# NERSC/swin_v2_weather

Measured on AMD Instinct MI355X. Metric: ERA5 samples/sec (73x721x1440) swin_73var depth12, higher is better.
Workload: dtype bf16

## Files before the change

include/swv2.h:

```cpp
#ifndef SWV2_H
#define SWV2_H
#include <stddef.h>
#include <stdint.h>

#ifdef __cplusplus
extern "C" {
#endif

#define SWV2_VERSION 112

enum {
    SWV2_OK = 0,
    SWV2_ERR_INVALID = -1,
    SWV2_ERR_UNSUPPORTED = -2,
    SWV2_ERR_LAUNCH = -3
};

int swv2_version(void);
const char* swv2_last_error(void);

int swv2_attn_geometry(int L, int head_dim, int* Lp, int* DP);

int swv2_attn_fwd_regime(int L, int head_dim, int has_bias, int dbg);

#define SWV2_ATTN_FIRST_GEN 16
#define SWV2_ATTN_PLAIN_STATS 8192
#define SWV2_ATTN_BWD_TWO_PHASE 32

typedef struct swv2_attn_args {
    const void* qkvh;
    const float* logit_scale;
    const float* bias;
    const void* bias_pack;
    void* oh;
    float* lse;
    const void* doh;
    const float* rnorm;
    void* dqkvh;
    float* dlogit_scale;
    float* dbias;
    int Bw, heads, L, head_dim;
    int nwh, nww;
    int mask_thr;
    int max_chunks;
    int dbg;
    void* dbias_ws;
    size_t dbias_ws_bytes;
    int dbias_partials;
} swv2_attn_args;

#define SWV2_ATTN_K_D256 0
#define SWV2_ATTN_K_FWD3 1
#define SWV2_ATTN_K_FWD3W 2
#define SWV2_ATTN_K_FWD3B 3
#define SWV2_ATTN_K_WIDE 4
#define SWV2_ATTN_K_STREAM 5
#define SWV2_ATTN_K_FIRST_GEN 6
typedef struct swv2_attn_kernel_t {
    int family;
    int Lp, DP;
    int LT, DK;
    int LFIX;
    int regime;
    int aug;
    int bias_lds;
    int qg;
} swv2_attn_kernel_t;
int swv2_attn_fwd_kernel(const swv2_attn_args* a, swv2_attn_kernel_t* out);
int swv2_attn_bwd_kernel(const swv2_attn_args* a, swv2_attn_kernel_t* out);

size_t swv2_attn_dbias_ws_bytes(int heads, int L, int max_chunks);

int swv2_attn_bias_chunks(int Bw);

size_t swv2_attn_pack_bias_bytes(int heads, int L);
int swv2_attn_pack_bias(const float* bias, int heads, int L, void* out, void* stream);
int swv2_attn_pack_bias_multi(const float* bias, int ntab, int heads, int L, void* out, void* stream);

int swv2_attn_fwd(const swv2_attn_args* a, void* stream);
int swv2_attn_bwd(const swv2_attn_args* a, void* stream);


enum swv2_operand_kind {
    SWV2_OP_F32 = 0,
    SWV2_OP_BF16 = 1,
    SWV2_OP_BF16_GELU = 2,
    SWV2_OP_HEADS = 3,
    SWV2_OP_PATCH = 4,
    SWV2_OP_MERGE_LN = 5,
    SWV2_OP_BF16_CSCALE = 6
};

typedef struct swv2_operand {
    int kind;
    const void* ptr;
    const int32_t* rowidx;
    const float* aux0;
    const float* aux1;
    const float* aux2;
    const float* aux3;
    long ld;
    int rows, cols;
    int p[4];
} swv2_operand;

enum swv2_epilogue_kind {
    SWV2_EPI_BF16 = 0,
    SWV2_EPI_F32 = 1,
    SWV2_EPI_QKV_HEADS = 2,
    SWV2_EPI_GELU_GRAD = 3,
    SWV2_EPI_UNPATCH = 4,
    SWV2_EPI_HEADS = 5,
    SWV2_EPI_F32_ACC = 6,
    SWV2_EPI_BF16_GELU = 7,
    SWV2_EPI_UNPATCH_LOSS = 8
};

typedef struct swv2_epilogue {
    int kind;
    void* out;
    const float* bias;
    const void* aux;
    float* aux_out;
    const int32_t* rowidx;
    long ld;
    int p[5];
    const float* loss_tar;
    const float* loss_qw;
    float* loss_part;
    void* loss_resid;
    int q[3];
} swv2_epilogue;

int swv2_linear(const swv2_operand* a, const void* w_bf16, const swv2_epilogue* e, int N, void* stream);

#define SWV2_LINEAR_RESIDENT_QKV128 0
#define SWV2_LINEAR_RESIDENT_QKV192X3 1
#define SWV2_LINEAR_RESIDENT_DX128 2
#define SWV2_LINEAR_WIDE_DMA 3
#define SWV2_LINEAR_WIDE 4
#define SWV2_LINEAR_TILE64 5
#define SWV2_LINEAR_TILE128 6
int swv2_linear_kernel(const swv2_operand* a, const swv2_epilogue* e, int N);

int swv2_linear_wgrad(const swv2_operand* dy, const swv2_operand* x, float* dW, float* db, const int32_t* nmap,
                      const int32_t* kmap, int ldw, int splits, void* stream);
size_t swv2_linear_wgrad_ws_bytes(int M, int N, int K, int splits);
int swv2_linear_wgrad_ws(const swv2_operand* dy, const swv2_operand* x, float* dW, float* db, const int32_t* nmap,
                         const int32_t* kmap, int ldw, int splits, void* ws, size_t ws_bytes, void* stream);
#define SWV2_WGRAD_WIDE 0
#define SWV2_WGRAD_TILE 1
int swv2_linear_wgrad_kernel(const swv2_operand* dy, const swv2_operand* x, int splits, size_t ws_bytes);

typedef struct swv2_wgrad_item {
    swv2_operand dy, x;
    float* dW;
    float* db;
    const int32_t* nmap;
    const int32_t* kmap;
    int ldw;
} swv2_wgrad_item;
size_t swv2_block_wgrad_ws_bytes(int C, int hidden, int heads_dp, int slices);
int swv2_block_wgrad(const swv2_wgrad_item* items4, int slices, void* ws, size_t ws_bytes, void* stream);
#define SWV2_BLOCK_WGRAD_SLAB 0
#define SWV2_BLOCK_WGRAD_GROUPED 1
int swv2_block_wgrad_kernel(const swv2_wgrad_item* items4, int slices, size_t ws_bytes);

int swv2_qk_normalize(void* qkvh_bf16, float* rnorm, int Bw, int heads, int Lp, int L, int DP, void* stream);

int swv2_prep_weight(const float* w, int rows, int cols, int transpose, const int32_t* row_map, int out_rows,
                     const int32_t* col_map, int out_cols, void* out_bf16, void* stream);

typedef struct swv2_prep_item {
    const float* w;
    int rows, cols, transpose;
    const int32_t* row_map;
    int out_rows;
    const int32_t* col_map;
    int out_cols;
    void* out;
    int out_f32;
} swv2_prep_item;
int swv2_prep_chunk(void);
int swv2_prep_item_chunks(int out_rows, int out_cols, int transpose);
int swv2_prep_multi(const swv2_prep_item* items_dev, const int* chunks_dev, int n_chunks, void* stream);

#define SWV2_LN_BWD_MAX_BLOCKS 512
typedef struct swv2_ln_args {
    const void* a;
    const float* res;
    const float* gamma;
    const float* beta;
    const float* scale;
    const int32_t* rowidx;
    float* y;
    float* mean;
    float* rstd;
    const float* dy;
    void* da;
    float* dgamma;
    float* dbeta;
    float* ws;
    int M, C, res_mod, rows_per_sample;
    float eps;
} swv2_ln_args;

int swv2_ln_residual_fwd(const swv2_ln_args* a, void* stream);
int swv2_ln_residual_bwd(const swv2_ln_args* a, void* stream);

int swv2_batch_sum(const float* in, float* out, int B, long n, int accumulate, void* stream);

int swv2_merge_stats(const float* x, float* mean, float* rstd, int B, int H, int W, int C, float eps, void* stream);
int swv2_merge_ln_bwd(const float* x, const void* dn_bf16, const float* gamma, const float* mean, const float* rstd,
                      float* dx, float* dgamma, float* dbeta, int B, int H, int W, int C, void* stream);

int swv2_loss_sums(const float* prd, const float* tar, const float* quad_w, float* sums, int BC, int H, int W, void* stream);
int swv2_loss_grad(const float* prd, const float* tar, const float* quad_w, const float* coef, float* dprd, int BC, int H,
                   int W, void* stream);
#define SWV2_LOSS_PART_SLICES 8
#define SWV2_LOSS_GROUP_ROWS 32
#define SWV2_LOSS_DUMP_BYTES 2048
#define SWV2_LOSS_RESID_PITCH(N) (((N) + 63) / 64 * 64)
int swv2_loss_part_reduce(const float* part, int M, int T, int B, int Cout, int Ct, int coff, float* sums, void* stream);
int swv2_loss_resid_to_image(const void* resid, const float* coef, const float* add, float* out, int B, int Cout, int H, int W, int Cs, int Cadd,
                             void* stream);
int swv2_loss_finalize(const float* sums, int layers, const float* chw, int BC, int C, int absolute, int squared, float* loss, float* coef,
                       void* stream);

int swv2_adam_step(float* p, const float* g, float* m, float* v, long n, float lr, float beta1, float beta2, float eps,
                   int step, float grad_inv_scale, void* stream);

typedef struct swv2_adam_item {
    float* p;
    const float* g;
    float* m;
    float* v;
    long n;
} swv2_adam_item;
int swv2_adam_chunk(void);
int swv2_adam_multi(const swv2_adam_item* items_dev, const int* chunks_dev, int n_chunks, float lr, float beta1, float beta2,
                    float eps, int step, float grad_inv_scale, void* stream);

typedef struct swv2_lamb_item {
    float* p;
    const float* g;
    float* m;
    float* v;
    long n;
    long chunk0;
} swv2_lamb_item;
#define SWV2_LAMB_SUM_DEPTH 64
#define SWV2_LAMB_ADAMW 1
#define SWV2_LAMB_BIAS_CORRECTION 2
#define SWV2_LAMB_GRAD_AVERAGING 4
#define SWV2_LAMB_NVLAMB 8
#define SWV2_LAMB_WS_GNORM2 0
#define SWV2_LAMB_WS_CLIP 1
#define SWV2_LAMB_WS_BC1 2
#define SWV2_LAMB_WS_BC2 3
#define SWV2_LAMB_WS_ITEM(i) (4 + 4 * (i))
int swv2_lamb_chunk(void);
size_t swv2_lamb_ws_bytes(int n_items, int n_chunks);
int swv2_lamb_grad_norm(const swv2_lamb_item* items_dev, const int* chunks_dev, int n_items, int n_chunks, float grad_inv_scale, void* ws,
                        size_t ws_bytes, void* stream);
int swv2_lamb_multi(const swv2_lamb_item* items_dev, const int* chunks_dev, int n_items, int n_chunks, int item_lo, int item_hi,
                    int chunk_lo, int chunk_hi, float lr, float beta1, float beta2, float eps, float weight_decay, float grad_inv_scale,
                    float max_grad_norm, int step, int flags, const float* extra_gnorm2, void* ws, size_t ws_bytes, void* stream);

int swv2_score_slices(int planes, int H, int W);
size_t swv2_score_ws_bytes(int planes, int H, int W);
int swv2_score_sums(const float* prd, long prd_bstride, const float* tar, long tar_bstride, const float* clim, const float* w, int B, int C,
                    int H, int W, void* ws, size_t ws_bytes, void* stream);
int swv2_score_finalize(const void* ws, size_t ws_bytes, int B, int C, int H, int W, const float* scale, float* sums, float* rmse, float* acc,
                        float* rmse_mean, float* acc_mean, void* stream);

int swv2_stats_slices(int C, int H, int W);
size_t swv2_stats_ws_bytes(int C, int H, int W);
int swv2_stats_accumulate(const float* slab, const float* prev, const double* pivot, double* tsum, void* part, size_t part_bytes, int C, int H,
                          int W, int first, void* stream);
int swv2_stats_finalize(const void* part, size_t part_bytes, const double* tsum, const double* pivot, int C, int H, int W, long T,
                        double* folded, float* time_means, void* stream);

size_t swv2_quantile_ws_bytes(int planes, int H, int W, int K);
int swv2_plane_order_stats(const float* x, long bstride, int B, int C, int H, int W, const int* ranks, int K, float* out, int* nan_count,
                           void* ws, size_t ws_bytes, void* stream);

size_t swv2_ens_ws_bytes(int planes, int H, int W, int M);
int swv2_ens_sums(const float* ens, long ens_mstride, long ens_bstride, const float* tar, long tar_bstride, const float* w, int M, int B, int C,
                  int H, int W, void* ws, size_t ws_bytes, void* stream);
int swv2_ens_finalize(const void* ws, size_t ws_bytes, int M, int B, int C, int H, int W, const float* scale, float* sums, int* hist,
                      float* ens_rmse, float* spread, float* crps, float* fair_crps, float* means, void* stream);

int swv2_era5_select_normalize(const float* raw, float* out, const int* chan, const float* mean, const float* stdv, int B, int S,
                               int Csel, int Craw, int Hraw, int Wraw, int H, int W, int Cout_total, int coff, void* stream);
int swv2_era5_zenith(float* out, const float* sun, int B, int nz, int H, int W, int Cout_total, int coff, void* stream);
int swv2_era5_static(const float* stat, float* out, int B, int Cs, int H, int W, int Cout_total, int coff, void* stream);

typedef struct {
    const void* oh;
    const void* wp;
    const float* bp;
    const float* gamma; const float* beta; const float* scale;
    const int32_t* rowidx;
    const float* x;
    void* a1; float* mean; float* rstd;
    float* y;
    int Bw, Lp, heads, C, rows_per_sample;
    float eps;
} swv2_proj_ln_args;
typedef struct {
    const float* dy;
    const void* a1; const float* mean; const float* rstd; const float* gamma; const float* scale;
    const int32_t* rowidx;
    const void* wpt;
    void* da1;
    void* doh;
    float* dgamma; float* dbeta; float* ws;
    int Bw, Lp, heads, C, rows_per_sample;
} swv2_proj_ln_bwd_args;
int swv2_proj_ln_supported(int C, int heads, int head_pad);
size_t swv2_proj_ln_bwd_ws_floats(int Mw, int C);
int swv2_proj_ln_fwd(const swv2_proj_ln_args* a, void* stream);
int swv2_proj_ln_bwd(const swv2_proj_ln_bwd_args* a, void* stream);

typedef struct {
    const float* x;
    const void* w1;
    const float* b1;
    const void* w2;
    const float* b2;
    const float* gamma;
    const float* beta;
    const float* scale;
    void* hpre;
    void* a2;
    float* mean;
    float* rstd;
    float* y;
    int M, C, hidden, rows_per_sample;
    float eps;
} swv2_mlp_args;
int swv2_mlp_supported(int C, int hidden);
int swv2_mlp_recompute_supported(int C, int hidden);
int swv2_mlp_fwd(const swv2_mlp_args* a, void* stream);

typedef struct {
    const float* dy;
    const void* a2;
    const float* mean;
    const float* rstd;
    const float* gamma;
    const float* scale;
    const void* hpre;
    const void* w2t;
    const void* w1t;
    void* da2;
    void* dh;
    float* dx;
    float* dgamma;
    float* dbeta;
    float* ws;
    int M, C, hidden, rows_per_sample;
    const float* x;
    const void* w1;
    const float* b1;
} swv2_mlp_bwd_args;
size_t swv2_mlp_bwd_ws_floats(int M, int C);
int swv2_mlp_bwd(const swv2_mlp_bwd_args* a, void* stream);

int swv2_cpb_fwd(const float* w1, const float* b1, const float* w2, const float* b2, const void* keep_bf16, float* bias,
                 int wh, int ww, int heads, int hidden, float drop_p, void* stream);
int swv2_cpb_bwd(const float* dbias, const float* w1, const float* b1, const float* w2, const void* keep_bf16, float* dw1,
                 float* db1, float* dw2, float* db2, int wh, int ww, int heads, int hidden, float drop_p, void* stream);
size_t swv2_cpb_bwd_ws_bytes(int wh, int ww, int heads, int hidden);
int swv2_cpb_bwd_ws(const float* dbias, const float* w1, const float* b1, const float* w2, const void* keep_bf16, float* dw1,
                    float* db1, float* dw2, float* db2, int wh, int ww, int heads, int hidden, float drop_p, void* ws,
                    size_t ws_bytes, void* stream);

int swv2_cpb_fwd_multi(const float* const* params_dev, int nblk, const uint32_t* keep_bits, float* bias, int wh, int ww, int heads,
                       int hidden, float drop_p, void* stream);
size_t swv2_cpb_bwd_multi_ws_bytes(int nblk, int wh, int ww, int heads, int hidden);
int swv2_cpb_bwd_multi(const float* dbias_tables, int nchunk, const float* const* params_dev, int nblk, const uint32_t* keep_bits,
                       float* grads, int wh, int ww, int heads, int hidden, float drop_p, void* ws, size_t ws_bytes, void* stream);

typedef struct swv2_block_desc {
    int B, T, C, heads, head_dim, hidden, L, Lp, DP, nwh, nww, mask_thr;
    const int32_t* rowidx;
    const int32_t* qkv_map;
    const int32_t* proj_map;
    const float *logit_scale, *qkv_b_pad, *proj_b, *n1_w, *n1_b, *fc1_b, *fc2_b, *n2_w, *n2_b;
    const void *w_qkv, *w_proj, *w_fc1, *w_fc2;
    const void *w_qkvt, *w_projt, *w_fc1t, *w_fc2t;
    const float* x;
    const float* bias;
    void* bias_pack;
    const float* dp1;
    const float* dp2;
    void* qkvh;  float* rnorm; void* oh; float* lse; void* a1; float* mean1; float* rstd1; float* x1;
    void* hpre;  void* hact;   void* a2; float* mean2; float* rstd2;
    float* x2;
    const float* dx2;
    void *da2, *dh, *da1, *doh, *dqkvh;
    float* dx1;
    float* ln_ws;
    float* dx;
    float *d_logit_scale, *d_bias, *d_qkv_w, *d_qkv_b, *d_proj_w, *d_proj_b, *d_n1_w, *d_n1_b, *d_fc1_w, *d_fc1_b,
          *d_fc2_w, *d_fc2_b, *d_n2_w, *d_n2_b;
    int wgrad_splits;
    int ev_kernel;
    void* ev_start;
    void* ev_stop;
    int fuse_proj_ln;
    int fuse_mlp;
    void* wgrad_ws;
    size_t wgrad_ws_bytes;
    int wgrad_group;
    void* grad_zero;
    size_t grad_zero_bytes;
    size_t ln_ws_floats;
    int bias_prepacked;
    float* dbias_part;
    size_t dbias_part_bytes;
} swv2_block_desc;

enum swv2_block_step {
    SWV2_STEP_RNORM_ZERO = 1,
    SWV2_STEP_QKV,
    SWV2_STEP_QK_NORMALIZE,
    SWV2_STEP_PACK_BIAS,
    SWV2_STEP_ATTN_FWD,
    SWV2_STEP_PROJ, SWV2_STEP_LN1_FWD,
    SWV2_STEP_PROJ_LN_FWD,
    SWV2_STEP_FC1, SWV2_STEP_FC2, SWV2_STEP_LN2_FWD,
    SWV2_STEP_MLP_FWD,
    SWV2_STEP_LN2_BWD, SWV2_STEP_WGRAD_FC2, SWV2_STEP_DH, SWV2_STEP_WGRAD_FC1, SWV2_STEP_DX1,
    SWV2_STEP_MLP_BWD,
    SWV2_STEP_LN1_BWD,
    SWV2_STEP_PROJ_LN_BWD,
    SWV2_STEP_WGRAD_PROJ, SWV2_STEP_DOH, SWV2_STEP_ATTN_BWD, SWV2_STEP_WGRAD_QKV, SWV2_STEP_DX,
    SWV2_STEP_LN_FOLD,
    SWV2_STEP_WGRAD_GROUP,
    SWV2_STEP_COUNT
};
#define SWV2_BLOCK_MAX_STEPS 12
enum { SWV2_DBIAS_NONE = 0,
       SWV2_DBIAS_ATOMICS = 1,
       SWV2_DBIAS_WGRAD_WS = 2,
       SWV2_DBIAS_PART = 3 };
typedef struct swv2_block_plan_t {
    int mlp_fused;
    int proj_ln_fused;
    int ln_deferred;
    int wgrad_grouped;
    int wgrad_kernel;
    int grad_zero_in_kernel;
    int attn_fwd_chunks, attn_bwd_chunks;
    int dbias_dest;
    size_t need_hact_bytes;
    size_t need_ln_ws_floats;
    size_t need_wgrad_ws_bytes;
    int n_fwd, n_bwd;
    int fwd[SWV2_BLOCK_MAX_STEPS], bwd[SWV2_BLOCK_MAX_STEPS];
} swv2_block_plan_t;
int swv2_block_plan(const swv2_block_desc* d, swv2_block_plan_t* out);
int swv2_block_step_id(int step);
const char* swv2_block_step_name(int step);

int swv2_block_fwd(const swv2_block_desc* d, void* stream);
int swv2_block_bwd(const swv2_block_desc* d, void* stream);

#ifdef __cplusplus
}
#endif
#endif
```

swin_v2_weather_amd/_lib.py:

```python
from __future__ import annotations

import ctypes as C
import os
import subprocess
import threading

HERE = os.path.dirname(os.path.abspath(__file__))
CSRC = os.path.join(HERE, "csrc")
LIB_PATH = os.environ.get("SWV2_LIB") or os.path.join(HERE, "libswv2.so")
SOURCES = ["capi.hip", "attn.hip", "attn2.hip", "attn_bwd_stream.hip", "attn_wide.hip", "attn_d256.hip", "gemm.hip", "gemm_tn.hip", "gemm_tn_slab.hip", "rowops.hip", "lamb.hip", "block.hip", "cpb.hip", "mlp.hip", "proj_ln.hip", "dataio.hip", "score.hip", "stats.hip", "quantile.hip", "ensemble.hip"]

ABI_VERSION = 112

_lib = None
_lock = threading.Lock()


class Swv2Error(RuntimeError):
    pass


def build_library(force: bool = False, verbose: bool = False) -> str:
    import glob
    srcs = [os.path.join(CSRC, s) for s in SOURCES]
    deps = srcs + glob.glob(os.path.join(CSRC, "*.h")) + [os.path.join(HERE, "..", "include", "swv2.h")]
    if not force and os.path.exists(LIB_PATH) and all(os.path.getmtime(LIB_PATH) >= os.path.getmtime(d) for d in deps):
        return LIB_PATH
    hipcc = os.environ.get("HIPCC", "/opt/rocm/bin/hipcc")
    objs, procs = [], []
    os.makedirs(os.path.join(HERE, "build"), exist_ok=True)
    for s in srcs:
        o = os.path.join(HERE, "build", os.path.basename(s) + ".o")
        objs.append(o)
        cmd = [hipcc, "--offload-arch=gfx950", "-O3", "-std=c++17", "-fPIC", "-c", s, "-o", o]
        procs.append((cmd, subprocess.Popen(cmd, stdout=subprocess.PIPE, stderr=subprocess.STDOUT)))
    for cmd, p in procs:
        out, _ = p.communicate()
        if p.returncode != 0:
            raise Swv2Error("hipcc failed: %s\n%s" % (" ".join(cmd), out.decode()))
        if verbose and out:
            print(out.decode())
    cmd = [hipcc, "--offload-arch=gfx950", "-shared", "-fPIC", "-o", LIB_PATH] + objs
    r = subprocess.run(cmd, stdout=subprocess.PIPE, stderr=subprocess.STDOUT)
    if r.returncode != 0:
        raise Swv2Error("link failed: %s\n%s" % (" ".join(cmd), r.stdout.decode()))
    return LIB_PATH


def source_hash() -> str:
    import glob
    import hashlib
    h = hashlib.sha256()
    files = sorted(glob.glob(os.path.join(CSRC, "*"))) + [os.path.join(HERE, "..", "include", "swv2.h")]
    for f in files:
        if os.path.isfile(f):
            h.update(os.path.basename(f).encode())
            h.update(open(f, "rb").read())
    return h.hexdigest()[:16]


class AttnArgs(C.Structure):
    _fields_ = [("qkvh", C.c_void_p), ("logit_scale", C.c_void_p), ("bias", C.c_void_p), ("bias_pack", C.c_void_p), ("oh", C.c_void_p),
                ("lse", C.c_void_p), ("doh", C.c_void_p), ("rnorm", C.c_void_p), ("dqkvh", C.c_void_p),
                ("dlogit_scale", C.c_void_p), ("dbias", C.c_void_p),
                ("Bw", C.c_int), ("heads", C.c_int), ("L", C.c_int), ("head_dim", C.c_int),
                ("nwh", C.c_int), ("nww", C.c_int), ("mask_thr", C.c_int), ("max_chunks", C.c_int), ("dbg", C.c_int),
                ("dbias_ws", C.c_void_p), ("dbias_ws_bytes", C.c_size_t), ("dbias_partials", C.c_int)]


class AttnKernelInfo(C.Structure):
    _fields_ = [(n, C.c_int) for n in ("family", "Lp", "DP", "LT", "DK", "LFIX", "regime", "aug", "bias_lds", "qg")]


ATTN_K_D256, ATTN_K_FWD3, ATTN_K_FWD3W, ATTN_K_FWD3B, ATTN_K_WIDE, ATTN_K_STREAM, ATTN_K_FIRST_GEN = range(7)
ATTN_K_NAMES = ("D256", "FWD3", "FWD3W", "FWD3B", "WIDE", "STREAM", "FIRST_GEN")


class Operand(C.Structure):
    _fields_ = [("kind", C.c_int), ("ptr", C.c_void_p), ("rowidx", C.c_void_p), ("aux0", C.c_void_p),
                ("aux1", C.c_void_p), ("aux2", C.c_void_p), ("aux3", C.c_void_p), ("ld", C.c_long),
                ("rows", C.c_int), ("cols", C.c_int), ("p", C.c_int * 4)]


class PrepItem(C.Structure):
    _fields_ = [("w", C.c_void_p), ("rows", C.c_int), ("cols", C.c_int), ("transpose", C.c_int), ("row_map", C.c_void_p),
                ("out_rows", C.c_int), ("col_map", C.c_void_p), ("out_cols", C.c_int), ("out", C.c_void_p), ("out_f32", C.c_int)]


class AdamItem(C.Structure):
    _fields_ = [("p", C.c_void_p), ("g", C.c_void_p), ("m", C.c_void_p), ("v", C.c_void_p), ("n", C.c_long)]


class LambItem(C.Structure):
    _fields_ = [("p", C.c_void_p), ("g", C.c_void_p), ("m", C.c_void_p), ("v", C.c_void_p), ("n", C.c_long), ("chunk0", C.c_long)]


class WgradItem(C.Structure):
    _fields_ = [("dy", Operand), ("x", Operand), ("dW", C.c_void_p), ("db", C.c_void_p), ("nmap", C.c_void_p),
                ("kmap", C.c_void_p), ("ldw", C.c_int)]


class Epilogue(C.Structure):
    _fields_ = [("kind", C.c_int), ("out", C.c_void_p), ("bias", C.c_void_p), ("aux", C.c_void_p),
                ("aux_out", C.c_void_p), ("rowidx", C.c_void_p), ("ld", C.c_long), ("p", C.c_int * 5),
                ("loss_tar", C.c_void_p), ("loss_qw", C.c_void_p), ("loss_part", C.c_void_p),
                ("loss_resid", C.c_void_p),
                ("q", C.c_int * 3)]


class ProjLnArgs(C.Structure):
    _fields_ = [(n, C.c_void_p) for n in ("oh", "wp", "bp", "gamma", "beta", "scale", "rowidx", "x", "a1", "mean", "rstd", "y")] + \
               [(n, C.c_int) for n in ("Bw", "Lp", "heads", "C", "rows_per_sample")] + [("eps", C.c_float)]


class ProjLnBwdArgs(C.Structure):
    _fields_ = [(n, C.c_void_p) for n in ("dy", "a1", "mean", "rstd", "gamma", "scale", "rowidx", "wpt", "da1", "doh", "dgamma", "dbeta",
                                           "ws")] + [(n, C.c_int) for n in ("Bw", "Lp", "heads", "C", "rows_per_sample")]


class MlpArgs(C.Structure):
    _fields_ = [(n, C.c_void_p) for n in ("x", "w1", "b1", "w2", "b2", "gamma", "beta", "scale", "hpre", "a2", "mean", "rstd", "y")] + \
               [(n, C.c_int) for n in ("M", "C", "hidden", "rows_per_sample")] + [("eps", C.c_float)]


class MlpBwdArgs(C.Structure):
    _fields_ = [(n, C.c_void_p) for n in ("dy", "a2", "mean", "rstd", "gamma", "scale", "hpre", "w2t", "w1t", "da2", "dh", "dx",
                                           "dgamma", "dbeta", "ws")] + [(n, C.c_int) for n in ("M", "C", "hidden", "rows_per_sample")] + \
               [(n, C.c_void_p) for n in ("x", "w1", "b1")]


class LnArgs(C.Structure):
    _fields_ = [("a", C.c_void_p), ("res", C.c_void_p), ("gamma", C.c_void_p), ("beta", C.c_void_p),
                ("scale", C.c_void_p), ("rowidx", C.c_void_p), ("y", C.c_void_p), ("mean", C.c_void_p),
                ("rstd", C.c_void_p), ("dy", C.c_void_p), ("da", C.c_void_p), ("dgamma", C.c_void_p),
                ("dbeta", C.c_void_p), ("ws", C.c_void_p), ("M", C.c_int), ("C", C.c_int), ("res_mod", C.c_int),
                ("rows_per_sample", C.c_int), ("eps", C.c_float)]


LN_BWD_MAX_BLOCKS = 512
ATTN_FIRST_GEN, ATTN_PLAIN_STATS, ATTN_BWD_TWO_PHASE = 16, 8192, 32
LOSS_PART_SLICES = 8
LOSS_GROUP_ROWS = 32
LOSS_DUMP_BYTES = 2048


def loss_resid_pitch(n: int) -> int:
    return (n + 63) // 64 * 64
class BlockDesc(C.Structure):
    _fields_ = ([(n, C.c_int) for n in ("B", "T", "C", "heads", "head_dim", "hidden", "L", "Lp", "DP", "nwh", "nww", "mask_thr")] +
                [(n, C.c_void_p) for n in (
                    "rowidx", "qkv_map", "proj_map",
                    "logit_scale", "qkv_b_pad", "proj_b", "n1_w", "n1_b", "fc1_b", "fc2_b", "n2_w", "n2_b",
                    "w_qkv", "w_proj", "w_fc1", "w_fc2", "w_qkvt", "w_projt", "w_fc1t", "w_fc2t",
                    "x", "bias", "bias_pack", "dp1", "dp2",
                    "qkvh", "rnorm", "oh", "lse", "a1", "mean1", "rstd1", "x1", "hpre", "hact", "a2", "mean2", "rstd2", "x2",
                    "dx2", "da2", "dh", "da1", "doh", "dqkvh", "dx1", "ln_ws", "dx",
                    "d_logit_scale", "d_bias", "d_qkv_w", "d_qkv_b", "d_proj_w", "d_proj_b", "d_n1_w", "d_n1_b", "d_fc1_w",
                    "d_fc1_b", "d_fc2_w", "d_fc2_b", "d_n2_w", "d_n2_b")] +
                [("wgrad_splits", C.c_int), ("ev_kernel", C.c_int), ("ev_start", C.c_void_p), ("ev_stop", C.c_void_p),
                 ("fuse_proj_ln", C.c_int), ("fuse_mlp", C.c_int), ("wgrad_ws", C.c_void_p), ("wgrad_ws_bytes", C.c_size_t), ("wgrad_group", C.c_int), ("grad_zero", C.c_void_p),
                 ("grad_zero_bytes", C.c_size_t), ("ln_ws_floats", C.c_size_t),
                 ("bias_prepacked", C.c_int), ("dbias_part", C.c_void_p), ("dbias_part_bytes", C.c_size_t)])


LAMB_ADAMW, LAMB_BIAS_CORRECTION, LAMB_GRAD_AVERAGING, LAMB_NVLAMB = 1, 2, 4, 8
LAMB_SUM_DEPTH = 64
LAMB_WS_GNORM2, LAMB_WS_CLIP, LAMB_WS_BC1, LAMB_WS_BC2 = range(4)


def lamb_ws_item(i: int) -> int:
    return 4 + 4 * i


BLOCK_MAX_STEPS = 12
DBIAS_NONE, DBIAS_ATOMICS, DBIAS_WGRAD_WS, DBIAS_PART = range(4)


class BlockPlan(C.Structure):
    _fields_ = ([(n, C.c_int) for n in ("mlp_fused", "proj_ln_fused", "ln_deferred", "wgrad_grouped", "wgrad_kernel", "grad_zero_in_kernel",
                                        "attn_fwd_chunks", "attn_bwd_chunks", "dbias_dest")] +
                [(n, C.c_size_t) for n in ("need_hact_bytes", "need_ln_ws_floats", "need_wgrad_ws_bytes")] +
                [("n_fwd", C.c_int), ("n_bwd", C.c_int), ("fwd", C.c_int * BLOCK_MAX_STEPS), ("bwd", C.c_int * BLOCK_MAX_STEPS)])

    def steps(self, phase):
        lib = load()
        return [lib.swv2_block_step_name(s).decode() for s in getattr(self, phase)[:getattr(self, "n_" + phase)]]


def block_plan(desc: BlockDesc) -> BlockPlan:
    plan = BlockPlan()
    check(load().swv2_block_plan(C.byref(desc), C.byref(plan)), "swv2_block_plan")
    return plan


OP_F32, OP_BF16, OP_BF16_GELU, OP_HEADS, OP_PATCH, OP_MERGE_LN, OP_BF16_CSCALE = range(7)
EPI_BF16, EPI_F32, EPI_QKV_HEADS, EPI_GELU_GRAD, EPI_UNPATCH, EPI_HEADS, EPI_F32_ACC, EPI_BF16_GELU, EPI_UNPATCH_LOSS = range(9)
LINEAR_RESIDENT_QKV128, LINEAR_RESIDENT_QKV192X3, LINEAR_RESIDENT_DX128, LINEAR_WIDE_DMA, LINEAR_WIDE, LINEAR_TILE64, LINEAR_TILE128 = range(7)
LINEAR_WIDE_KERNELS, LINEAR_TILE_KERNELS = (LINEAR_WIDE_DMA, LINEAR_WIDE), (LINEAR_TILE64, LINEAR_TILE128)
WGRAD_WIDE, WGRAD_TILE = range(2)
BLOCK_WGRAD_SLAB, BLOCK_WGRAD_GROUPED = range(2)

_P, _I, _L, _F = C.c_void_p, C.c_int, C.c_long, C.c_float
SYMBOLS = {
    "swv2_version": (_I, []),
    "swv2_last_error": (C.c_char_p, []),
    "swv2_attn_geometry": (_I, [_I, _I, C.POINTER(_I), C.POINTER(_I)]),
    "swv2_attn_fwd_regime": (_I, [_I, _I, _I, _I]),
    "swv2_attn_fwd_kernel": (_I, [C.POINTER(AttnArgs), C.POINTER(AttnKernelInfo)]),
    "swv2_attn_bwd_kernel": (_I, [C.POINTER(AttnArgs), C.POINTER(AttnKernelInfo)]),
    "swv2_attn_pack_bias_bytes": (C.c_size_t, [_I, _I]),
    "swv2_attn_dbias_ws_bytes": (C.c_size_t, [_I, _I, _I]),
    "swv2_attn_pack_bias": (_I, [_P, _I, _I, _P, _P]),
    "swv2_attn_pack_bias_multi": (_I, [_P, _I, _I, _I, _P, _P]),
    "swv2_attn_bias_chunks": (_I, [_I]),
    "swv2_attn_fwd": (_I, [C.POINTER(AttnArgs), _P]),
    "swv2_attn_bwd": (_I, [C.POINTER(AttnArgs), _P]),
    "swv2_linear": (_I, [C.POINTER(Operand), _P, C.POINTER(Epilogue), _I, _P]),
    "swv2_linear_kernel": (_I, [C.POINTER(Operand), C.POINTER(Epilogue), _I]),
    "swv2_linear_wgrad_kernel": (_I, [C.POINTER(Operand), C.POINTER(Operand), _I, C.c_size_t]),
    "swv2_block_wgrad_kernel": (_I, [C.POINTER(WgradItem), _I, C.c_size_t]),
    "swv2_linear_wgrad": (_I, [C.POINTER(Operand), C.POINTER(Operand), _P, _P, _P, _P, _I, _I, _P]),
    "swv2_linear_wgrad_ws_bytes": (C.c_size_t, [_I, _I, _I, _I]),
    "swv2_qk_normalize": (_I, [_P, _P, _I, _I, _I, _I, _I, _P]),
    "swv2_block_wgrad_ws_bytes": (C.c_size_t, [_I, _I, _I, _I]),
    "swv2_block_wgrad": (_I, [C.POINTER(WgradItem), _I, _P, C.c_size_t, _P]),
    "swv2_linear_wgrad_ws": (_I, [C.POINTER(Operand), C.POINTER(Operand), _P, _P, _P, _P, _I, _I, _P, C.c_size_t, _P]),
    "swv2_prep_weight": (_I, [_P, _I, _I, _I, _P, _I, _P, _I, _P, _P]),
    "swv2_ln_residual_fwd": (_I, [C.POINTER(LnArgs), _P]),
    "swv2_ln_residual_bwd": (_I, [C.POINTER(LnArgs), _P]),
    "swv2_batch_sum": (_I, [_P, _P, _I, _L, _I, _P]),
    "swv2_merge_stats": (_I, [_P, _P, _P, _I, _I, _I, _I, _F, _P]),
    "swv2_merge_ln_bwd": (_I, [_P, _P, _P, _P, _P, _P, _P, _P, _I, _I, _I, _I, _P]),
    "swv2_loss_sums": (_I, [_P, _P, _P, _P, _I, _I, _I, _P]),
    "swv2_loss_grad": (_I, [_P, _P, _P, _P, _P, _I, _I, _I, _P]),
    "swv2_loss_part_reduce": (_I, [_P, _I, _I, _I, _I, _I, _I, _P, _P]),
    "swv2_loss_resid_to_image": (_I, [_P, _P, _P, _P, _I, _I, _I, _I, _I, _I, _P]),
    "swv2_loss_finalize": (_I, [_P, _I, _P, _I, _I, _I, _I, _P, _P, _P]),
    "swv2_prep_chunk": (_I, []),
    "swv2_prep_item_chunks": (_I, [_I, _I, _I]),
    "swv2_prep_multi": (_I, [_P, _P, _I, _P]),
    "swv2_adam_chunk": (_I, []),
    "swv2_adam_multi": (_I, [_P, _P, _I, _F, _F, _F, _F, _I, _F, _P]),
    "swv2_adam_step": (_I, [_P, _P, _P, _P, _L, _F, _F, _F, _F, _I, _F, _P]),
    "swv2_lamb_chunk": (_I, []),
    "swv2_lamb_ws_bytes": (C.c_size_t, [_I, _I]),
    "swv2_lamb_grad_norm": (_I, [_P, _P, _I, _I, _F, _P, C.c_size_t, _P]),
    "swv2_lamb_multi": (_I, [_P, _P, _I, _I, _I, _I, _I, _I, _F, _F, _F, _F, _F, _F, _F, _I, _I, _P, _P, C.c_size_t, _P]),
    "swv2_score_slices": (_I, [_I, _I, _I]),
    "swv2_score_ws_bytes": (C.c_size_t, [_I, _I, _I]),
    "swv2_score_sums": (_I, [_P, _L, _P, _L, _P, _P, _I, _I, _I, _I, _P, C.c_size_t, _P]),
    "swv2_score_finalize": (_I, [_P, C.c_size_t, _I, _I, _I, _I, _P, _P, _P, _P, _P, _P, _P]),
    "swv2_stats_slices": (_I, [_I, _I, _I]),
    "swv2_stats_ws_bytes": (C.c_size_t, [_I, _I, _I]),
    "swv2_stats_accumulate": (_I, [_P, _P, _P, _P, _P, C.c_size_t, _I, _I, _I, _I, _P]),
    "swv2_stats_finalize": (_I, [_P, C.c_size_t, _P, _P, _I, _I, _I, _L, _P, _P, _P]),
    "swv2_quantile_ws_bytes": (C.c_size_t, [_I, _I, _I, _I]),
    "swv2_plane_order_stats": (_I, [_P, _L, _I, _I, _I, _I, _P, _I, _P, _P, _P, C.c_size_t, _P]),
    "swv2_ens_ws_bytes": (C.c_size_t, [_I, _I, _I, _I]),
    "swv2_ens_sums": (_I, [_P, _L, _L, _P, _L, _P, _I, _I, _I, _I, _I, _P, C.c_size_t, _P]),
    "swv2_ens_finalize": (_I, [_P, C.c_size_t, _I, _I, _I, _I, _I, _P, _P, _P, _P, _P, _P, _P, _P, _P]),
    "swv2_era5_select_normalize": (_I, [_P, _P, _P, _P, _P] + [_I] * 10 + [_P]),
    "swv2_era5_zenith": (_I, [_P, _P, _I, _I, _I, _I, _I, _I, _P]),
    "swv2_era5_static": (_I, [_P, _P, _I, _I, _I, _I, _I, _I, _P]),
    "swv2_proj_ln_supported": (_I, [_I, _I, _I]),
    "swv2_proj_ln_bwd_ws_floats": (C.c_size_t, [_I, _I]),
    "swv2_proj_ln_fwd": (_I, [C.POINTER(ProjLnArgs), _P]),
    "swv2_proj_ln_bwd": (_I, [C.POINTER(ProjLnBwdArgs), _P]),
    "swv2_mlp_supported": (_I, [_I, _I]),
    "swv2_mlp_recompute_supported": (_I, [_I, _I]),
    "swv2_mlp_fwd": (_I, [C.POINTER(MlpArgs), _P]),
    "swv2_mlp_bwd_ws_floats": (C.c_size_t, [_I, _I]),
    "swv2_mlp_bwd": (_I, [C.POINTER(MlpBwdArgs), _P]),
    "swv2_cpb_fwd": (_I, [_P, _P, _P, _P, _P, _P, _I, _I, _I, _I, _F, _P]),
    "swv2_cpb_bwd": (_I, [_P, _P, _P, _P, _P, _P, _P, _P, _P, _I, _I, _I, _I, _F, _P]),
    "swv2_cpb_bwd_ws": (_I, [_P, _P, _P, _P, _P, _P, _P, _P, _P, _I, _I, _I, _I, _F, _P, C.c_size_t, _P]),
    "swv2_cpb_bwd_ws_bytes": (C.c_size_t, [_I, _I, _I, _I]),
    "swv2_cpb_fwd_multi": (_I, [_P, _I, _P, _P, _I, _I, _I, _I, _F, _P]),
    "swv2_cpb_bwd_multi_ws_bytes": (C.c_size_t, [_I, _I, _I, _I, _I]),
    "swv2_cpb_bwd_multi": (_I, [_P, _I, _P, _I, _P, _P, _I, _I, _I, _I, _F, _P, C.c_size_t, _P]),
    "swv2_block_plan": (_I, [C.POINTER(BlockDesc), C.POINTER(BlockPlan)]),
    "swv2_block_step_id": (_I, [_I]),
    "swv2_block_step_name": (C.c_char_p, [_I]),
    "swv2_block_fwd": (_I, [C.POINTER(BlockDesc), _P]),
    "swv2_block_bwd": (_I, [C.POINTER(BlockDesc), _P]),
}


def load() -> C.CDLL:
    global _lib
    if _lib is not None:
        return _lib
    with _lock:
        if _lib is None:
            if not os.path.exists(LIB_PATH):
                raise Swv2Error(f"{LIB_PATH} not found: run `python -c 'import __graft_entry__ as g; g.build()'` "
                                "(the HIP library is required; there is no fallback path)")
            import torch
            lib = C.CDLL(LIB_PATH)
            for name, (res, args) in SYMBOLS.items():
                fn = getattr(lib, name)
                fn.restype, fn.argtypes = res, args
            got = lib.swv2_version()
            if got != ABI_VERSION:
                raise Swv2Error(f"{LIB_PATH} reports ABI revision {got}, this binding mirrors revision {ABI_VERSION} of include/swv2.h: "
                                "rebuild the library (python -c 'import __graft_entry__ as g; g.build()')")
            _lib = lib
    return _lib


def check(rc: int, what: str = "") -> None:
    if rc != 0:
        msg = load().swv2_last_error()
        raise Swv2Error(f"{what} failed with code {rc}: {msg.decode() if msg else ''}")
```

swin_v2_weather_amd/csrc/block.hip:

```cpp
#include "common.h"

namespace {

swv2_operand op(int kind, const void* p, int rows, int cols, long ld, const int32_t* rowidx = nullptr) {
    swv2_operand o = {};
    o.kind = kind; o.ptr = p; o.rowidx = rowidx; o.ld = ld; o.rows = rows; o.cols = cols;
    return o;
}
swv2_operand op_heads(const void* p, int Bw, int heads, int parts, int Lp, int DP) {
    swv2_operand o = op(SWV2_OP_HEADS, p, Bw * Lp, parts * heads * DP, parts);
    o.p[0] = heads; o.p[2] = Lp; o.p[3] = DP;
    return o;
}
swv2_epilogue epi(int kind, void* out, long ld, const float* bias = nullptr, const void* aux = nullptr,
                  float* aux_out = nullptr, const int32_t* rowidx = nullptr) {
    swv2_epilogue e = {};
    e.kind = kind; e.out = out; e.ld = ld; e.bias = bias; e.aux = aux; e.aux_out = aux_out; e.rowidx = rowidx;
    return e;
}
swv2_attn_args attn(const swv2_block_desc* d, int max_chunks) {
    swv2_attn_args a = {};
    a.qkvh = d->qkvh; a.logit_scale = d->logit_scale; a.bias = d->bias; a.bias_pack = d->bias ? d->bias_pack : nullptr;
    a.oh = d->oh; a.lse = d->lse;
    a.Bw = d->B * d->nwh * d->nww; a.heads = d->heads; a.L = d->L; a.head_dim = d->head_dim; a.nwh = d->nwh; a.nww = d->nww;
    a.mask_thr = d->mask_thr; a.max_chunks = max_chunks;
    return a;
}
void wgrad_items(const swv2_block_desc* d, bool fused, swv2_wgrad_item it[4]) {
    const int BT = d->B * d->T, Bw = d->B * d->nwh * d->nww, Mw = Bw * d->Lp, C = d->C, h = d->heads, hid = d->hidden;
    it[0].dy = op(SWV2_OP_BF16, d->da2, BT, C, C);
    it[0].x = fused ? op(SWV2_OP_BF16_GELU, d->hpre, BT, hid, hid) : op(SWV2_OP_BF16, d->hact, BT, hid, hid);
    it[0].dW = d->d_fc2_w; it[0].db = d->d_fc2_b; it[0].ldw = hid;
    it[1].dy = op(SWV2_OP_BF16, d->dh, BT, hid, hid); it[1].x = op(SWV2_OP_F32, d->x1, BT, C, C);
    it[1].dW = d->d_fc1_w; it[1].db = d->d_fc1_b; it[1].ldw = C;
    it[2].dy = op(SWV2_OP_BF16, d->da1, Mw, C, C); it[2].x = op_heads(d->oh, Bw, h, 1, d->Lp, d->DP);
    it[2].dW = d->d_proj_w; it[2].db = d->d_proj_b; it[2].kmap = d->proj_map; it[2].ldw = C;
    it[3].dy = op_heads(d->dqkvh, Bw, h, 3, d->Lp, d->DP); it[3].x = op(SWV2_OP_F32, d->x, Mw, C, C, d->rowidx);
    it[3].dW = d->d_qkv_w; it[3].db = d->d_qkv_b; it[3].nmap = d->qkv_map; it[3].ldw = C;
}
#define TRY(x) do { int rc_ = (x); if (rc_) return rc_; } while (0)

const struct { int id; const char* name; } STEPS[SWV2_STEP_COUNT] = {
    {0, "end"},
    {0, "rnorm_zero"}, {1, "qkv"}, {0, "qk_normalize"}, {0, "pack_bias"}, {2, "attn_fwd"}, {3, "proj"}, {4, "ln1_fwd"}, {3, "proj_ln_fwd"},
    {5, "fc1"}, {6, "fc2"}, {7, "ln2_fwd"}, {5, "mlp_fwd"},
    {11, "ln2_bwd"}, {12, "wgrad_fc2"}, {13, "dh"}, {14, "wgrad_fc1"}, {15, "dx1"}, {13, "mlp_bwd"}, {16, "ln1_bwd"}, {16, "proj_ln_bwd"},
    {17, "wgrad_proj"}, {18, "doh"}, {19, "attn_bwd"}, {20, "wgrad_qkv"}, {21, "dx"}, {0, "ln_fold"}, {22, "wgrad_group"},
};
static_assert(SWV2_STEP_WGRAD_GROUP + 1 == SWV2_STEP_COUNT && SWV2_STEP_MLP_FWD == 12 && SWV2_STEP_LN2_BWD == 13, "STEPS follows enum swv2_block_step");

#define LAUNCH(step, x)                                                                                     \
    do {                                                                                                    \
        const bool t_ = d->ev_kernel == STEPS[step].id && d->ev_start && d->ev_stop;                         \
        if (t_) (void)hipEventRecord((hipEvent_t)d->ev_start, (hipStream_t)st);                             \
        TRY(x);                                                                                             \
        if (t_) (void)hipEventRecord((hipEvent_t)d->ev_stop, (hipStream_t)st);                              \
    } while (0)

int plan_block(const swv2_block_desc* d, swv2_block_plan_t* p) {
    SWV2_CHECK_ARG(d && p, "swv2_block_plan: null descriptor or plan");
    SWV2_CHECK_ARG(d->B > 0 && d->T > 0 && d->C > 0 && d->heads > 0 && d->hidden > 0 && d->Lp > 0 && d->DP > 0 && d->nwh > 0 && d->nww > 0,
                   "swv2_block_plan: non-positive geometry");
    *p = {};
    const int BT = d->B * d->T, Bw = d->B * d->nwh * d->nww, Mw = Bw * d->Lp, C = d->C, h = d->heads, hid = d->hidden;
    const int sp = d->wgrad_splits > 0 ? d->wgrad_splits : 64;
    const size_t ws_bytes = d->wgrad_ws ? d->wgrad_ws_bytes : 0;
    const size_t ln_pair = swv2_mlp_bwd_ws_floats(BT, C) + swv2_proj_ln_bwd_ws_floats(Mw, C);
    p->need_ln_ws_floats = std::max((size_t)SWV2_LN_BWD_MAX_BLOCKS * 2 * C, ln_pair);
    p->need_wgrad_ws_bytes = d->wgrad_group ? swv2_block_wgrad_ws_bytes(C, hid, h * d->DP, 0) : 0;
    const int prod[4][3] = {{BT, C, hid}, {BT, hid, C}, {Mw, C, h * d->DP}, {Mw, 3 * h * d->DP, C}};
    for (const auto& q : prod)
        p->need_wgrad_ws_bytes = std::max(p->need_wgrad_ws_bytes, swv2_linear_wgrad_ws_bytes(q[0], q[1], q[2], sp));

    p->mlp_fused = d->fuse_mlp && swv2_mlp_supported(C, hid);
    p->proj_ln_fused = d->fuse_proj_ln && swv2_proj_ln_supported(C, h, d->DP);
    p->need_hact_bytes = p->mlp_fused ? 0 : (size_t)BT * hid * 2;
    p->ln_deferred = p->mlp_fused && p->proj_ln_fused && d->ln_ws_floats >= ln_pair;
    p->wgrad_grouped = d->wgrad_group && p->mlp_fused && d->wgrad_ws && ws_bytes >= swv2_block_wgrad_ws_bytes(C, hid, h * d->DP, 0);
    p->wgrad_kernel = -1;
    p->grad_zero_in_kernel = p->mlp_fused && d->grad_zero != nullptr;
    p->attn_fwd_chunks = d->bias ? 32 : 64;
    p->attn_bwd_chunks = 64;
    if (d->bias) {
        p->attn_bwd_chunks = swv2_attn_bias_chunks(Bw);
        p->dbias_dest = d->dbias_part ? SWV2_DBIAS_PART : ws_bytes ? SWV2_DBIAS_WGRAD_WS : SWV2_DBIAS_ATOMICS;
    } else if (d->Lp == 176 && h <= 256) {
        p->attn_bwd_chunks = 256 / h;
    }

    auto fwd = [&](int s) { p->fwd[p->n_fwd++] = s; };
    auto bwd = [&](int s) { p->bwd[p->n_bwd++] = s; };
    const bool wide = d->DP > 64;
    if (wide) fwd(SWV2_STEP_RNORM_ZERO);
    fwd(SWV2_STEP_QKV);
    if (wide) fwd(SWV2_STEP_QK_NORMALIZE);
    if (d->bias && d->bias_pack && !d->bias_prepacked) fwd(SWV2_STEP_PACK_BIAS);
    fwd(SWV2_STEP_ATTN_FWD);
    if (p->proj_ln_fused) fwd(SWV2_STEP_PROJ_LN_FWD);
    else { fwd(SWV2_STEP_PROJ); fwd(SWV2_STEP_LN1_FWD); }
    if (p->mlp_fused) fwd(SWV2_STEP_MLP_FWD);
    else { fwd(SWV2_STEP_FC1); fwd(SWV2_STEP_FC2); fwd(SWV2_STEP_LN2_FWD); }

    const bool single = !p->wgrad_grouped;
    if (p->mlp_fused) {
        bwd(SWV2_STEP_MLP_BWD);
        if (single) { bwd(SWV2_STEP_WGRAD_FC2); bwd(SWV2_STEP_WGRAD_FC1); }
    } else {
        bwd(SWV2_STEP_LN2_BWD); bwd(SWV2_STEP_WGRAD_FC2); bwd(SWV2_STEP_DH); bwd(SWV2_STEP_WGRAD_FC1); bwd(SWV2_STEP_DX1);
    }
    bwd(p->proj_ln_fused ? SWV2_STEP_PROJ_LN_BWD : SWV2_STEP_LN1_BWD);
    if (single) bwd(SWV2_STEP_WGRAD_PROJ);
    if (!p->proj_ln_fused) bwd(SWV2_STEP_DOH);
    bwd(SWV2_STEP_ATTN_BWD);
    if (single) bwd(SWV2_STEP_WGRAD_QKV);
    bwd(SWV2_STEP_DX);
    if (p->ln_deferred && single) bwd(SWV2_STEP_LN_FOLD);
    if (p->wgrad_grouped) bwd(SWV2_STEP_WGRAD_GROUP);
    return SWV2_OK;
}

}

extern "C" int swv2_block_step_id(int step) { return step > 0 && step < SWV2_STEP_COUNT ? STEPS[step].id : -1; }
extern "C" const char* swv2_block_step_name(int step) { return step > 0 && step < SWV2_STEP_COUNT ? STEPS[step].name : nullptr; }

extern "C" int swv2_block_plan(const swv2_block_desc* d, swv2_block_plan_t* p) {
    TRY(plan_block(d, p));
    if (p->wgrad_grouped) {
        swv2_wgrad_item it[4] = {};
        wgrad_items(d, true, it);
        p->wgrad_kernel = swv2_block_wgrad_kernel(it, 0, d->wgrad_ws_bytes);
    }
    return SWV2_OK;
}

extern "C" int swv2_block_fwd(const swv2_block_desc* d, void* st) {
    SWV2_CHECK_ARG(d && d->x && d->x2 && d->qkvh && d->rowidx, "swv2_block_fwd: null descriptor field");
    swv2_block_plan_t p;
    TRY(plan_block(d, &p));
    SWV2_CHECK_ARG(d->hact || !p.need_hact_bytes, "swv2_block_fwd: the separate MLP kernels need hact (swv2_block_plan: need_hact_bytes)");
    const int BT = d->B * d->T, Bw = d->B * d->nwh * d->nww, Mw = Bw * d->Lp, C = d->C, h = d->heads, hid = d->hidden;
    for (int i = 0; i < p.n_fwd; ++i) switch (p.fwd[i]) {
    case SWV2_STEP_RNORM_ZERO:
        if (hipMemsetAsync(d->rnorm, 0, (size_t)Bw * h * 2 * d->Lp * sizeof(float), (hipStream_t)st) != hipSuccess) {
            swv2_set_error("swv2_block_fwd: hipMemsetAsync(rnorm) failed");
            return SWV2_ERR_LAUNCH;
        }
        break;
    case SWV2_STEP_QKV: {
        swv2_operand a = op(SWV2_OP_F32, d->x, Mw, C, C, d->rowidx);
        swv2_epilogue e = epi(SWV2_EPI_QKV_HEADS, d->qkvh, 0, d->qkv_b_pad, nullptr, d->rnorm);
        e.p[0] = h; e.p[2] = d->Lp; e.p[3] = d->DP; e.p[4] = d->L;
        LAUNCH(SWV2_STEP_QKV, swv2_linear(&a, d->w_qkv, &e, 3 * h * d->DP, st));
    } break;
    case SWV2_STEP_QK_NORMALIZE: TRY(swv2_qk_normalize(d->qkvh, (float*)d->rnorm, Bw, h, d->Lp, d->L, d->DP, st)); break;
    case SWV2_STEP_PACK_BIAS: TRY(swv2_attn_pack_bias(d->bias, h, d->L, d->bias_pack, st)); break;
    case SWV2_STEP_ATTN_FWD: {
        swv2_attn_args a = attn(d, p.attn_fwd_chunks);
        LAUNCH(SWV2_STEP_ATTN_FWD, swv2_attn_fwd(&a, st));
    } break;
    case SWV2_STEP_PROJ_LN_FWD: {
        swv2_proj_ln_args m = {};
        m.oh = d->oh; m.wp = d->w_proj; m.bp = d->proj_b; m.gamma = d->n1_w; m.beta = d->n1_b; m.scale = d->dp1; m.rowidx = d->rowidx;
        m.x = d->x; m.a1 = d->a1; m.mean = d->mean1; m.rstd = d->rstd1; m.y = d->x1; m.Bw = Bw; m.Lp = d->Lp; m.heads = h; m.C = C;
        m.rows_per_sample = d->T; m.eps = 1e-5f;
        LAUNCH(SWV2_STEP_PROJ_LN_FWD, swv2_proj_ln_fwd(&m, st));
    } break;
    case SWV2_STEP_PROJ: {
        swv2_operand a = op_heads(d->oh, Bw, h, 1, d->Lp, d->DP);
        swv2_epilogue e = epi(SWV2_EPI_BF16, d->a1, C, d->proj_b);
        LAUNCH(SWV2_STEP_PROJ, swv2_linear(&a, d->w_proj, &e, C, st));
    } break;
    case SWV2_STEP_LN1_FWD: {
        swv2_ln_args l = {};
        l.a = d->a1; l.res = d->x; l.gamma = d->n1_w; l.beta = d->n1_b; l.scale = d->dp1; l.rowidx = d->rowidx; l.y = d->x1;
        l.mean = d->mean1; l.rstd = d->rstd1; l.M = Mw; l.C = C; l.res_mod = 0; l.rows_per_sample = d->T; l.eps = 1e-5f;
        LAUNCH(SWV2_STEP_LN1_FWD, swv2_ln_residual_fwd(&l, st));
    } break;
    case SWV2_STEP_MLP_FWD: {
        swv2_mlp_args m = {};
        m.x = d->x1; m.w1 = d->w_fc1; m.b1 = d->fc1_b; m.w2 = d->w_fc2; m.b2 = d->fc2_b; m.gamma = d->n2_w; m.beta = d->n2_b;
        m.scale = d->dp2; m.hpre = d->hpre; m.a2 = d->a2; m.mean = d->mean2; m.rstd = d->rstd2; m.y = d->x2;
        m.M = BT; m.C = C; m.hidden = hid; m.rows_per_sample = d->T; m.eps = 1e-5f;
        LAUNCH(SWV2_STEP_MLP_FWD, swv2_mlp_fwd(&m, st));
    } break;
    case SWV2_STEP_FC1: {
        swv2_operand a = op(SWV2_OP_F32, d->x1, BT, C, C);
        swv2_epilogue e = epi(SWV2_EPI_BF16_GELU, d->hpre, hid, d->fc1_b, nullptr, (float*)d->hact);
        LAUNCH(SWV2_STEP_FC1, swv2_linear(&a, d->w_fc1, &e, hid, st));
    } break;
    case SWV2_STEP_FC2: {
        swv2_operand a = op(SWV2_OP_BF16, d->hact, BT, hid, hid);
        swv2_epilogue e = epi(SWV2_EPI_BF16, d->a2, C, d->fc2_b);
        LAUNCH(SWV2_STEP_FC2, swv2_linear(&a, d->w_fc2, &e, C, st));
    } break;
    case SWV2_STEP_LN2_FWD: {
        swv2_ln_args l = {};
        l.a = d->a2; l.res = d->x1; l.gamma = d->n2_w; l.beta = d->n2_b; l.scale = d->dp2; l.y = d->x2; l.mean = d->mean2;
        l.rstd = d->rstd2; l.M = BT; l.C = C; l.res_mod = 0; l.rows_per_sample = d->T; l.eps = 1e-5f;
        LAUNCH(SWV2_STEP_LN2_FWD, swv2_ln_residual_fwd(&l, st));
    } break;
    }
    return SWV2_OK;
}

extern "C" int swv2_block_bwd(const swv2_block_desc* d, void* st) {
    SWV2_CHECK_ARG(d && d->dx2 && d->dx && d->da2 && d->dh && d->dx1 && d->da1 && d->doh && d->dqkvh && d->ln_ws,
                   "swv2_block_bwd: null descriptor field");
    swv2_block_plan_t p;
    TRY(plan_block(d, &p));
    SWV2_CHECK_ARG(d->hact || !p.need_hact_bytes, "swv2_block_bwd: the separate MLP kernels need hact (swv2_block_plan: need_hact_bytes)");
    const int BT = d->B * d->T, Bw = d->B * d->nwh * d->nww, Mw = Bw * d->Lp, C = d->C, h = d->heads, hid = d->hidden;
    const int sp = d->wgrad_splits > 0 ? d->wgrad_splits : 64;
    swv2_wgrad_item it[4] = {};
    wgrad_items(d, p.mlp_fused, it);
    float* const ln1_ws = p.ln_deferred ? d->ln_ws + swv2_mlp_bwd_ws_floats(BT, C) : d->ln_ws;
    int n_ln1 = 0, n_ln2 = 0;
    for (int i = 0; i < p.n_bwd; ++i) switch (const int s = p.bwd[i]; s) {
    case SWV2_STEP_MLP_BWD: {
        swv2_mlp_bwd_args m = {};
        m.dy = d->dx2; m.a2 = d->a2; m.mean = d->mean2; m.rstd = d->rstd2; m.gamma = d->n2_w; m.scale = d->dp2; m.hpre = d->hpre;
        m.w2t = d->w_fc2t; m.w1t = d->w_fc1t; m.da2 = d->da2; m.dh = d->dh; m.dx = d->dx1; m.dgamma = d->d_n2_w;
        m.dbeta = d->d_n2_b; m.ws = d->ln_ws; m.M = BT; m.C = C; m.hidden = hid; m.rows_per_sample = d->T;
        LAUNCH(SWV2_STEP_MLP_BWD, swv2_mlp_bwd_impl(&m, st, p.ln_deferred ? &n_ln2 : nullptr, p.grad_zero_in_kernel ? (float*)d->grad_zero : nullptr,
                                                    (long)(d->grad_zero_bytes / 4)));
    } break;
    case SWV2_STEP_LN2_BWD: {
        swv2_ln_args l = {};
        l.a = d->a2; l.dy = d->dx2; l.gamma = d->n2_w; l.scale = d->dp2; l.mean = d->mean2; l.rstd = d->rstd2; l.da = d->da2;
        l.dgamma = d->d_n2_w; l.dbeta = d->d_n2_b; l.ws = d->ln_ws; l.M = BT; l.C = C; l.rows_per_sample = d->T;
        LAUNCH(SWV2_STEP_LN2_BWD, swv2_ln_residual_bwd(&l, st));
    } break;
    case SWV2_STEP_WGRAD_FC2: case SWV2_STEP_WGRAD_FC1: case SWV2_STEP_WGRAD_PROJ: case SWV2_STEP_WGRAD_QKV: {
        const swv2_wgrad_item& w = it[s == SWV2_STEP_WGRAD_FC2 ? 0 : s == SWV2_STEP_WGRAD_FC1 ? 1 : s == SWV2_STEP_WGRAD_PROJ ? 2 : 3];
        LAUNCH(s, swv2_linear_wgrad_ws(&w.dy, &w.x, w.dW, w.db, w.nmap, w.kmap, w.ldw, sp, d->wgrad_ws, d->wgrad_ws_bytes, st));
    } break;
    case SWV2_STEP_DH: {
        swv2_epilogue e = epi(SWV2_EPI_GELU_GRAD, d->dh, hid, nullptr, d->hpre);
        LAUNCH(SWV2_STEP_DH, swv2_linear(&it[0].dy, d->w_fc2t, &e, hid, st));
    } break;
    case SWV2_STEP_DX1: {
        swv2_epilogue e = epi(SWV2_EPI_F32, d->dx1, C, nullptr, d->dx2);
        LAUNCH(SWV2_STEP_DX1, swv2_linear(&it[1].dy, d->w_fc1t, &e, C, st));
    } break;
    case SWV2_STEP_PROJ_LN_BWD: {
        swv2_proj_ln_bwd_args m = {};
        m.dy = d->dx1; m.a1 = d->a1; m.mean = d->mean1; m.rstd = d->rstd1; m.gamma = d->n1_w; m.scale = d->dp1; m.rowidx = d->rowidx;
        m.wpt = d->w_projt; m.da1 = d->da1; m.doh = d->doh; m.dgamma = d->d_n1_w; m.dbeta = d->d_n1_b; m.ws = ln1_ws;
        m.Bw = Bw; m.Lp = d->Lp; m.heads = h; m.C = C; m.rows_per_sample = d->T;
        LAUNCH(SWV2_STEP_PROJ_LN_BWD, swv2_proj_ln_bwd_impl(&m, st, p.ln_deferred ? &n_ln1 : nullptr));
    } break;
    case SWV2_STEP_LN1_BWD: {
        swv2_ln_args l = {};
        l.a = d->a1; l.dy = d->dx1; l.gamma = d->n1_w; l.scale = d->dp1; l.rowidx = d->rowidx; l.mean = d->mean1; l.rstd = d->rstd1;
        l.da = d->da1; l.dgamma = d->d_n1_w; l.dbeta = d->d_n1_b; l.ws = d->ln_ws; l.M = Mw; l.C = C; l.rows_per_sample = d->T;
        LAUNCH(SWV2_STEP_LN1_BWD, swv2_ln_residual_bwd(&l, st));
    } break;
    case SWV2_STEP_DOH: {
        swv2_epilogue e = epi(SWV2_EPI_HEADS, d->doh, 0);
        e.p[0] = h; e.p[2] = d->Lp; e.p[3] = d->DP; e.p[4] = d->L;
        LAUNCH(SWV2_STEP_DOH, swv2_linear(&it[2].dy, d->w_projt, &e, h * d->DP, st));
    } break;
    case SWV2_STEP_ATTN_BWD: {
        swv2_attn_args a = attn(d, p.attn_bwd_chunks);
        a.doh = d->doh; a.rnorm = d->rnorm; a.dqkvh = d->dqkvh; a.dlogit_scale = d->d_logit_scale; a.dbias = d->d_bias;
        if (p.dbias_dest == SWV2_DBIAS_PART) { a.dbias_ws = d->dbias_part; a.dbias_ws_bytes = d->dbias_part_bytes; a.dbias_partials = 1; }
        if (p.dbias_dest == SWV2_DBIAS_WGRAD_WS) { a.dbias_ws = d->wgrad_ws; a.dbias_ws_bytes = d->wgrad_ws_bytes; }
        LAUNCH(SWV2_STEP_ATTN_BWD, swv2_attn_bwd(&a, st));
    } break;
    case SWV2_STEP_DX: {
        swv2_epilogue e = epi(SWV2_EPI_F32, d->dx, C, nullptr, d->dx1, nullptr, d->rowidx);
        LAUNCH(SWV2_STEP_DX, swv2_linear(&it[3].dy, d->w_qkvt, &e, C, st));
    } break;
    case SWV2_STEP_LN_FOLD:
        swv2_launch_ln_partials_reduce2(d->ln_ws, d->d_n2_w, d->d_n2_b, n_ln2, ln1_ws, d->d_n1_w, d->d_n1_b, n_ln1, C, (hipStream_t)st);
        break;
    case SWV2_STEP_WGRAD_GROUP: {
        swv2_ln_partials lnp = {{d->ln_ws, ln1_ws}, {d->d_n2_w, d->d_n1_w}, {d->d_n2_b, d->d_n1_b}, {n_ln2, n_ln1}, C};
        LAUNCH(SWV2_STEP_WGRAD_GROUP, swv2_block_wgrad_ln(it, 0, d->wgrad_ws, d->wgrad_ws_bytes, p.ln_deferred ? &lnp : nullptr, st));
    } break;
    }
    return SWV2_OK;
}
```

swin_v2_weather_amd/csrc/gemm.hip:

```cpp
#include "common.h"

#include <cmath>
#include <cstdlib>
#include "gemm_common.h"

namespace {

constexpr int EP = 68;

struct EpiDesc {
    void* out;
    const float* bias;
    const void* aux;
    float* aux_out;
    const int32_t* rowidx;
    long ld;
    int M, N;
    int p0, p1, p2, p3, p4;
    uint32_t mg0, mg1, mg2;
    const float* loss_tar; const float* loss_qw; float* loss_part; uint16_t* loss_resid; int q0, q1, q2, q3;
};

enum { E_BF16 = 0, E_F32 = 1, E_QKV_HEADS = 2, E_GELU_GRAD = 3, E_UNPATCH = 4, E_HEADS = 5, E_F32_ACC = 6, E_BF16_GELU = 7,
       E_UNPATCH_LOSS = 8, E_UNPATCH_LOSS_SKIP = 9 };
// ... 638 lines not shown
    const int wr = wave >> 2, wc = wave & 3;
    const int xcd = blockIdx.x & 7, nper = gridDim.x >> 3, stages = K / 32;
    const uint32_t lds0 = (uint32_t)(uintptr_t)smem;
    const int drow = wave * 32 + (lane >> 2);
    int dkc[2];
#pragma unroll
    for (int i = 0; i < 2; ++i) dkc[i] = (lane & 3) ^ ((0 - ((drow + 16 * i) >> 2)) & 3);
    struct Tile { int m_base, n_base; uint32_t boff[2], aoff[2]; };
    auto make_tile = [&](int mt, int nt) {
        Tile t;
        t.m_base = mt * WBM; t.n_base = nt * WBN;
#pragma unroll
        for (int i = 0; i < 2; ++i) {
            const int row = drow + 16 * i;
            t.boff[i] = 2u * (uint32_t)(min(t.n_base + row, N - 1) * K + dkc[i] * 8);
            t.aoff[i] = AK == A_BF16 ? 2u * (uint32_t)(min(t.m_base + row, M - 1) * (int)al.d.ld + dkc[i] * 8) : 0u;
        }
        return t;
    };
    auto issue = [&](const Tile& tl, int t, int slot) {
        const uint32_t la = lds0 + (uint32_t)(slot * WSTG * 2) + (uint32_t)(wave * 2048), lb = la + WBM * 32 * 2;
#pragma unroll
        for (int i = 0; i < 2; ++i) dma_x4(Wb + t * 32, tl.boff[i], lb + 1024 * i);
        if constexpr (AK == A_BF16) {
#pragma unroll
            for (int i = 0; i < 2; ++i) dma_x4((const uint16_t*)al.d.ptr + t * 32, tl.aoff[i], la + 1024 * i);
        } else {
#pragma unroll
            for (int i = 0; i < 2; ++i)
                dma_x4(al.d.ptr, 2u * al.elem_off(min(tl.m_base + drow + 16 * i, M - 1), t * 32 + dkc[i] * 8), la + 1024 * i);
        }
    };
    int v = blockIdx.x >> 3, mt = 0, nt = 0;
    while (v < vmax && !wide_tile(xcd, v, mtiles, ntn, mt, nt)) v += nper;
    if (v >= vmax) return;
    Tile cur = make_tile(mt, nt);
    issue(cur, 0, 0); issue(cur, 1, 1); issue(cur, 2, 2);
    asm volatile("s_waitcnt vmcnt(8)" ::: "memory");
    __builtin_amdgcn_s_barrier();
    if (wr == 1) __builtin_amdgcn_s_barrier();
    for (;;) {
        int v2 = v + nper, mt2 = 0, nt2 = 0;
        while (v2 < vmax && !wide_tile(xcd, v2, mtiles, ntn, mt2, nt2)) v2 += nper;
        const bool has_next = v2 < vmax;
        const Tile nxt = has_next ? make_tile(mt2, nt2) : cur;
        f32x4 acc[8][4];
#pragma unroll
        for (int i = 0; i < 8; ++i)
#pragma unroll
            for (int j = 0; j < 4; ++j) acc[i][j] = (f32x4){0.f, 0.f, 0.f, 0.f};
        for (int t = 0; t < stages; ++t) {
            if (t + 3 < stages) issue(cur, t + 3, (t + 3) & 3);
            else issue(nxt, has_next ? t + 3 - stages : stages - 1, (t + 3) & 3);
            const uint16_t* As = smem + (t & 3) * WSTG;
            const uint16_t* Bs = As + WBM * 32;
            bf16x8 af[8], bf[4];
#pragma unroll
            for (int j = 0; j < 4; ++j) bf[j] = *(const bf16x8*)(Bs + swz32(wc * 64 + j * 16 + fr, g));
#pragma unroll
            for (int i = 0; i < 8; ++i) af[i] = *(const bf16x8*)(As + swz32(wr * 128 + i * 16 + fr, g));
            asm volatile("s_waitcnt vmcnt(8)" ::: "memory");
            asm volatile("s_waitcnt lgkmcnt(0)" ::: "memory");
            __builtin_amdgcn_sched_barrier(0);
            __builtin_amdgcn_s_barrier();
            __builtin_amdgcn_sched_barrier(0);
            __builtin_amdgcn_s_setprio(1);
#pragma unroll
            for (int i = 0; i < 8; ++i)
#pragma unroll
                for (int j = 0; j < 4; ++j) acc[i][j] = mfma32(af[i], bf[j], acc[i][j]);
            __builtin_amdgcn_s_setprio(0);
            __builtin_amdgcn_sched_barrier(0);
            __builtin_amdgcn_s_barrier();
            __builtin_amdgcn_sched_barrier(0);
        }
        if (wr == 0) __builtin_amdgcn_s_barrier();
        __builtin_amdgcn_sched_barrier(0);
        {
            float* st = (float*)(smem + 3 * WSTG) + wave * 16 * EP;
            if (cur.n_base + wc * 64 < N) wide_epilogue<EK>(ep, acc, st, cur.m_base + wr * 128, cur.n_base + wc * 64, lane);
        }
        asm volatile("s_waitcnt lgkmcnt(0)" ::: "memory");
        __builtin_amdgcn_sched_barrier(0);
        __builtin_amdgcn_s_barrier();
        if (wr == 1) __builtin_amdgcn_s_barrier();
        __builtin_amdgcn_sched_barrier(0);
        if (!has_next) break;
        cur = nxt; v = v2;
    }
    if (wr == 0) __builtin_amdgcn_s_barrier();
}

__device__ __forceinline__ int tn_pchunk(int row, int c) { return ((((c >> 1) ^ (row & 7)) << 1) | (c & 1)); }
template <int YK, int XK>
__global__ __launch_bounds__(WTH) void gemm_tn_wide_kernel(ALoad<YK> yl, ALoad<XK> xl, float* __restrict__ part, float* __restrict__ dbpart,
                                                           int M, int N, int K, int S, int wgs, int per_xcd) {
    static_assert((YK == A_BF16 || YK == A_HEADS) && (XK == A_BF16 || XK == A_HEADS), "raw bf16 operands");
    constexpr int SLABE = 32 * 256;
    __shared__ __attribute__((aligned(1024))) unsigned char smem_b[WSM_BYTES];
    uint16_t* const smem = (uint16_t*)smem_b;
    const int tid = threadIdx.x, lane = tid & 63, wave = __builtin_amdgcn_readfirstlane(tid >> 6);
    const int fr = lane & 15, g = lane >> 4;
    const int wr = wave >> 2, wc = wave & 3;
    const int w = (blockIdx.x & 7) * per_xcd + (blockIdx.x >> 3);
    if ((int)(blockIdx.x >> 3) >= per_xcd || w >= wgs) return;
    const int ntk = K / WBN, tiles = (N / WBM) * ntk;
    const int slice = w / tiles, tile = w - slice * tiles, tn = tile / ntk, tk = tile - tn * ntk;
    const int n_base = tn * WBM, k_base = tk * WBN;
    const int T = M / 32, t0 = (int)((long)slice * T / S), t1 = (int)((long)(slice + 1) * T / S), stages = t1 - t0;
    const uint32_t lds0 = (uint32_t)(uintptr_t)smem;
    int drw[2], dcl[2];
    uint32_t yoff[2], xoff[2];
#pragma unroll
    for (int i = 0; i < 2; ++i) {
        drw[i] = wave * 4 + 2 * i + (lane >> 5);
        dcl[i] = tn_pchunk(drw[i], lane & 31) * 8;
        yoff[i] = YK == A_BF16 ? 2u * (uint32_t)((t0 * 32 + drw[i]) * (int)yl.d.ld + n_base + dcl[i]) : 0u;
        xoff[i] = XK == A_BF16 ? 2u * (uint32_t)((t0 * 32 + drw[i]) * (int)xl.d.ld + k_base + dcl[i]) : 0u;
    }
    const long ystep = 32 * (long)yl.d.ld, xstep = 32 * (long)xl.d.ld;
    auto issue = [&](int t, int slot) {
        const uint32_t ly = lds0 + (uint32_t)(slot * WSTG * 2) + (uint32_t)(wave * 2048), lx = ly + SLABE * 2;
#pragma unroll
        for (int i = 0; i < 2; ++i) {
            if constexpr (YK == A_BF16) dma_x4((const uint16_t*)yl.d.ptr + t * ystep, yoff[i], ly + 1024 * i);
            else dma_x4(yl.d.ptr, 2u * yl.elem_off((t0 + t) * 32 + drw[i], n_base + dcl[i]), ly + 1024 * i);
        }
#pragma unroll
        for (int i = 0; i < 2; ++i) {
            if constexpr (XK == A_BF16) dma_x4((const uint16_t*)xl.d.ptr + t * xstep, xoff[i], lx + 1024 * i);
            else dma_x4(xl.d.ptr, 2u * xl.elem_off((t0 + t) * 32 + drw[i], k_base + dcl[i]), lx + 1024 * i);
        }
    };
    f32x4 acc[8][4];
#pragma unroll
    for (int i = 0; i < 8; ++i)
#pragma unroll
        for (int j = 0; j < 4; ++j) acc[i][j] = (f32x4){0.f, 0.f, 0.f, 0.f};
    auto trf = [&](const uint16_t* slab, int r0, int c0) -> bf16x4 {
        const int row = r0 + 4 * g + (fr >> 2), col = c0 + (fr & 3) * 4;
        return lds_tr_read(slab + row * 256 + tn_pchunk(row, col >> 3) * 8 + (col & 7));
    };
    float cs[8] = {0.f, 0.f, 0.f, 0.f, 0.f, 0.f, 0.f, 0.f};
    const int cs_off = (tid >> 5) * 256 + tn_pchunk(tid >> 5, tid & 31) * 8;
    const bool want_db = dbpart != nullptr;

    if (stages > 0) {
        issue(0, 0); issue(min(1, stages - 1), 1); issue(min(2, stages - 1), 2);
        asm volatile("s_waitcnt vmcnt(8)" ::: "memory");
        __builtin_amdgcn_s_barrier();
        if (wr == 1) __builtin_amdgcn_s_barrier();
        for (int t = 0; t < stages; ++t) {
            issue(min(t + 3, stages - 1), (t + 3) & 3);
            const uint16_t* Ys = smem + (t & 3) * WSTG;
            const uint16_t* Xs = Ys + SLABE;
            bf16x8 af[8], bf[4];
#pragma unroll
            for (int j = 0; j < 4; ++j)
                bf[j] = __builtin_shufflevector(trf(Xs, 0, wc * 64 + 16 * j), trf(Xs, 16, wc * 64 + 16 * j), 0, 1, 2, 3, 4, 5, 6, 7);
#pragma unroll
            for (int i = 0; i < 8; ++i)
                af[i] = __builtin_shufflevector(trf(Ys, 0, wr * 128 + 16 * i), trf(Ys, 16, wr * 128 + 16 * i), 0, 1, 2, 3, 4, 5, 6, 7);
            if (want_db && ((t0 + t) % ntk) == tk) {
                const uint4 a = *(const uint4*)(Ys + cs_off), b = *(const uint4*)(Ys + cs_off + 16 * 256);
                float va[8], vb[8];
                unpack8(a, va); unpack8(b, vb);
#pragma unroll
                for (int e = 0; e < 8; ++e) cs[e] += va[e] + vb[e];
            }
            asm volatile("s_waitcnt vmcnt(8)" ::: "memory");
            asm volatile("s_waitcnt lgkmcnt(0)" ::: "memory");
            __builtin_amdgcn_sched_barrier(0);
            __builtin_amdgcn_s_barrier();
            __builtin_amdgcn_sched_barrier(0);
            __builtin_amdgcn_s_setprio(1);
#pragma unroll
            for (int i = 0; i < 8; ++i)
#pragma unroll
                for (int j = 0; j < 4; ++j) acc[i][j] = mfma32(af[i], bf[j], acc[i][j]);
            __builtin_amdgcn_s_setprio(0);
            __builtin_amdgcn_sched_barrier(0);
            __builtin_amdgcn_s_barrier();
            __builtin_amdgcn_sched_barrier(0);
        }
        if (wr == 0) __builtin_amdgcn_s_barrier();
        asm volatile("s_waitcnt vmcnt(0)" ::: "memory");
    }
    __syncthreads();
    Epi<E_F32> ep;
    ep.d.out = part + (size_t)slice * N * K; ep.d.bias = nullptr; ep.d.aux = nullptr; ep.d.aux_out = nullptr; ep.d.rowidx = nullptr;
    ep.d.ld = K; ep.d.M = N; ep.d.N = K;
    wide_epilogue<E_F32>(ep, acc, (float*)smem + wave * 16 * EP, n_base + wr * 128, k_base + wc * 64, lane);
    if (want_db) {
        __syncthreads();
        float* red = (float*)smem;
#pragma unroll
        for (int e = 0; e < 8; ++e) red[(tid >> 5) * 256 + (tid & 31) * 8 + e] = cs[e];
        __syncthreads();
        if (tid < 256) {
            float sum = 0.f;
#pragma unroll
            for (int r = 0; r < 16; ++r) sum += red[r * 256 + tid];
            dbpart[((size_t)slice * ntk + tk) * N + n_base + tid] = sum;
        }
    }
}

template <int AK, int EK>
__global__ __launch_bounds__(WTH) void gemm_nt_wide_kernel(ALoad<AK> al, const uint16_t* __restrict__ Wb, Epi<EK> ep,
                                                           int M, int N, int K, int mtiles, int ntn) {
    static_assert(!ALoad<AK>::ROW_FASTEST, "row-major staging map only");
    constexpr int TILE = (WBM + WBN) * BK;
    __shared__ __attribute__((aligned(1024))) uint16_t smem[2 * TILE];
    static_assert(2 * TILE * 2 >= 8 * 16 * EP * 4, "the epilogue staging re-uses the tile buffers");
    const int tid = threadIdx.x, lane = tid & 63, wave = __builtin_amdgcn_readfirstlane(tid >> 6);
    const int fr = lane & 15, g = lane >> 4;
    const int wr = wave >> 2, wc = wave & 3;
    int mt, nt;
    if (!wide_tile(blockIdx.x & 7, blockIdx.x >> 3, mtiles, ntn, mt, nt)) return;
    const int m_base = mt * WBM, n_base = nt * WBN;
    const uint32_t lds0 = (uint32_t)(uintptr_t)smem;
    f32x4 acc[8][4];
#pragma unroll
    for (int i = 0; i < 8; ++i)
#pragma unroll
        for (int j = 0; j < 4; ++j) acc[i][j] = (f32x4){0.f, 0.f, 0.f, 0.f};
    {
        const int ksteps = K / BK;
        const int drow = wave * 32 + (lane >> 3);
        uint32_t boff[4];
#pragma unroll
        for (int i = 0; i < 4; ++i) {
            const int row = drow + 8 * i, kcl = (lane & 7) ^ ((row >> 1) & 7);
            boff[i] = 2u * (uint32_t)((n_base + row) * K + kcl * 8);
        }
        typename ALoad<AK>::Raw ra[4];
        int arow[4];
        uint32_t aok = 0;
        const int kc = tid & 7;
#pragma unroll
        for (int i = 0; i < 4; ++i) {
            const int src = al.row_of(m_base + (tid >> 3) + 64 * i);
            arow[i] = max(src, 0);
            aok |= (src >= 0 ? 1u : 0u) << i;
        }
        auto issue = [&](int s, int buf) {
            const uint32_t lb = lds0 + (uint32_t)(buf * TILE * 2) + (uint32_t)(wave * 4096) + WBM * BK * 2;
#pragma unroll
            for (int i = 0; i < 4; ++i) dma_x4(Wb + s * BK, boff[i], lb + 1024 * i);
#pragma unroll
            for (int i = 0; i < 4; ++i) ra[i] = al.raw_unc(arow[i], s * BK + kc * 8);
        };
        auto commit = [&](int buf) {
            uint16_t* As = smem + buf * TILE;
#pragma unroll
            for (int i = 0; i < 4; ++i) {
                uint4 v = al.cvt(ra[i]);
                if (!((aok >> i) & 1)) v = make_uint4(0, 0, 0, 0);
                *(uint4*)(As + swz((tid >> 3) + 64 * i, kc)) = v;
            }
        };
        auto compute = [&](int buf) {
            const uint16_t* As = smem + buf * TILE;
            const uint16_t* Bs = As + WBM * BK;
#pragma unroll
            for (int kk = 0; kk < 2; ++kk) {
                bf16x8 bf[4];
#pragma unroll
                for (int j = 0; j < 4; ++j) bf[j] = *(const bf16x8*)(Bs + swz(wc * 64 + j * 16 + fr, kk * 4 + g));
#pragma unroll
                for (int i = 0; i < 8; ++i) {
                    const bf16x8 af = *(const bf16x8*)(As + swz(wr * 128 + i * 16 + fr, kk * 4 + g));
#pragma unroll
                    for (int j = 0; j < 4; ++j) acc[i][j] = mfma32(af, bf[j], acc[i][j]);
                }
            }
        };
        issue(0, 0);
        asm volatile("s_waitcnt vmcnt(0)" ::: "memory");
        commit(0);
        __syncthreads();
        for (int s = 0; s + 1 < ksteps; ++s) {
            issue(s + 1, (s + 1) & 1);
            __builtin_amdgcn_sched_barrier(0);
            compute(s & 1);
            __builtin_amdgcn_sched_barrier(0);
            asm volatile("s_waitcnt vmcnt(0)" ::: "memory");
            commit((s + 1) & 1);
            __syncthreads();
        }
        compute((ksteps - 1) & 1);
        __syncthreads();
    }
    wide_epilogue<EK>(ep, acc, (float*)smem + wave * 16 * EP, m_base + wr * 128, n_base + wc * 64, lane);
}

#ifdef SWV2_RW_STAMPS
__device__ unsigned long long rw_stamps[256 * 8];
#define SWV2_STAMPS
#endif
#include "stamps.h"
__device__ __forceinline__ int swzk(int r, int kc, int K) { return r * K + ((kc ^ ((r >> 1) & 7)) << 3); }

template <int AK, int EK, int N, int K, int BMT, int HS = 16>
__global__ __launch_bounds__(512) void gemm_rw_kernel(ALoad<AK> al, const uint16_t* __restrict__ Wb, Epi<EK> ep, int M) {
    constexpr int NTH = 512, KC = K / 8;
    constexpr int ACH = BMT * KC / NTH;
    constexpr int RT = BMT / 64;
    constexpr int CT = N / 32;
    constexpr int WCH = N * KC / NTH;
    constexpr int A_BYTES = BMT * K * 2, ST_BYTES = 8 * 16 * EP * 4;
    constexpr int AS_BYTES = A_BYTES > ST_BYTES ? A_BYTES : ST_BYTES;
    static_assert(BMT * KC % NTH == 0 && N * KC % NTH == 0 && K % 64 == 0 && N % 64 == 0, "tile shapes");
    static_assert(N * K * 2 + AS_BYTES <= 160 * 1024, "LDS budget");
    __shared__ __attribute__((aligned(16))) uint16_t Ws[N * K];
    __shared__ __attribute__((aligned(16))) unsigned char as_raw[AS_BYTES];
    __shared__ __attribute__((aligned(16))) float bs[N];
    uint16_t* As = (uint16_t*)as_raw;
    float* stage_all = (float*)as_raw;

    const int tid = threadIdx.x, lane = tid & 63, wave = tid >> 6;
    const int fr = lane & 15, g = lane >> 4;
    const int wr = wave >> 1, wc = wave & 1;
    const int ntiles = (M + BMT - 1) / BMT;
    static_assert(EK != E_F32 || (RT == 1 && CT == 4), "the E_F32 prefetch below covers one 16 x 64 wave tile");
    for (int i = tid; i < N; i += NTH) bs[i] = ep.d.bias ? ep.d.bias[i] : 0.f;
    int erow_nxt = -1, erow_cur = -1;
    f32x4 aux_nxt[4], aux_cur[4];
    const int ecol = wc * (N / 2) + (lane & 3) * 16;

    typename ALoad<AK>::Raw ra[ACH];
    int arow[ACH];
    int erow_res = -1;
    auto crow = [&](int c) { return AK == A_HEADS ? ((c >> 1) & (BMT - 1)) : c / KC; };
    auto ccol = [&](int c) { return AK == A_HEADS ? (((c / (2 * BMT)) << 1) | (c & 1)) : c % KC; };
    static_assert(AK != A_HEADS || (BMT & (BMT - 1)) == 0, "head-major chunk map needs a power-of-two tile height");
    uint32_t ain = 0;
    uint32_t aok = 0;
    bool ein = false;
    auto resolve = [&](int t) {
        ain = 0;
#pragma unroll
        for (int i = 0; i < ACH; ++i) {
            const int c = tid + i * NTH, m = t * BMT + crow(c);
            const bool in = (t < ntiles) && (m < M);
            ain |= (uint32_t)in << i;
            if constexpr (AK == A_F32) arow[i] = al.d.rowidx[min(m, M - 1)];
            else arow[i] = min(m, M - 1);
        }
        if constexpr (EK == E_F32) {
            const int m = t * BMT + wr * 16 + (lane >> 2);
            ein = (t < ntiles) && (m < M);
            erow_res = ein ? ep.d.rowidx[m] : -1;
        }
    };
    auto issue = [&]() {
        aok = 0;
#pragma unroll
        for (int i = 0; i < ACH; ++i) {
            const int c = tid + i * NTH;
            const int r = ((ain >> i) & 1) ? arow[i] : -1;
            if constexpr (AK == A_HEADS) ra[i] = al.raw_at(r, ccol(c) * 8);
            else ra[i] = al.raw_unc(max(r, 0), ccol(c) * 8);
            aok |= (uint32_t)(r >= 0) << i;
        }
        if constexpr (EK == E_F32) {
            erow_nxt = ein ? erow_res : -1;
            const float* ax = (const float*)ep.d.aux + (long)max(erow_nxt, 0) * ep.d.ld + ecol;
#pragma unroll
            for (int i = 0; i < 4; ++i) aux_nxt[i] = *(const f32x4*)(ax + 4 * i);
        }
    };
    auto commit = [&]() {
#pragma unroll
        for (int i = 0; i < ACH; ++i) {
            const int c = tid + i * NTH;
            *(uint4*)(As + swzk(crow(c), ccol(c), K)) = ((aok >> i) & 1) ? al.cvt(ra[i]) : make_uint4(0, 0, 0, 0);
        }
    };
    const int G = gridDim.x;
    STAMP_DECL(8)
    auto tile_step = [&](int t) {
        STAMP_WAITV();
        STAMP(0);
        commit();
        if constexpr (EK == E_F32) {
            erow_cur = erow_nxt;
#pragma unroll
            for (int i = 0; i < 4; ++i) aux_cur[i] = aux_nxt[i];
        }
        STAMP(1);
        __syncthreads();
        STAMP(2);
        issue();
        resolve(t + 2 * G);
        STAMP(3);
        f32x4 acc[RT][CT];
#pragma unroll
        for (int i = 0; i < RT; ++i)
#pragma unroll
            for (int j = 0; j < CT; ++j) acc[i][j] = (f32x4){0.f, 0.f, 0.f, 0.f};
#pragma unroll
        for (int ks = 0; ks < K / 32; ++ks) {
            bf16x8 af[RT];
#pragma unroll
            for (int i = 0; i < RT; ++i) af[i] = *(const bf16x8*)(As + swzk(wr * 16 * RT + i * 16 + fr, ks * 4 + g, K));
#pragma unroll
            for (int j = 0; j < CT; ++j) {
                const bf16x8 bf = *(const bf16x8*)(Ws + swzk(wc * (N / 2) + j * 16 + fr, ks * 4 + g, K));
#pragma unroll
                for (int i = 0; i < RT; ++i) acc[i][j] = mfma32(af[i], bf, acc[i][j]);
            }
        }
        asm volatile("" :: "v"(acc[0][0][0]), "v"(acc[RT - 1][CT - 1][3]));
        STAMP(4);
        __syncthreads();
        STAMP(5);
        float* st = stage_all + wave * 16 * EP;
#pragma unroll
        for (int i = 0; i < RT; ++i)
#pragma unroll
            for (int j0 = 0; j0 < CT; j0 += 4) {
#pragma unroll
                for (int j = 0; j < 4; ++j)
#pragma unroll
                    for (int r = 0; r < 4; ++r) st[(4 * g + r) * EP + 16 * j + fr] = acc[i][j0 + j][r];
                const int m0 = t * BMT + wr * 16 * RT + i * 16, n0 = wc * (N / 2) + j0 * 16;
                if constexpr (EK == E_QKV_HEADS) {
                    const EpiDesc& d = ep.d;
                    const int h = d.p0, Lp = d.p2, L = d.p4;
                    const int r = lane & 15, slot = lane >> 4, nb = n0 + slot * 16, m = m0 + r;
                    if (m < d.M) {
                        const int ph = HS == 16 ? nb >> 4 : nb >> 5, lp = (h == 1) ? ph : fdiv(ph, h, d.mg1), hd = ph - lp * h;
                        const int part = lp + d.p1;
                        const int bw = fdiv(m, Lp, d.mg0), tt = m - bw * Lp;
                        const bool valid = tt < L;
                        float v[16];
                        float ss = 0.f;
#pragma unroll
                        for (int j = 0; j < 16; j += 4) {
                            const f32x4 x = *(const f32x4*)(st + r * EP + slot * 16 + j) + *(const f32x4*)(bs + nb + j);
#pragma unroll
                            for (int e = 0; e < 4; ++e) {
                                v[j + e] = valid ? x[e] : 0.f;
                                ss = fmaf(v[j + e], v[j + e], ss);
                            }
                        }
                        if constexpr (HS == 32) ss += __shfl_xor(ss, 16);
                        float rn = 1.f;
                        if (part < 2) {
                            rn = 1.f / fmaxf(sqrtf(ss), 1e-12f);
                            if (HS == 16 || !(slot & 1)) d.aux_out[(((long)bw * h + hd) * 2 + part) * Lp + tt] = valid ? rn : 0.f;
                        }
                        uint16_t* o = (uint16_t*)d.out + ((((long)bw * h + hd) * 3 + part) * Lp + tt) * HS + (HS == 32 ? (slot & 1) * 16 : 0);
                        float w8[8];
#pragma unroll
                        for (int e = 0; e < 8; ++e) w8[e] = v[e] * rn;
                        *(uint4*)o = pack8(w8);
#pragma unroll
                        for (int e = 0; e < 8; ++e) w8[e] = v[8 + e] * rn;
                        *(uint4*)(o + 8) = pack8(w8);
                    }
                } else if constexpr (EK == E_F32) {
                    if (erow_cur >= 0) {
                        float* o = (float*)ep.d.out + (long)erow_cur * ep.d.ld + ecol;
                        const int r = lane >> 2, c0 = (lane & 3) * 16;
#pragma unroll
                        for (int q = 0; q < 4; ++q)
                            *(f32x4*)(o + 4 * q) = *(const f32x4*)(st + r * EP + c0 + 4 * q) + *(const f32x4*)(bs + ecol + 4 * q) + aux_cur[q];
                    }
                } else {
                    ep.tile(st, m0, n0, lane);
                }
            }
        STAMP(6);
        __syncthreads();
        STAMP(7);
    };
    int t = blockIdx.x;
    resolve(t);
    issue();
    resolve(t + G);
#pragma unroll
    for (int i = 0; i < WCH; ++i) {
        const int c = tid + i * NTH, n = c / KC, kc = c - n * KC;
        *(uint4*)(Ws + swzk(n, kc, K)) = *(const uint4*)(Wb + (long)n * K + kc * 8);
    }

    STAMP_START();
    for (; t < ntiles; t += G) tile_step(t);
#ifdef SWV2_RW_STAMPS
    if (tid == 0)
        for (int k = 0; k < 8; ++k) rw_stamps[blockIdx.x * 8 + k] = st_acc[k];
#endif
}

enum class LinearKernel {
    RESIDENT_QKV128 = SWV2_LINEAR_RESIDENT_QKV128, RESIDENT_QKV192X3 = SWV2_LINEAR_RESIDENT_QKV192X3, RESIDENT_DX128 = SWV2_LINEAR_RESIDENT_DX128,
    WIDE_DMA = SWV2_LINEAR_WIDE_DMA, WIDE = SWV2_LINEAR_WIDE, TILE64 = SWV2_LINEAR_TILE64, TILE128 = SWV2_LINEAR_TILE128
};

constexpr bool qkv_pair(int ak, int ek) { return ak == A_F32 && ek == E_QKV_HEADS; }
constexpr bool dx_pair(int ak, int ek) { return ak == A_HEADS && ek == E_F32; }
constexpr bool loss_epi(int ek) { return ek == E_UNPATCH_LOSS || ek == E_UNPATCH_LOSS_SKIP; }
constexpr bool wide_pair(int ak, int ek) {
    return (ak == A_F32 || ak == A_BF16 || ak == A_HEADS) &&
           (ek == E_BF16 || ek == E_F32 || ek == E_F32_ACC || ek == E_QKV_HEADS || ek == E_HEADS || ek == E_GELU_GRAD || ek == E_BF16_GELU);
}
constexpr bool dma_loader(int ak) { return ak == A_BF16 || ak == A_HEADS; }

LinearKernel linear_kernel_for(int ak, int ek, const swv2_operand* a, const swv2_epilogue* e, int N, int wide) {
    const int M = a->rows, K = a->cols;
    if (qkv_pair(ak, ek) && M >= 256 * 128 && a->rowidx) {
        if (N == 384 && K == 128 && e->p[3] == 16) return LinearKernel::RESIDENT_QKV128;
        if (N == 768 && K == 192 && e->p[3] == 32 && e->p[0] == 8) return LinearKernel::RESIDENT_QKV192X3;
    }
    if (dx_pair(ak, ek) && N == 128 && K == 384 && M >= 256 * 64 && e->rowidx && e->aux && !a->rowidx) return LinearKernel::RESIDENT_DX128;
    if (wide_pair(ak, ek)) {
        const bool part192 = dx_pair(ak, ek) && N == 192 && K == 768 && !a->rowidx && M >= 64 * WBM &&
                             (double)a->rows * a->cols * 2 < 4.29e9;
        if (wide && (N % WBN == 0 || part192) && K % BK == 0 && (N >= 512 || part192) && K >= 512 && M >= 16 * WBM) {
            const bool small = (double)a->rows * (ak == A_HEADS ? a->cols : a->ld) * 2 < 4.29e9;
            return dma_loader(ak) && small && K % 128 == 0 && (ak == A_HEADS || !a->rowidx) ? LinearKernel::WIDE_DMA : LinearKernel::WIDE;
        }
    }
    if (loss_epi(ek)) return LinearKernel::TILE64;
    if (qkv_pair(ak, ek) || dx_pair(ak, ek)) {
        const double w1 = cdiv(M, BM), w2 = cdiv(M, BM / 2), slots = 768.0;
        const double e1 = w1 / (std::ceil(w1 / slots) * slots), e2 = w2 / (std::ceil(w2 / slots) * slots);
        if (e2 > e1 + 0.08) return LinearKernel::TILE64;
    }
    return LinearKernel::TILE128;
}

int linear_epi_kind(int ak, const swv2_epilogue* e) {
    static_assert(E_BF16 == SWV2_EPI_BF16 && E_BF16_GELU == SWV2_EPI_BF16_GELU && A_F32 == SWV2_OP_F32 && A_BF16_CS == SWV2_OP_BF16_CSCALE,
                  "A_* / E_* mirror the public kinds");
    if (ak == A_BF16_CS) {
        if (e->kind == SWV2_EPI_F32) return E_F32;
        swv2_set_error("swv2_linear: SWV2_OP_BF16_CSCALE supports SWV2_EPI_F32 only (got %d)", e->kind);
        return SWV2_ERR_INVALID;
    }
    if (ak == A_F32 && e->kind == SWV2_EPI_UNPATCH_LOSS) return e->p[3] ? E_UNPATCH_LOSS_SKIP : E_UNPATCH_LOSS;
    if (e->kind >= SWV2_EPI_BF16 && e->kind <= SWV2_EPI_BF16_GELU) return e->kind;
    swv2_set_error("swv2_linear: unknown epilogue kind %d (or not available for operand kind %d)", e->kind, ak);
    return SWV2_ERR_INVALID;
}

template <int EK>
Epi<EK> make_epi(const swv2_epilogue* e, int M, int N) {
    Epi<EK> ep;
    ep.d.out = e->out; ep.d.bias = e->bias; ep.d.aux = e->aux; ep.d.aux_out = e->aux_out; ep.d.rowidx = e->rowidx;
    ep.d.ld = e->ld; ep.d.M = M; ep.d.N = N;
    ep.d.p0 = e->p[0]; ep.d.p1 = e->p[1]; ep.d.p2 = e->p[2]; ep.d.p3 = e->p[3]; ep.d.p4 = e->p[4];
    ep.d.mg0 = ep.d.mg1 = ep.d.mg2 = 0;
    ep.d.loss_tar = nullptr; ep.d.loss_qw = nullptr; ep.d.loss_part = nullptr; ep.d.loss_resid = nullptr; ep.d.q0 = ep.d.q1 = ep.d.q2 = ep.d.q3 = 0;
    if (EK == E_QKV_HEADS || EK == E_HEADS) { ep.d.mg0 = fdiv_magic(e->p[2]); ep.d.mg1 = fdiv_magic(e->p[0]); ep.d.mg2 = fdiv_magic(e->p[3]); }
    if (EK == E_UNPATCH || loss_epi(EK)) { ep.d.mg0 = fdiv_magic((e->p[1] / 4) * (e->p[2] / 4)); ep.d.mg1 = fdiv_magic(e->p[2] / 4); }
    if (loss_epi(EK)) {
        ep.d.loss_tar = e->loss_tar; ep.d.loss_qw = e->loss_qw; ep.d.loss_part = e->loss_part; ep.d.loss_resid = (uint16_t*)e->loss_resid;
        ep.d.q0 = e->q[0]; ep.d.q1 = e->q[1];
        const long nb = M / ((e->p[1] / 4) * (e->p[2] / 4)), plane = (long)e->p[1] * e->p[2];
        ep.d.q2 = e->q[2] ? e->q[2] : (int)(nb * e->p[0] * plane);
        ep.d.q3 = (int)(nb * e->ld * plane);
    }
    return ep;
}

template <int AK, int EK>
int launch_nt2(const swv2_operand* a, const void* w, const swv2_epilogue* e, int M, int N, int K, hipStream_t st) {
    const Epi<EK> ep = make_epi<EK>(e, M, N);
    const uint16_t* wb = (const uint16_t*)w;
    const LinearKernel kern = linear_kernel_for(AK, EK, a, e, N, swv2_gemm_wide());
    switch (kern) {
        case LinearKernel::RESIDENT_QKV128:
            if constexpr (qkv_pair(AK, EK)) {
                Epi<EK> ep1 = ep;
                ep1.d.p1 = 0;
                hipLaunchKernelGGL((gemm_rw_kernel<AK, EK, 384, 128, 128>), dim3(256), dim3(512), 0, st, make_loader<AK>(a), wb, ep1, M);
            }
            break;
        case LinearKernel::RESIDENT_QKV192X3:
            if constexpr (qkv_pair(AK, EK)) {
                for (int part = 0; part < 3; ++part) {
                    Epi<EK> ep2 = ep;
                    ep2.d.N = 256;
                    ep2.d.p1 = part;
                    ep2.d.bias = e->bias ? e->bias + 256 * part : nullptr;
                    hipLaunchKernelGGL((gemm_rw_kernel<AK, EK, 256, 192, 128, 32>), dim3(256), dim3(512), 0, st, make_loader<AK>(a),
                                       wb + (size_t)part * 256 * 192, ep2, M);
                }
            }
            break;
        case LinearKernel::RESIDENT_DX128:
            if constexpr (dx_pair(AK, EK))
                hipLaunchKernelGGL((gemm_rw_kernel<AK, EK, 128, 384, 64>), dim3(256), dim3(512), 0, st, make_loader<AK>(a), wb, ep, M);
            break;
        case LinearKernel::WIDE_DMA:
        case LinearKernel::WIDE:
            if constexpr (wide_pair(AK, EK)) {
                SWV2_CHECK_ARG((double)N * K * 2 < 4.29e9, "swv2_linear: weight too large for the wide kernel's 32-bit offsets");
                const int mtiles = cdiv(M, WBM), ntn = cdiv(N, WBN), groups = cdiv(mtiles, 8);
                const int vmax = cdiv(groups, 8) * 8 * ntn;
                if (kern == LinearKernel::WIDE_DMA) {
                    if constexpr (dma_loader(AK))
                        hipLaunchKernelGGL((gemm_nt_wide_dma_kernel<AK, EK>), dim3(8 * (vmax < 32 || !swv2_wide_persist() ? vmax : 32)), dim3(WTH), 0, st,
                                           make_loader<AK>(a), wb, ep, M, N, K, mtiles, ntn, vmax);
                } else {
                    hipLaunchKernelGGL((gemm_nt_wide_kernel<AK, EK>), dim3(8 * vmax), dim3(WTH), 0, st, make_loader<AK>(a), wb, ep, M, N, K, mtiles, ntn);
                }
            }
            break;
        case LinearKernel::TILE64:
            if constexpr (qkv_pair(AK, EK) || dx_pair(AK, EK) || loss_epi(EK))
                hipLaunchKernelGGL((gemm_nt_kernel<AK, EK, BM / 2>), dim3(cdiv(M, BM / 2)), dim3(NTHREADS), 0, st, make_loader<AK>(a), wb, ep, M, N, K);
            break;
        case LinearKernel::TILE128:
            if constexpr (!loss_epi(EK))
                hipLaunchKernelGGL((gemm_nt_kernel<AK, EK>), dim3(cdiv(M, BM)), dim3(NTHREADS), 0, st, make_loader<AK>(a), wb, ep, M, N, K);
            break;
    }
    SWV2_CHECK_LAUNCH("swv2_linear");
    return SWV2_OK;
}

template <int AK>
int launch_nt1(const swv2_operand* a, const void* w, const swv2_epilogue* e, int M, int N, int K, hipStream_t st) {
    const int ek = linear_epi_kind(AK, e);
    if (ek < 0) return ek;
    if constexpr (AK == A_BF16_CS) {
        return launch_nt2<AK, E_F32>(a, w, e, M, N, K, st);
    } else {
    if constexpr (AK == A_F32) {
        if (ek == E_UNPATCH_LOSS_SKIP) return launch_nt2<AK, E_UNPATCH_LOSS_SKIP>(a, w, e, M, N, K, st);
        if (ek == E_UNPATCH_LOSS) return launch_nt2<AK, E_UNPATCH_LOSS>(a, w, e, M, N, K, st);
    }
    switch (ek) {
        case E_BF16: return launch_nt2<AK, E_BF16>(a, w, e, M, N, K, st);
        case E_F32: return launch_nt2<AK, E_F32>(a, w, e, M, N, K, st);
        case E_F32_ACC: return launch_nt2<AK, E_F32_ACC>(a, w, e, M, N, K, st);
        case E_QKV_HEADS: return launch_nt2<AK, E_QKV_HEADS>(a, w, e, M, N, K, st);
        case E_HEADS: return launch_nt2<AK, E_HEADS>(a, w, e, M, N, K, st);
        case E_GELU_GRAD: return launch_nt2<AK, E_GELU_GRAD>(a, w, e, M, N, K, st);
        case E_UNPATCH: return launch_nt2<AK, E_UNPATCH>(a, w, e, M, N, K, st);
        case E_BF16_GELU: return launch_nt2<AK, E_BF16_GELU>(a, w, e, M, N, K, st);
    }
    return SWV2_ERR_INVALID;
    }
}

}

int swv2_tn_wide_launch(const swv2_operand* y, const swv2_operand* x, float* part, float* dbpart, int M, int N, int K, int S, hipStream_t st) {
    const int tiles = (N / WBM) * (K / WBN), wgs = S * tiles, per_xcd = cdiv(wgs, 8);
#define SWV2_TNW(YK_, XK_)                                                                                                           \
    hipLaunchKernelGGL((gemm_tn_wide_kernel<YK_, XK_>), dim3(8 * per_xcd), dim3(WTH), 0, st, make_loader<YK_>(y), make_loader<XK_>(x), part, \
                       dbpart, M, N, K, S, wgs, per_xcd)
    if (y->kind == SWV2_OP_BF16 && x->kind == SWV2_OP_BF16) SWV2_TNW(A_BF16, A_BF16);
    else if (y->kind == SWV2_OP_BF16 && x->kind == SWV2_OP_HEADS) SWV2_TNW(A_BF16, A_HEADS);
    else if (y->kind == SWV2_OP_HEADS && x->kind == SWV2_OP_BF16) SWV2_TNW(A_HEADS, A_BF16);
    else { swv2_set_error("swv2_linear_wgrad: wide kernel: operand pair (%d, %d) not instantiated", y->kind, x->kind); return SWV2_ERR_UNSUPPORTED; }
#undef SWV2_TNW
    SWV2_CHECK_LAUNCH("swv2_linear_wgrad");
    return SWV2_OK;
}

#ifdef SWV2_RW_STAMPS
extern "C" int swv2_debug_rw_stamps(void* out) {
    return hipMemcpyFromSymbol(out, HIP_SYMBOL(rw_stamps), sizeof(unsigned long long) * 256 * 8) == hipSuccess ? 0 : -3;
}
#endif

extern "C" int swv2_linear_kernel(const swv2_operand* a, const swv2_epilogue* e, int N) {
    SWV2_CHECK_ARG(a && e && N > 0 && a->rows > 0 && a->cols > 0, "swv2_linear_kernel: null operand / epilogue or empty product");
    SWV2_CHECK_ARG(a->kind >= SWV2_OP_F32 && a->kind <= SWV2_OP_BF16_CSCALE, "swv2_linear_kernel: unknown operand kind %d", a->kind);
    const int ek = linear_epi_kind(a->kind, e);
    return ek < 0 ? ek : (int)linear_kernel_for(a->kind, ek, a, e, N, swv2_gemm_wide());
}

extern "C" int swv2_linear(const swv2_operand* a, const void* w_bf16, const swv2_epilogue* e, int N, void* stream) {
    int rc = check_operand(a, "swv2_linear");
    if (rc) return rc;
    SWV2_CHECK_ARG(w_bf16 && e && e->out && N > 0, "swv2_linear: null weight / epilogue / N");
    SWV2_CHECK_ARG(((uintptr_t)w_bf16 & 15) == 0 && ((uintptr_t)e->out & 15) == 0, "swv2_linear: unaligned pointer");
    if (e->kind == SWV2_EPI_BF16_GELU) SWV2_CHECK_ARG(e->aux_out != nullptr, "swv2_linear: GELU epilogue needs aux_out");
    if (e->kind == SWV2_EPI_BF16 || e->kind == SWV2_EPI_GELU_GRAD || e->kind == SWV2_EPI_BF16_GELU)
        SWV2_CHECK_ARG(e->ld % 8 == 0 && e->ld >= N, "swv2_linear: output pitch %ld must be a multiple of 8 and >= N", e->ld);
    if (e->kind == SWV2_EPI_F32 || e->kind == SWV2_EPI_F32_ACC)
        SWV2_CHECK_ARG(e->ld % 4 == 0 && e->ld >= N, "swv2_linear: output pitch %ld must be a multiple of 4 and >= N", e->ld);
    if (e->kind == SWV2_EPI_QKV_HEADS || e->kind == SWV2_EPI_HEADS)
        SWV2_CHECK_ARG((e->p[3] == 16 || e->p[3] == 32 || e->p[3] == 64 || e->p[3] == 96 || e->p[3] == 128 || e->p[3] == 256) && N % e->p[3] == 0 && e->p[0] > 0 && e->p[2] > 0,
                       "swv2_linear: head-split epilogue needs DP in {16,32,64,96,128,256} and N a multiple of DP (DP=%d N=%d)", e->p[3], N);
    if (e->kind == SWV2_EPI_UNPATCH || e->kind == SWV2_EPI_UNPATCH_LOSS)
        SWV2_CHECK_ARG(N == e->p[0] * 16, "swv2_linear: un-patchify needs N == Cout*16");
    if (e->kind == SWV2_EPI_UNPATCH_LOSS) {
        SWV2_CHECK_ARG(a->kind == SWV2_OP_F32, "swv2_linear: the loss epilogue takes an fp32 operand");
        SWV2_CHECK_ARG((e->p[4] == 0 || (e->p[4] >= e->p[0] && e->q[2] > 0)) && (!e->aux_out || e->ld >= e->p[0]) && e->q[2] >= 0,
                       "swv2_linear: loss epilogue: p[4] (channels of the destination tensor) needs q[2] (its dump offset), aux_out needs ld >= Cout");
        SWV2_CHECK_ARG(e->loss_tar && e->loss_qw && e->loss_part && e->loss_resid && e->q[0] >= e->q[1] + e->p[0] && e->q[1] >= 0,
                       "swv2_linear: the loss epilogue needs target, quadrature weights, sums, residual and q[1] + Cout <= q[0]");
        SWV2_CHECK_ARG((((uintptr_t)e->loss_tar | (uintptr_t)e->loss_resid) & 15) == 0, "swv2_linear: unaligned loss pointer");
        const double plane_ = (double)e->p[1] * e->p[2], nb_ = (double)a->rows / ((e->p[1] / 4) * (e->p[2] / 4));
        SWV2_CHECK_ARG((e->p[1] / 4) * (e->p[2] / 4) >= SWV2_LOSS_GROUP_ROWS, "swv2_linear: the loss epilogue needs at least %d patches per sample", SWV2_LOSS_GROUP_ROWS);
        const double cmax_ = fmax(fmax((double)e->p[3], (double)e->p[0]), fmax((double)e->p[4], e->aux_out ? (double)e->ld : 0.0));
        SWV2_CHECK_ARG(nb_ * e->q[0] * plane_ < 4.29e9 && nb_ * cmax_ * plane_ + 1024 < 4.29e9 && (double)a->rows * SWV2_LOSS_RESID_PITCH(N) + 2048 < 4.29e9 && (double)e->q[2] < 4.29e9,
                       "swv2_linear: the loss epilogue indexes its tensors with 32-bit element offsets (tensor too large)");
    }
    const int M = a->rows, K = a->cols;
    hipStream_t st = (hipStream_t)stream;
    switch (a->kind) {
        case SWV2_OP_F32: return launch_nt1<A_F32>(a, w_bf16, e, M, N, K, st);
        case SWV2_OP_BF16: return launch_nt1<A_BF16>(a, w_bf16, e, M, N, K, st);
        case SWV2_OP_BF16_GELU: return launch_nt1<A_BF16_GELU>(a, w_bf16, e, M, N, K, st);
        case SWV2_OP_HEADS: return launch_nt1<A_HEADS>(a, w_bf16, e, M, N, K, st);
        case SWV2_OP_PATCH: return launch_nt1<A_PATCH>(a, w_bf16, e, M, N, K, st);
        case SWV2_OP_MERGE_LN: return launch_nt1<A_MERGE_LN>(a, w_bf16, e, M, N, K, st);
        case SWV2_OP_BF16_CSCALE: return launch_nt1<A_BF16_CS>(a, w_bf16, e, M, N, K, st);
    }
    swv2_set_error("swv2_linear: unknown operand kind %d", a->kind);
    return SWV2_ERR_INVALID;
}
```

swin_v2_weather_amd/csrc/gemm_common.h:

```cpp
#pragma once
#include <cstdlib>
#include "common.h"

int swv2_tn_wide_launch(const swv2_operand* y, const swv2_operand* x, float* part, float* dbpart, int M, int N, int K, int S, hipStream_t st);

size_t swv2_tn_slab_ws_bytes(int C, int hidden, int heads_dp);
bool swv2_tn_slab_covers(const swv2_wgrad_item* it, size_t ws_bytes);
int swv2_tn_slab_launch(const swv2_wgrad_item* it, void* ws, size_t ws_bytes, const swv2_ln_partials* ln, hipStream_t st);

inline int swv2_env_switch(const char* name) { const char* v = getenv(name); return v ? atoi(v) : 1; }
inline int swv2_gemm_wide() { return swv2_env_switch("SWV2_GEMM_WIDE"); }
inline int swv2_wide_persist() { return swv2_env_switch("SWV2_WIDE_PERSIST"); }

namespace {

constexpr int BM = 128, BN = 128, BK = 64;
constexpr int KCH = BK / 8;
constexpr int NTHREADS = 256;

__device__ __forceinline__ int swz(int r, int kc) { return r * BK + ((kc ^ ((r >> 1) & 7)) << 3); }

__device__ __forceinline__ void erf_parts(float x, float& erf_v, float& gauss) {
    const float z = fabsf(x) * 0.70710678118654752f;
    const float t = __builtin_amdgcn_rcpf(fmaf(0.3275911f, z, 1.f));
    gauss = __expf(-z * z);
    const float poly = t * fmaf(t, fmaf(t, fmaf(t, fmaf(t, 1.061405429f, -1.453152027f), 1.421413741f), -0.284496736f), 0.254829592f);
    const float e = fmaf(-poly, gauss, 1.f);
    erf_v = copysignf(e, x);
}
__device__ __forceinline__ int fdiv(int n, int d, uint32_t magic) {
    int q = (int)__umulhi((uint32_t)n, magic);
    return q - (q * d > n);
}
static inline uint32_t fdiv_magic(int d) { return d > 1 ? (uint32_t)((0x100000000ull + (uint64_t)d - 1) / (uint64_t)d) : 0u; }

__device__ __forceinline__ float gelu_f(float x) {
    float e, gs;
    erf_parts(x, e, gs);
    return 0.5f * x * (1.f + e);
}
__device__ __forceinline__ float gelu_grad_f(float x) {
    float e, gs;
    erf_parts(x, e, gs);
    return fmaf(x * 0.3989422804014327f, gs, 0.5f * (1.f + e));
}

constexpr int GT_LO = (127 - 14) << 7;
constexpr int GT_HALF = 18 * 128;
constexpr int GT_N = 2 * GT_HALF;
typedef unsigned short u16x2_t __attribute__((ext_vector_type(2)));

__device__ __forceinline__ uint16_t gelu_tab_arg(int i) { return (uint16_t)(((i / GT_HALF) << 15) | (GT_LO + i % GT_HALF)); }

template <int ESZ, bool SIGNED = true>
__device__ __forceinline__ uint32_t gelu_tab_off2(uint32_t w, bool& bad) {
    const u16x2_t a = __builtin_bit_cast(u16x2_t, w & 0x7fff7fffu);
    const u16x2_t lo = {(unsigned short)GT_LO, (unsigned short)GT_LO};
    const u16x2_t mx = {(unsigned short)(GT_HALF - 1), (unsigned short)(GT_HALF - 1)};
    const u16x2_t idx = a - lo;
    const u16x2_t idc = __builtin_elementwise_min(idx, mx);
    bad = bad || (__builtin_bit_cast(uint32_t, idx) != __builtin_bit_cast(uint32_t, idc));
    if constexpr (!SIGNED) return __builtin_bit_cast(uint32_t, (u16x2_t)(idc * (unsigned short)ESZ));
    const u16x2_t sg = __builtin_bit_cast(u16x2_t, w) >> 15;
    const u16x2_t half = {(unsigned short)GT_HALF, (unsigned short)GT_HALF};
    const u16x2_t off = (idc + sg * half) * (unsigned short)ESZ;
    return __builtin_bit_cast(uint32_t, off);
}

struct LoadDesc {
    const void* ptr;
    const int32_t* rowidx;
    const float* aux0;
    const float* aux1;
    const float* aux2;
    const float* aux3;
    long ld;
    int M, K;
    int p0, p1, p2, p3;
    uint32_t mg0, mg1, mg2;
};

template <int KIND> struct ALoad;

enum { A_F32 = 0, A_BF16 = 1, A_BF16_GELU = 2, A_HEADS = 3, A_PATCH = 4, A_MERGE_LN = 5, A_BF16_CS = 6 };

struct RawF32 { f32x4 a, b; };
__device__ __forceinline__ uint4 cvt_f32x8(const RawF32& r) {
    uint4 o;
    o.x = f2bf2(r.a[0], r.a[1]); o.y = f2bf2(r.a[2], r.a[3]); o.z = f2bf2(r.b[0], r.b[1]); o.w = f2bf2(r.b[2], r.b[3]);
    return o;
}

template <> struct ALoad<A_F32> {
    static constexpr bool ROW_FASTEST = false;
    static constexpr bool LINEAR = true;
    typedef RawF32 Raw;
    LoadDesc d;
    __device__ __forceinline__ Raw raw_lin(uint32_t off) const {
        const float* p = (const float*)d.ptr + off;
        Raw o = {*(const f32x4*)p, *(const f32x4*)(p + 4)};
        return o;
    }
    __device__ __forceinline__ int row_of(int m) const { return m >= d.M ? -1 : (d.rowidx ? d.rowidx[m] : m); }
    __device__ __forceinline__ Raw raw_at(int r, int k0) const {
        Raw z = {(f32x4){0.f, 0.f, 0.f, 0.f}, (f32x4){0.f, 0.f, 0.f, 0.f}};
        if (r < 0 || k0 >= d.K) return z;
        const float* p = (const float*)d.ptr + (long)r * d.ld + k0;
        Raw o = {*(const f32x4*)p, *(const f32x4*)(p + 4)};
        return o;
    }
    __device__ __forceinline__ Raw raw(int m, int k0) const { return raw_at(row_of(m), k0); }
    __device__ __forceinline__ Raw raw_unc(int r, int k0) const {
        const float* p = (const float*)d.ptr + (long)r * d.ld + k0;
        Raw o = {*(const f32x4*)p, *(const f32x4*)(p + 4)};
        return o;
    }
    __device__ __forceinline__ uint4 cvt(const Raw& r) const { return cvt_f32x8(r); }
    __device__ __forceinline__ uint4 chunk(int m, int k0) const { return cvt(raw(m, k0)); }
};
template <> struct ALoad<A_BF16> {
    static constexpr bool ROW_FASTEST = false;
    static constexpr bool LINEAR = true;
    typedef uint4 Raw;
    LoadDesc d;
    __device__ __forceinline__ Raw raw_lin(uint32_t off) const { return *(const uint4*)((const uint16_t*)d.ptr + off); }
    __device__ __forceinline__ uint4 cvt(const Raw& r) const { return r; }
    __device__ __forceinline__ int row_of(int m) const { return m >= d.M ? -1 : (d.rowidx ? d.rowidx[m] : m); }
    __device__ __forceinline__ Raw raw_at(int r, int k0) const {
        if (r < 0 || k0 >= d.K) return make_uint4(0, 0, 0, 0);
        return *(const uint4*)((const uint16_t*)d.ptr + (long)r * d.ld + k0);
    }
    __device__ __forceinline__ Raw raw_unc(int r, int k0) const { return *(const uint4*)((const uint16_t*)d.ptr + (long)r * d.ld + k0); }
    __device__ __forceinline__ Raw raw(int m, int k0) const { return raw_at(row_of(m), k0); }
    __device__ __forceinline__ uint4 chunk(int m, int k0) const { return raw(m, k0); }
};
struct RawCS { uint4 v; float s; };
template <> struct ALoad<A_BF16_CS> {
    static constexpr bool ROW_FASTEST = false;
    static constexpr bool LINEAR = false;
    typedef RawCS Raw;
    LoadDesc d;
    __device__ __forceinline__ int row_of(int m) const { return m >= d.M ? -1 : m; }
    __device__ __forceinline__ Raw raw_unc(int r, int k0) const {
        const int b = fdiv(r, d.p0, d.mg0);
        Raw o = {*(const uint4*)((const uint16_t*)d.ptr + (long)r * d.ld + k0), d.aux0[b * d.p2 + (k0 >> 4)]};
        return o;
    }
    __device__ __forceinline__ Raw raw_at(int r, int k0) const {
        Raw z = {make_uint4(0, 0, 0, 0), 0.f};
        if (r < 0 || k0 >= d.K) return z;
        return raw_unc(r, k0);
    }
    __device__ __forceinline__ Raw raw(int m, int k0) const { return raw_at(row_of(m), k0); }
    __device__ __forceinline__ uint4 cvt(const Raw& r) const {
        float v[8];
        unpack8(r.v, v);
#pragma unroll
        for (int i = 0; i < 8; ++i) v[i] *= r.s;
        return pack8(v);
    }
    __device__ __forceinline__ uint4 chunk(int m, int k0) const { return cvt(raw(m, k0)); }
};
template <> struct ALoad<A_BF16_GELU> {
    static constexpr bool ROW_FASTEST = false;
    static constexpr bool LINEAR = true;
    __device__ __forceinline__ uint4 raw_lin(uint32_t off) const { return *(const uint4*)((const uint16_t*)d.ptr + off); }
    __device__ __forceinline__ int row_of(int m) const { return m >= d.M ? -1 : m; }
    __device__ __forceinline__ auto raw_at(int r, int k0) const { return raw(r < 0 ? d.M : r, k0); }
    typedef uint4 Raw;
    LoadDesc d;
    __device__ __forceinline__ Raw raw(int m, int k0) const {
        if (m >= d.M || k0 >= d.K) return make_uint4(0, 0, 0, 0);
        return *(const uint4*)((const uint16_t*)d.ptr + (long)m * d.ld + k0);
    }
    __device__ __forceinline__ Raw raw_unc(int r, int k0) const { return *(const uint4*)((const uint16_t*)d.ptr + (long)r * d.ld + k0); }
    const uint16_t* tab = nullptr;
    __device__ __forceinline__ uint4 cvt(const Raw& r) const {
        if (tab) {
            bool bad = false;
            const uint32_t o[4] = {gelu_tab_off2<2>(r.x, bad), gelu_tab_off2<2>(r.y, bad), gelu_tab_off2<2>(r.z, bad),
                                   gelu_tab_off2<2>(r.w, bad)};
            if (!__builtin_expect(__any((int)bad), 0)) {
                const unsigned char* tb = (const unsigned char*)tab;
                uint32_t q[4];
#pragma unroll
                for (int i = 0; i < 4; ++i)
                    q[i] = (uint32_t)*(const uint16_t*)(tb + (o[i] & 0xffffu)) | ((uint32_t)*(const uint16_t*)(tb + (o[i] >> 16)) << 16);
                return make_uint4(q[0], q[1], q[2], q[3]);
            }
        }
        float v[8];
        unpack8(r, v);
#pragma unroll
        for (int i = 0; i < 8; ++i) v[i] = gelu_f(v[i]);
        return pack8(v);
    }
    __device__ __forceinline__ uint4 chunk(int m, int k0) const { return cvt(raw(m, k0)); }
};
template <> struct ALoad<A_HEADS> {
    static constexpr bool ROW_FASTEST = false;
    static constexpr bool LINEAR = false;
    __device__ __forceinline__ int row_of(int m) const { return m >= d.M ? -1 : m; }
    __device__ __forceinline__ auto raw_at(int r, int k0) const { return raw(r < 0 ? d.M : r, k0); }
    typedef uint4 Raw;
    LoadDesc d;
    __device__ __forceinline__ uint4 cvt(const Raw& r) const { return r; }
    __device__ __forceinline__ Raw raw(int m, int k0) const { return chunk(m, k0); }
    __device__ __forceinline__ uint4 chunk(int m, int k0) const {
        if (m >= d.M || k0 >= d.K) return make_uint4(0, 0, 0, 0);
        return raw_unc(m, k0);
    }
    struct Split { int bw, t, part, hd, j; };
    __device__ __forceinline__ Split split(int m, int k0) const {
        const int h = d.p0, Lp = d.p2, DP = d.p3;
        const int bw = fdiv(m, Lp, d.mg0), t = m - bw * Lp;
        const int ph = d.p1 >= 0 ? (k0 >> d.p1) : fdiv(k0, DP, d.mg2), j = k0 - ph * DP;
        const int part = (h == 1) ? ph : fdiv(ph, h, d.mg1), hd = ph - part * h;
        return {bw, t, part, hd, j};
    }
    __device__ __forceinline__ uint4 raw_unc(int m, int k0) const {
        const int h = d.p0, Lp = d.p2, DP = d.p3, S = (int)d.ld;
        const Split s = split(m, k0);
        return *(const uint4*)((const uint16_t*)d.ptr + ((((long)s.bw * h + s.hd) * S + s.part) * Lp + s.t) * DP + s.j);
    }
    __device__ __forceinline__ uint32_t elem_off(const Split& s) const {
        return (uint32_t)((((s.bw * d.p0 + s.hd) * (int)d.ld + s.part) * d.p2 + s.t) * d.p3 + s.j);
    }
    __device__ __forceinline__ uint32_t elem_off(int m, int k0) const { return elem_off(split(m, k0)); }
    struct Step { uint32_t off0; int t0; };
    __device__ __forceinline__ Step step_base(int m, int k0) const {
        const Split s = split(m, k0);
        Step o = {elem_off(s), s.t};
        return o;
    }
    __device__ __forceinline__ uint32_t step_off(const Step& b, int i) const {
        const int Lp = d.p2, DP = d.p3;
        const uint32_t hop = (uint32_t)((d.p0 * (int)d.ld - 1) * Lp * DP);
        return b.off0 + (uint32_t)(16 * i * DP) + ((b.t0 + 16 * i >= Lp) ? hop : 0u);
    }
    __device__ __forceinline__ uint4 raw_lin(uint32_t off) const { return *(const uint4*)((const uint16_t*)d.ptr + off); }
};
template <> struct ALoad<A_PATCH> {
    static constexpr bool ROW_FASTEST = true;
    static constexpr bool LINEAR = false;
    __device__ __forceinline__ int row_of(int m) const { return m >= d.M ? -1 : m; }
    __device__ __forceinline__ auto raw_at(int r, int k0) const { return raw(r < 0 ? d.M : r, k0); }
    typedef RawF32 Raw;
    LoadDesc d;
    __device__ __forceinline__ Raw raw(int m, int k0) const {
        Raw z = {(f32x4){0.f, 0.f, 0.f, 0.f}, (f32x4){0.f, 0.f, 0.f, 0.f}};
        if (m >= d.M || k0 >= d.K) return z;
        return raw_unc(m, k0);
    }
    __device__ __forceinline__ Raw raw_unc(int m, int k0) const {
        const int Cin = d.p0, H = d.p1, W = d.p2, gw = W >> 2, gh = H >> 2;
        const int b = fdiv(m, gh * gw, d.mg0), ij = m - b * gh * gw, i = fdiv(ij, gw, d.mg1), j = ij - i * gw;
        const int cin = k0 >> 4, p = (k0 >> 2) & 3;
        const int Ct = d.p3 ? d.p3 : Cin;
        const float* src = (const float*)d.ptr + (((long)b * Ct + cin) * H + 4 * i + p) * W + 4 * j;
        Raw o = {*(const f32x4*)src, *(const f32x4*)(src + W)};
        if (d.aux0) {
            const float* s2 = d.aux0 + (((long)b * d.ld + cin) * H + 4 * i + p) * W + 4 * j;
            o.a += *(const f32x4*)s2;
            o.b += *(const f32x4*)(s2 + W);
        }
        return o;
    }
    __device__ __forceinline__ uint4 cvt(const Raw& r) const { return cvt_f32x8(r); }
    __device__ __forceinline__ uint4 chunk(int m, int k0) const { return cvt(raw(m, k0)); }
};
template <> struct ALoad<A_MERGE_LN> {
    static constexpr bool ROW_FASTEST = false;
    static constexpr bool LINEAR = false;
    __device__ __forceinline__ int row_of(int m) const { return m >= d.M ? -1 : m; }
    __device__ __forceinline__ auto raw_at(int r, int k0) const { return raw(r < 0 ? d.M : r, k0); }
    typedef uint4 Raw;
    LoadDesc d;
    __device__ __forceinline__ uint4 cvt(const Raw& r) const { return r; }
    __device__ __forceinline__ Raw raw(int m, int k0) const { return chunk(m, k0); }
    __device__ __forceinline__ uint4 chunk(int m, int k0) const {
        if (m >= d.M || k0 >= d.K) return make_uint4(0, 0, 0, 0);
        return raw_unc(m, k0);
    }
    __device__ __forceinline__ uint4 raw_unc(int m, int k0) const {
        const int H = d.p0, W = d.p1, C = d.p2, h2 = H >> 1, w2 = W >> 1;
        const int b = m / (h2 * w2), ij = m - b * h2 * w2, i = ij / w2, j = ij - i * w2;
        const float mu = d.aux0[m], rs = d.aux1[m];
        float v[8];
#pragma unroll
        for (int e = 0; e < 8; ++e) {
            const int k = k0 + e, blk = k / C, c = k - blk * C, wp = blk >> 1, hp = blk & 1;
            const float x = ((const float*)d.ptr)[(((long)b * H + 2 * i + hp) * W + 2 * j + wp) * C + c];
            v[e] = (x - mu) * rs * d.aux2[k] + d.aux3[k];
        }
        return pack8(v);
    }
};

template <int AK>
ALoad<AK> make_loader(const swv2_operand* o) {
    ALoad<AK> l;
    l.d.ptr = o->ptr; l.d.rowidx = o->rowidx; l.d.aux0 = o->aux0; l.d.aux1 = o->aux1; l.d.aux2 = o->aux2;
    l.d.aux3 = o->aux3; l.d.ld = o->ld; l.d.M = o->rows; l.d.K = o->cols;
    l.d.p0 = o->p[0]; l.d.p1 = o->p[1]; l.d.p2 = o->p[2]; l.d.p3 = o->p[3];
    l.d.mg0 = l.d.mg1 = l.d.mg2 = 0;
    if (AK == A_HEADS) {
        l.d.mg0 = fdiv_magic(o->p[2]); l.d.mg1 = fdiv_magic(o->p[0]);
        l.d.p1 = o->p[3] == 16 ? 4 : o->p[3] == 32 ? 5 : o->p[3] == 64 ? 6 : o->p[3] == 128 ? 7 : o->p[3] == 256 ? 8 : -1;
        l.d.mg2 = fdiv_magic(o->p[3]);
    }
    if (AK == A_PATCH) { l.d.mg0 = fdiv_magic((o->p[1] / 4) * (o->p[2] / 4)); l.d.mg1 = fdiv_magic(o->p[2] / 4); }
    if (AK == A_BF16_CS) l.d.mg0 = fdiv_magic(o->p[0]);
    return l;
}

int check_operand(const swv2_operand* o, const char* who) {
    SWV2_CHECK_ARG(o && o->ptr, "%s: null operand", who);
    SWV2_CHECK_ARG(o->rows > 0 && o->cols > 0, "%s: empty operand", who);
    SWV2_CHECK_ARG(o->cols % 8 == 0, "%s: operand width %d must be a multiple of 8", who, o->cols);
    SWV2_CHECK_ARG(((uintptr_t)o->ptr & 15) == 0, "%s: operand pointer must be 16-byte aligned", who);
    if (o->kind == SWV2_OP_F32 || o->kind == SWV2_OP_BF16 || o->kind == SWV2_OP_BF16_GELU || o->kind == SWV2_OP_BF16_CSCALE)
        SWV2_CHECK_ARG(o->ld % 8 == 0 && o->ld >= o->cols, "%s: row pitch %ld must be a multiple of 8 and >= cols", who, o->ld);
    if (o->kind == SWV2_OP_F32 || o->kind == SWV2_OP_BF16 || o->kind == SWV2_OP_BF16_GELU)
        SWV2_CHECK_ARG((double)o->rows * (double)o->ld < 4.29e9, "%s: row-major operands are indexed with 32-bit element offsets (%d x %ld too large)", who, o->rows, o->ld);
    if (o->kind == SWV2_OP_BF16_CSCALE)
        SWV2_CHECK_ARG(o->aux0 && o->p[0] > 0 && o->p[2] * 16 >= o->cols && o->cols % 16 == 0 && !o->rowidx,
                       "%s: scaled operand needs aux0, rows per sample p[0] > 0, p[2] >= cols / 16 groups, no gather", who);
    if (o->kind == SWV2_OP_HEADS)
        SWV2_CHECK_ARG(o->p[3] == 16 || o->p[3] == 32 || o->p[3] == 64 || o->p[3] == 96 || o->p[3] == 128 || o->p[3] == 256, "%s: head pad %d not in {16,32,64,96,128,256}", who, o->p[3]);
    if (o->kind == SWV2_OP_PATCH)
        SWV2_CHECK_ARG(o->p[1] % 4 == 0 && o->p[2] % 4 == 0 && o->cols == o->p[0] * 16, "%s: bad patch geometry", who);
    if (o->kind == SWV2_OP_MERGE_LN)
        SWV2_CHECK_ARG(o->aux0 && o->aux1 && o->aux2 && o->aux3 && o->cols == 4 * o->p[2], "%s: bad merge operand", who);
    return SWV2_OK;
}


}
```

swin_v2_weather_amd/csrc/proj_ln.hip:

```cpp
#include <cstdlib>
#include "gemm_common.h"
#include "ln_common.h"

namespace {

constexpr int PL_MAX_HDP = 128;

template <int ROWS, int COLS, int PITCH, int NT>
__device__ __forceinline__ void stage_weight(uint16_t* dst, const uint16_t* __restrict__ src, int rows, int cols, int tid) {
    typedef uint32_t u32x4 __attribute__((ext_vector_type(4)));
    constexpr int CPRW = COLS / 8, CHUNKS = ROWS * CPRW, PER = (CHUNKS + NT - 1) / NT, B = PER < 6 ? PER : 6;
#pragma unroll
    for (int j0 = 0; j0 < PER; j0 += B) {
        u32x4 v[B];
#pragma unroll
        for (int u = 0; u < B; ++u) {
            const int i = tid + (j0 + u) * NT, r = i / CPRW, c8 = i % CPRW;
            v[u] = *(const u32x4*)(src + (size_t)min(r, rows - 1) * cols + min(8 * c8, cols - 8));
        }
#pragma unroll
        for (int u = 0; u < B; ++u) {
            const int i = tid + (j0 + u) * NT, r = i / CPRW, c8 = i % CPRW;
            if (j0 + u < PER && r < rows && 8 * c8 < cols) *(u32x4*)(dst + r * PITCH + 8 * c8) = v[u];
        }
    }
}

struct ProjLnFwd {
    const uint16_t* oh; const uint16_t* wp; const float* bp; const float* gamma; const float* beta; const float* scale;
    const int32_t* rowidx; const float* x; uint16_t* a1; float* mean; float* rstd; float* y;
    int Mw, Lp, h, rows_per_sample; float eps;
};

template <int C, int MT, int HS = 16, int NW = 4>
__global__ __launch_bounds__(64 * NW, NW == 4 ? 2 : 1) void proj_ln_fwd_kernel(const ProjLnFwd a) {
    constexpr int NTC = C / 16, NT = 64 * NW;
    constexpr int HDPM = 8 * HS;
    constexpr int PWP = HDPM + 8, PA = C + 8;
    constexpr int EWAVE = 16 * PA * 2 + 16 * 2 * 4;
    constexpr int KSM = HDPM / 32;
    static_assert(C * PWP * 2 + NW * EWAVE + 3 * C * 4 <= 160 * 1024, "LDS budget");
    __shared__ __attribute__((aligned(16))) uint16_t Wps[C * PWP];
    __shared__ __attribute__((aligned(16))) unsigned char epi[NW * EWAVE];
    __shared__ __attribute__((aligned(16))) float cs[3 * C];
    typedef uint32_t u32x4 __attribute__((ext_vector_type(4)));

    const int tid = threadIdx.x, lane = tid & 63, wave = tid >> 6, fr = lane & 15, g = lane >> 4;
    const int hdp = a.h * HS, ksn = hdp / 32;
    const int row0 = blockIdx.x * (16 * NW * MT) + wave * (16 * MT);

    constexpr int UNITS = 16 * (C / 8), NP = (UNITS + 63) / 64;
    int dstv[MT][NP];
    f32x4 xr[MT][NP][2];
    float scv[MT][NP];
#pragma unroll
    for (int mt = 0; mt < MT; ++mt)
#pragma unroll
        for (int p = 0; p < NP; ++p) {
            const int u = min(lane + 64 * p, UNITS - 1), row = u / (C / 8);
            const int m = min(row0 + 16 * mt + row, a.Mw - 1);
            dstv[mt][p] = a.rowidx ? a.rowidx[m] : m;
        }
    bf16x8 xf[MT][KSM];
#pragma unroll
    for (int mt = 0; mt < MT; ++mt) {
        const int m = min(row0 + 16 * mt + fr, a.Mw - 1), w = m / a.Lp, t = m - w * a.Lp;
#pragma unroll
        for (int ks = 0; ks < KSM; ++ks) {
            const int k0 = 32 * ks + 8 * g, kc = min(k0, hdp - 8);
            xf[mt][ks] = *(const bf16x8*)(a.oh + (((size_t)w * a.h + kc / HS) * a.Lp + t) * HS + (kc & (HS - 1)));
        }
    }
    stage_weight<C, HDPM, PWP, NT>(Wps, a.wp, C, hdp, tid);
    for (int i = tid; i < C; i += NT) { cs[i] = a.bp[i]; cs[C + i] = a.gamma[i]; cs[2 * C + i] = a.beta[i]; }
#pragma unroll
    for (int mt = 0; mt < MT; ++mt)
#pragma unroll
        for (int p = 0; p < NP; ++p) {
            const int u = min(lane + 64 * p, UNITS - 1), c8 = u % (C / 8);
            const size_t off = (size_t)max(dstv[mt][p], 0) * C + 8 * c8;
            xr[mt][p][0] = *(const f32x4*)(a.x + off);
            xr[mt][p][1] = *(const f32x4*)(a.x + off + 4);
            scv[mt][p] = (a.scale ? a.scale : a.gamma)[a.scale ? max(dstv[mt][p], 0) / a.rows_per_sample : 0];
        }
    __syncthreads();

    f32x4 yacc[MT][NTC];
#pragma unroll
    for (int mt = 0; mt < MT; ++mt)
#pragma unroll
        for (int tn = 0; tn < NTC; ++tn) yacc[mt][tn] = (f32x4){0.f, 0.f, 0.f, 0.f};
#pragma unroll
    for (int ks = 0; ks < KSM; ++ks) {
        if (ks < ksn) {
#pragma unroll
            for (int tn = 0; tn < NTC; ++tn) {
                const bf16x8 wf = *(const bf16x8*)(Wps + (16 * tn + fr) * PWP + 32 * ks + 8 * g);
#pragma unroll
                for (int mt = 0; mt < MT; ++mt) yacc[mt][tn] = mfma32(wf, xf[mt][ks], yacc[mt][tn]);
            }
        }
    }

    uint16_t* As = (uint16_t*)(epi + wave * EWAVE);
    float* St = (float*)(As + 16 * PA);
#pragma unroll
    for (int mt = 0; mt < MT; ++mt) {
        float s = 0.f;
#pragma unroll
        for (int tn = 0; tn < NTC; ++tn) {
            const f32x4 bv = *(const f32x4*)(cs + 16 * tn + 4 * g);
            const bf16x4 ar = f2bf4(yacc[mt][tn] + bv);
            *(bf16x4*)(As + fr * PA + 16 * tn + 4 * g) = ar;
#pragma unroll
            for (int e = 0; e < 4; ++e) { yacc[mt][tn][e] = bf2f(ar[e]); s += yacc[mt][tn][e]; }
        }
        s = xor32_allsum(xor16_allsum(s));
        const float mu = s * (1.f / C);
        float q = 0.f;
#pragma unroll
        for (int tn = 0; tn < NTC; ++tn)
#pragma unroll
            for (int e = 0; e < 4; ++e) { const float d = yacc[mt][tn][e] - mu; q = fmaf(d, d, q); }
        q = xor32_allsum(xor16_allsum(q));
        const float rs = rsqrtf(q * (1.f / C) + a.eps);
        if (g == 0) {
            const int m = min(row0 + 16 * mt + fr, a.Mw - 1);
            a.mean[m] = mu;
            a.rstd[m] = rs;
            St[2 * fr] = mu;
            St[2 * fr + 1] = rs;
        }
        __syncthreads();
#pragma unroll
        for (int p = 0; p < NP; ++p) {
            const int u = lane + 64 * p, row = u / (C / 8), c8 = u % (C / 8);
            if (UNITS % 64 == 0 || u < UNITS) {
                const int m = min(row0 + 16 * mt + row, a.Mw - 1);
                const u32x4 av = *(const u32x4*)(As + row * PA + 8 * c8);
                *(u32x4*)(a.a1 + (size_t)m * C + 8 * c8) = av;
                const int dst = dstv[mt][p];
                if (dst >= 0) {
                    const float mu_r = St[2 * row], rs_r = St[2 * row + 1];
                    const float sc = a.scale ? scv[mt][p] : 1.f;
                    const size_t off = (size_t)dst * C + 8 * c8;
                    float v[8];
                    unpack8(__builtin_bit_cast(uint4, av), v);
#pragma unroll
                    for (int hlf = 0; hlf < 2; ++hlf) {
                        const f32x4 gm = *(const f32x4*)(cs + C + 8 * c8 + 4 * hlf), bt = *(const f32x4*)(cs + 2 * C + 8 * c8 + 4 * hlf);
                        f32x4 o = xr[mt][p][hlf];
#pragma unroll
                        for (int e = 0; e < 4; ++e) o[e] += sc * ((v[4 * hlf + e] - mu_r) * rs_r * gm[e] + bt[e]);
                        *(f32x4*)(a.y + off + 4 * hlf) = o;
                    }
                }
            }
        }
        if (mt + 1 < MT) __syncthreads();
    }
}

struct ProjLnBwd {
    const float* dy; const uint16_t* a1; const float* mean; const float* rstd; const float* gamma; const float* scale;
    const int32_t* rowidx; const uint16_t* wpt; uint16_t* da1; uint16_t* doh; float* ws;
    int Mw, Lp, h, rows_per_sample;
};

template <int C, int MT, int HS = 16, int NW = 4>
__global__ __launch_bounds__(64 * NW, NW == 4 ? 2 : 1) void proj_ln_bwd_kernel(const ProjLnBwd a) {
    constexpr int KS = C / 32, NT = 64 * NW, HDPM = 8 * HS;
    constexpr int ROWS = 16 * NW * MT, PX = C + 8, PW = C + 8;
    typedef LnBwdShape<C, NT, ROWS> Sh;
    constexpr int LPR = Sh::LPR, RPP = Sh::RPP, NPASS = Sh::NPASS, BATCH = Sh::BATCH;
    constexpr bool TWO_ROUNDS = NW == 8;
    constexpr int GROWS = TWO_ROUNDS ? RPP / 2 : RPP;
    static_assert(HDPM * PW * 2 + ROWS * PX * 2 + GROWS * 2 * C * 4 <= 160 * 1024, "LDS budget");
    __shared__ __attribute__((aligned(16))) uint16_t Wts[HDPM * PW];
    __shared__ __attribute__((aligned(16))) uint16_t Xs[ROWS * PX];
    __shared__ __attribute__((aligned(16))) float gs[GROWS * 2 * C];
    typedef uint32_t u32x4 __attribute__((ext_vector_type(4)));
    typedef uint32_t u32x2 __attribute__((ext_vector_type(2)));

    const int tid = threadIdx.x, lane = tid & 63, wave = tid >> 6, fr = lane & 15, g = lane >> 4;
    const int hdp = a.h * HS;
    const int wg_row0 = blockIdx.x * ROWS;

    stage_weight<HDPM, C, PW, NT>(Wts, a.wpt, hdp, C, tid);
    {
        const int lr = tid % LPR, rg = tid / LPR;
        const bool act = 4 * lr < C;
        const int c0 = act ? 4 * lr : 0;
        const f32x4 gm = *(const f32x4*)(a.gamma + c0);
        f32x4 dgm = {0.f, 0.f, 0.f, 0.f}, dbt = {0.f, 0.f, 0.f, 0.f};
        int srcv[NPASS];
#pragma unroll
        for (int i = 0; i < NPASS; ++i) {
            const int m = min(wg_row0 + i * RPP + rg, a.Mw - 1);
            srcv[i] = a.rowidx ? a.rowidx[m] : m;
        }
        f32x4 d4s[2][BATCH];
        u32x2 a4s[2][BATCH];
        float mus[2][BATCH], rss[2][BATCH], scs[2][BATCH];
        int oks[2][BATCH];
        const float* scp = a.scale ? a.scale : a.gamma;
        auto load_batch = [&](int pb, auto set_c) {
            constexpr int S = decltype(set_c)::value;
#pragma unroll
            for (int i = 0; i < BATCH; ++i) {
                const int m = min(wg_row0 + (pb + i) * RPP + rg, a.Mw - 1);
                const int src = srcv[(pb + i) % NPASS];
                oks[S][i] = src >= 0;
                const int sr = max(src, 0);
                d4s[S][i] = *(const f32x4*)(a.dy + (size_t)sr * C + c0);
                a4s[S][i] = *(const u32x2*)(a.a1 + (size_t)m * C + c0);
                mus[S][i] = a.mean[m];
                rss[S][i] = a.rstd[m];
                scs[S][i] = scp[a.scale ? sr / a.rows_per_sample : 0];
            }
        };
        load_batch(0, std::integral_constant<int, 0>{});
#pragma unroll
        for (int pb = 0; pb < NPASS; pb += BATCH) {
            constexpr int dummy = 0; (void)dummy;
            const int cur = (pb / BATCH) & 1;
            if (pb + BATCH < NPASS) {
                if (cur == 0) load_batch(pb + BATCH, std::integral_constant<int, 1>{});
                else load_batch(pb + BATCH, std::integral_constant<int, 0>{});
            }
            f32x4 d4[BATCH];
            u32x2 a4[BATCH];
            float mu[BATCH], rs[BATCH], sc[BATCH];
            int ok[BATCH];
#pragma unroll
            for (int i = 0; i < BATCH; ++i) {
                d4[i] = d4s[cur][i]; a4[i] = a4s[cur][i]; mu[i] = mus[cur][i]; rs[i] = rss[cur][i];
                sc[i] = a.scale ? scs[cur][i] : 1.f; ok[i] = oks[cur][i];
            }
#pragma unroll
            for (int i = 0; i < BATCH; ++i) {
                const int row = (pb + i) * RPP + rg;
                const bool live = act && ok[i];
                const float once = (live && wg_row0 + row < a.Mw) ? 1.f : 0.f;
                const float av[4] = {__uint_as_float(a4[i][0] << 16), __uint_as_float(a4[i][0] & 0xffff0000u),
                                     __uint_as_float(a4[i][1] << 16), __uint_as_float(a4[i][1] & 0xffff0000u)};
                float gg[4], xh[4], t1 = 0.f, t2 = 0.f;
#pragma unroll
                for (int e = 0; e < 4; ++e) {
                    const float d = live ? sc[i] * d4[i][e] : 0.f;
                    xh[e] = (av[e] - mu[i]) * rs[i];
                    gg[e] = d * gm[e];
                    dgm[e] = fmaf(once * d, xh[e], dgm[e]);
                    dbt[e] = fmaf(once, d, dbt[e]);
                    t1 += gg[e];
                    t2 = fmaf(gg[e], xh[e], t2);
                }
                t1 = group_allsum<LPR>(t1); t2 = group_allsum<LPR>(t2);
                t1 *= (1.f / C); t2 *= (1.f / C);
                f32x4 o4;
#pragma unroll
                for (int e = 0; e < 4; ++e) o4[e] = ok[i] ? rs[i] * (gg[e] - t1 - xh[e] * t2) : 0.f;
                const bf16x4 ob = f2bf4(o4);
                if (act) {
                    *(bf16x4*)(a.da1 + (size_t)min(wg_row0 + row, a.Mw - 1) * C + c0) = ob;
                    *(bf16x4*)(Xs + row * PX + c0) = ob;
                }
            }
        }
        if constexpr (TWO_ROUNDS) {
            if (act && rg >= GROWS) {
                *(f32x4*)(gs + ((rg - GROWS) * 2 + 0) * C + c0) = dgm;
                *(f32x4*)(gs + ((rg - GROWS) * 2 + 1) * C + c0) = dbt;
            }
            __syncthreads();
            if (act && rg < GROWS) {
                dgm += *(const f32x4*)(gs + (rg * 2 + 0) * C + c0);
                dbt += *(const f32x4*)(gs + (rg * 2 + 1) * C + c0);
            }
            __syncthreads();
        }
        if (act && rg < GROWS) {
            *(f32x4*)(gs + (rg * 2 + 0) * C + c0) = dgm;
            *(f32x4*)(gs + (rg * 2 + 1) * C + c0) = dbt;
        }
        __syncthreads();
        for (int i = tid; i < 2 * C; i += NT) {
            float t = 0.f;
#pragma unroll
            for (int r = 0; r < GROWS; ++r) t += gs[r * 2 * C + i];
            a.ws[(size_t)blockIdx.x * 2 * C + i] = t;
        }
    }
#pragma unroll
    for (int mt = 0; mt < MT; ++mt) {
        bf16x8 xf[KS];
#pragma unroll
        for (int ks = 0; ks < KS; ++ks) xf[ks] = *(const bf16x8*)(Xs + (wave * 16 * MT + 16 * mt + fr) * PX + 32 * ks + 8 * g);
        const int m = min(wg_row0 + wave * 16 * MT + 16 * mt + fr, a.Mw - 1), w = m / a.Lp, t = m - w * a.Lp;
        for (int kt = 0; kt < a.h * (HS / 16); ++kt) {
            f32x4 acc = {0.f, 0.f, 0.f, 0.f};
#pragma unroll
            for (int ks = 0; ks < KS; ++ks) {
                const bf16x8 wf = *(const bf16x8*)(Wts + (16 * kt + fr) * PW + 32 * ks + 8 * g);
                acc = mfma32(wf, xf[ks], acc);
            }
            *(bf16x4*)(a.doh + (((size_t)w * a.h + kt / (HS / 16)) * a.Lp + t) * HS + 16 * (kt % (HS / 16)) + 4 * g) = f2bf4(acc);
        }
    }
}

}

extern "C" int swv2_proj_ln_supported(int C, int heads, int head_pad) {
    if (C == 192) return head_pad == 32 && heads >= 1 && heads <= 8;
    return (C == 32 || C == 64 || C == 96 || C == 128) && head_pad == 16 && heads >= 2 && heads % 2 == 0 && heads * 16 <= PL_MAX_HDP;
}

extern "C" size_t swv2_proj_ln_bwd_ws_floats(int Mw, int C) { return (Mw > 0 && C > 0) ? (size_t)cdiv(Mw, 64) * 2 * C : 0; }

extern "C" int swv2_proj_ln_fwd(const swv2_proj_ln_args* a, void* stream) {
    SWV2_CHECK_ARG(a && a->oh && a->wp && a->bp && a->gamma && a->beta && a->x && a->a1 && a->mean && a->rstd && a->y,
                   "swv2_proj_ln_fwd: null pointer");
    SWV2_CHECK_ARG(a->Bw > 0 && a->Lp > 0 && a->Lp % 16 == 0 && a->rows_per_sample > 0, "swv2_proj_ln_fwd: bad geometry");
    if (!swv2_proj_ln_supported(a->C, a->heads, a->C == 192 ? 32 : 16)) {
        swv2_set_error("swv2_proj_ln_fwd: C=%d heads=%d not instantiated; use swv2_linear + swv2_ln_residual_fwd", a->C, a->heads);
        return SWV2_ERR_UNSUPPORTED;
    }
    const int Mw = a->Bw * a->Lp;
    ProjLnFwd k = {(const uint16_t*)a->oh, (const uint16_t*)a->wp, a->bp, a->gamma, a->beta, a->scale, a->rowidx, a->x,
                   (uint16_t*)a->a1, a->mean, a->rstd, a->y, Mw, a->Lp, a->heads, a->rows_per_sample, a->eps};
    hipStream_t st = (hipStream_t)stream;
    const bool mt2 = Mw >= 128 * 256;
#define PL_CASE(CC)                                                                                                  \
    case CC:                                                                                                         \
        if (mt2) hipLaunchKernelGGL((proj_ln_fwd_kernel<CC, 2>), dim3(cdiv(Mw, 128)), dim3(256), 0, st, k);          \
        else hipLaunchKernelGGL((proj_ln_fwd_kernel<CC, 1>), dim3(cdiv(Mw, 64)), dim3(256), 0, st, k);               \
        break;
    switch (a->C) {
        PL_CASE(32) PL_CASE(64) PL_CASE(96) PL_CASE(128)
        case 192: hipLaunchKernelGGL((proj_ln_fwd_kernel<192, 1, 32, 8>), dim3(cdiv(Mw, 128)), dim3(512), 0, st, k); break;
    }
#undef PL_CASE
    SWV2_CHECK_LAUNCH("swv2_proj_ln_fwd");
    return SWV2_OK;
}

extern "C" int swv2_proj_ln_bwd(const swv2_proj_ln_bwd_args* a, void* stream) { return swv2_proj_ln_bwd_impl(a, stream, nullptr); }

int swv2_proj_ln_bwd_impl(const swv2_proj_ln_bwd_args* a, void* stream, int* deferred) {
    SWV2_CHECK_ARG(a && a->dy && a->a1 && a->mean && a->rstd && a->gamma && a->wpt && a->da1 && a->doh && a->dgamma && a->dbeta &&
                       a->ws, "swv2_proj_ln_bwd: null pointer");
    SWV2_CHECK_ARG(a->Bw > 0 && a->Lp > 0 && a->Lp % 16 == 0 && a->rows_per_sample > 0, "swv2_proj_ln_bwd: bad geometry");
    if (!swv2_proj_ln_supported(a->C, a->heads, a->C == 192 ? 32 : 16)) {
        swv2_set_error("swv2_proj_ln_bwd: C=%d heads=%d not instantiated; use swv2_ln_residual_bwd + swv2_linear", a->C, a->heads);
        return SWV2_ERR_UNSUPPORTED;
    }
    const int Mw = a->Bw * a->Lp;
    ProjLnBwd k = {a->dy, (const uint16_t*)a->a1, a->mean, a->rstd, a->gamma, a->scale, a->rowidx, (const uint16_t*)a->wpt,
                   (uint16_t*)a->da1, (uint16_t*)a->doh, a->ws, Mw, a->Lp, a->heads, a->rows_per_sample};
    hipStream_t st = (hipStream_t)stream;
    const bool mt2 = Mw >= 128 * 256;
#define PL_CASE(CC)                                                                                                  \
    case CC:                                                                                                         \
        if (mt2) hipLaunchKernelGGL((proj_ln_bwd_kernel<CC, 2>), dim3(cdiv(Mw, 128)), dim3(256), 0, st, k);          \
        else hipLaunchKernelGGL((proj_ln_bwd_kernel<CC, 1>), dim3(cdiv(Mw, 64)), dim3(256), 0, st, k);               \
        break;
    int nblk = cdiv(Mw, mt2 ? 128 : 64);
    switch (a->C) {
        PL_CASE(32) PL_CASE(64) PL_CASE(96) PL_CASE(128)
        case 192: nblk = cdiv(Mw, 128); hipLaunchKernelGGL((proj_ln_bwd_kernel<192, 1, 32, 8>), dim3(nblk), dim3(512), 0, st, k); break;
    }
#undef PL_CASE
    if (deferred) *deferred = nblk;
    else swv2_launch_ln_partials_reduce(a->ws, a->dgamma, a->dbeta, nblk, a->C, st);
    SWV2_CHECK_LAUNCH("swv2_proj_ln_bwd");
    return SWV2_OK;
}
```

swin_v2_weather_amd/ops.py:

```python
from __future__ import annotations

import ctypes as C
import functools
from typing import Optional

import torch

from . import _lib as L

BF16 = torch.bfloat16


def _p(t: Optional[torch.Tensor]):
    return None if t is None else t.data_ptr()


def _stream():
    return torch.cuda.current_stream().cuda_stream


_TIMED = None


_EVERY = 1
# ... 273 lines not shown
    a.doh, a.rnorm, a.dqkvh, a.dlogit_scale, a.dbias = _p(doh), _p(rnorm), _p(dqkvh), _p(dlogit), _p(dbias)
    a.Bw, a.heads, a.L, a.head_dim, a.nwh, a.nww, a.mask_thr, a.max_chunks = Bw, heads, Lwin, head_dim, nwh, nww, mask_thr, max_chunks
    if dbias_ws is not None:
        a.dbias_ws, a.dbias_ws_bytes = _p(dbias_ws), dbias_ws.numel() * dbias_ws.element_size()
    return a


def attn_pack_bias(bias: torch.Tensor) -> torch.Tensor:
    heads, Lw = bias.shape[0], bias.shape[1]
    out = torch.empty(L.load().swv2_attn_pack_bias_bytes(heads, Lw), dtype=torch.uint8, device=bias.device)
    L.check(L.load().swv2_attn_pack_bias(_p(bias), heads, Lw, _p(out), _stream()), "swv2_attn_pack_bias")
    return out


def attn_fwd(a: L.AttnArgs):
    L.check(_timed("attn_fwd", L.load().swv2_attn_fwd, C.byref(a), _stream()), "swv2_attn_fwd")


def attn_bwd(a: L.AttnArgs):
    L.check(_timed("attn_bwd", L.load().swv2_attn_bwd, C.byref(a), _stream()), "swv2_attn_bwd")


def batch_sum(inp: torch.Tensor, out: torch.Tensor, accumulate=False):
    B = inp.shape[0]
    n = inp[0].numel()
    L.check(L.load().swv2_batch_sum(_p(inp), _p(out), B, n, int(accumulate), _stream()), "swv2_batch_sum")


def merge_stats(x, mean, rstd, eps=1e-5):
    B, H, W, Cc = x.shape
    L.check(L.load().swv2_merge_stats(_p(x), _p(mean), _p(rstd), B, H, W, Cc, eps, _stream()), "swv2_merge_stats")


def merge_ln_bwd(x, dn, gamma, mean, rstd, dx, dgamma, dbeta):
    B, H, W, Cc = x.shape
    L.check(L.load().swv2_merge_ln_bwd(_p(x), _p(dn), _p(gamma), _p(mean), _p(rstd), _p(dx), _p(dgamma), _p(dbeta),
                                       B, H, W, Cc, _stream()), "swv2_merge_ln_bwd")


def loss_sums(prd, tar, qw, sums):
    B, Cc, H, W = prd.shape
    L.check(L.load().swv2_loss_sums(_p(prd), _p(tar), _p(qw), _p(sums), B * Cc, H, W, _stream()), "swv2_loss_sums")


def loss_finalize(sums, chw, absolute: bool, squared: bool, loss, coef):
    layers = sums.shape[0] if sums.dim() == 4 else 1
    BC, Cc = sums.shape[-3] * sums.shape[-2], chw.numel()
    L.check(L.load().swv2_loss_finalize(_p(sums), layers, _p(chw), BC, Cc, int(absolute), int(squared), _p(loss), _p(coef), _stream()),
            "swv2_loss_finalize")


def loss_part_reduce(part, M, T, B, Cout, coff, sums):
    L.check(L.load().swv2_loss_part_reduce(_p(part), M, T, B, Cout, sums.shape[2], coff, _p(sums), _stream()), "swv2_loss_part_reduce")


def loss_resid_to_image(resid, coef, out, Cout: int, add=None):
    _chk(resid, BF16, "loss residual"); _chk(coef, torch.float32, "coef"); _chk(out, torch.float32, "out")
    B, Cs, H, W = out.shape
    if resid.shape[1] != L.loss_resid_pitch(Cout * 16):
        raise L.Swv2Error(f"loss_resid_to_image: residual rows of {resid.shape[1]} elements, expected the padded pitch {L.loss_resid_pitch(Cout * 16)}")
    if add is not None:
        _chk(add, torch.float32, "add")
    L.check(L.load().swv2_loss_resid_to_image(_p(resid), _p(coef), _p(add), _p(out), B, Cout, H, W, Cs, add.shape[1] if add is not None else 0,
                                              _stream()), "swv2_loss_resid_to_image")


def loss_finalize_sums(sums, chw, absolute: bool, squared: bool):
    B, Cc = sums.shape[-3:-1]
    buf = torch.empty(B * Cc + 1, dtype=torch.float32, device=sums.device)
    coef, loss = buf[:B * Cc].view(B, Cc), buf[B * Cc:]
    loss_finalize(sums, chw, absolute, squared, loss, coef)
    return loss, coef


def loss_grad(prd, tar, qw, coef, dprd):
    B, Cc, H, W = prd.shape
    L.check(L.load().swv2_loss_grad(_p(prd), _p(tar), _p(qw), _p(coef), _p(dprd), B * Cc, H, W, _stream()), "swv2_loss_grad")


def score_slices(planes: int, H: int, W: int) -> int:
    return int(L.load().swv2_score_slices(planes, H, W))


def score_workspace(planes: int, H: int, W: int, device) -> torch.Tensor:
    return torch.empty(int(L.load().swv2_score_ws_bytes(planes, H, W)) // 4, dtype=torch.float32, device=device)


def _planes_in_place(t: torch.Tensor, lead: int) -> bool:
    if not (t.is_cuda and t.dtype == torch.float32 and t.dim() == lead + 3 and t.numel() > 0):
        return False
    B, (Cc, H, W), bs = t.shape[lead - 1], t.shape[lead:], t.stride(lead - 1)
    return tuple(t.stride()[lead:]) == (H * W, W, 1) and t.data_ptr() % 16 == 0 and (B == 1 or (bs % 4 == 0 and bs >= Cc * H * W))


def score_planes_ok(t: torch.Tensor) -> bool:
    return _planes_in_place(t, 1) and t.shape[3] % 4 == 0


def score_sums(prd, tar, w, ws, clim=None):
    if not (score_planes_ok(prd) and score_planes_ok(tar)) or prd.shape != tar.shape:
        raise L.Swv2Error(f"score_sums: expected two CUDA fp32 [B, C, H, W] tensors of one shape with contiguous planes and W % 4 == 0, got "
                          f"{tuple(prd.shape)} {prd.dtype} strides {prd.stride()} / {tuple(tar.shape)} {tar.dtype} strides {tar.stride()}")
    B, Cc, H, W = prd.shape
    _chk(w, torch.float32, "row weights"); _chk(ws, torch.float32, "score workspace")
    if w.numel() != H:
        raise L.Swv2Error(f"score_sums: {w.numel()} row weights for {H} rows")
    if clim is not None and (_chk(clim, torch.float32, "climatology").shape != (Cc, H, W)):
        raise L.Swv2Error(f"score_sums: climatology {tuple(clim.shape)}, expected {(Cc, H, W)}")
    L.check(L.load().swv2_score_sums(_p(prd), prd.stride(0) if B > 1 else Cc * H * W, _p(tar), tar.stride(0) if B > 1 else Cc * H * W,
                                     _p(clim), _p(w), B, Cc, H, W, _p(ws), ws.numel() * 4, _stream()), "swv2_score_sums")


def score_finalize(ws, B: int, Cc: int, H: int, W: int, scale=None):
    _chk(ws, torch.float32, "score workspace")
    if scale is not None and _chk(scale, torch.float32, "scale").numel() != Cc:
        raise L.Swv2Error(f"score_finalize: scale of {scale.numel()} values for {Cc} channels")
    n = B * Cc
    buf = torch.empty(6 * n + 2 * Cc, dtype=torch.float32, device=ws.device)
    sums, rmse, acc = buf[:4 * n].view(B, Cc, 4), buf[4 * n:5 * n].view(B, Cc), buf[5 * n:6 * n].view(B, Cc)
    rmse_mean, acc_mean = buf[6 * n:6 * n + Cc], buf[6 * n + Cc:]
    L.check(L.load().swv2_score_finalize(_p(ws), ws.numel() * 4, B, Cc, H, W, _p(scale), _p(sums), _p(rmse), _p(acc), _p(rmse_mean),
                                         _p(acc_mean), _stream()), "swv2_score_finalize")
    return sums, rmse, acc, rmse_mean, acc_mean


def forecast_scores(prd, tar, w, clim=None, scale=None, ws=None):
    B, Cc, H, W = prd.shape
    if ws is None:
        ws = score_workspace(B * Cc, H, W, prd.device)
    score_sums(prd, tar, w, ws, clim)
    return score_finalize(ws, B, Cc, H, W, scale)


ENS_MAX_MEMBERS = 64


def ens_workspace(planes: int, H: int, W: int, M: int, device) -> torch.Tensor:
    n = int(L.load().swv2_ens_ws_bytes(planes, H, W, M))
    if n == 0:
        raise L.Swv2Error(f"ens_workspace: planes {planes}, H {H}, W {W} must be positive and M = {M} within 2 .. {ENS_MAX_MEMBERS}")
    return torch.empty(n // 4, dtype=torch.float32, device=device)


def ens_members_ok(t: torch.Tensor) -> bool:
    return _planes_in_place(t, 2) and 2 <= t.shape[0] <= ENS_MAX_MEMBERS and t.shape[4] % 4 == 0 and t.stride(0) % 4 == 0


def ens_sums(ens, tar, w, ws):
    if not (ens_members_ok(ens) and score_planes_ok(tar)) or ens.shape[1:] != tar.shape or ens.device != tar.device:
        raise L.Swv2Error(f"ens_sums: expected CUDA fp32 members [M, B, C, H, W] (2 <= M <= {ENS_MAX_MEMBERS}) and truth [B, C, H, W] with contiguous "
                          f"planes and W % 4 == 0, got {tuple(ens.shape)} {ens.dtype} strides {ens.stride()} / {tuple(tar.shape)} {tar.dtype} "
                          f"strides {tar.stride()}")
    M, B, Cc, H, W = ens.shape
    _chk(w, torch.float32, "row weights"); _chk(ws, torch.float32, "ensemble workspace")
    if w.numel() != H:
        raise L.Swv2Error(f"ens_sums: {w.numel()} row weights for {H} rows")
    span = Cc * H * W
    L.check(L.load().swv2_ens_sums(_p(ens), ens.stride(0), ens.stride(1) if B > 1 else span, _p(tar), tar.stride(0) if B > 1 else span, _p(w),
                                   M, B, Cc, H, W, _p(ws), ws.numel() * 4, _stream()), "swv2_ens_sums")


def ens_finalize(ws, M: int, B: int, Cc: int, H: int, W: int, scale=None):
    _chk(ws, torch.float32, "ensemble workspace")
    if scale is not None and _chk(scale, torch.float32, "scale").numel() != Cc:
        raise L.Swv2Error(f"ens_finalize: scale of {scale.numel()} values for {Cc} channels")
    n = B * Cc
    buf = torch.empty(8 * n + 4 * Cc, dtype=torch.float32, device=ws.device)
    hist = torch.empty(B, Cc, M + 1, dtype=torch.int32, device=ws.device)
    sums = buf[:4 * n].view(B, Cc, 4)
    er, sp, cr, fc = (buf[(4 + k) * n:(5 + k) * n].view(B, Cc) for k in range(4))
    means = buf[8 * n:].view(4, Cc)
    L.check(L.load().swv2_ens_finalize(_p(ws), ws.numel() * 4, M, B, Cc, H, W, _p(scale), _p(sums), _p(hist), _p(er), _p(sp), _p(cr), _p(fc),
                                       _p(means), _stream()), "swv2_ens_finalize")
    return sums, hist, er, sp, cr, fc, means


QUANTILE_MAX_RANKS = 256


def quantile_workspace(planes: int, H: int, W: int, K: int, device) -> torch.Tensor:
    return torch.empty(int(L.load().swv2_quantile_ws_bytes(planes, H, W, K)) // 4, dtype=torch.int32, device=device)


def quantile_planes_ok(t: torch.Tensor) -> bool:
    return _planes_in_place(t, 1) and (t.shape[2] * t.shape[3]) % 4 == 0 and t.shape[2] * t.shape[3] < 2 ** 30


def plane_order_stats(x, ranks, ws=None):
    if not quantile_planes_ok(x):
        raise L.Swv2Error(f"plane_order_stats: expected a CUDA fp32 [B, C, H, W] tensor with contiguous planes and H * W % 4 == 0, got "
                          f"{tuple(x.shape)} {x.dtype} strides {x.stride()}")
    B, Cc, H, W = x.shape
    _chk(ranks, torch.int32, "ranks")
    K = ranks.numel()
    if ranks.dim() != 1 or ranks.device != x.device:
        raise L.Swv2Error(f"plane_order_stats: ranks {tuple(ranks.shape)} on {ranks.device}, expected [K] on {x.device}")
    if ws is None:
        ws = quantile_workspace(B * Cc, H, W, K, x.device)
    _chk(ws, torch.int32, "quantile workspace")
    out = torch.empty(K, B, Cc, dtype=torch.float32, device=x.device)
    nan_count = torch.empty(B, Cc, dtype=torch.int32, device=x.device)
    L.check(L.load().swv2_plane_order_stats(_p(x), x.stride(0) if B > 1 else Cc * H * W, B, Cc, H, W, _p(ranks), K, _p(out), _p(nan_count),
                                            _p(ws), ws.numel() * 4, _stream()), "swv2_plane_order_stats")
    return out, nan_count


def stats_slices(Cc: int, H: int, W: int) -> int:
    return int(L.load().swv2_stats_slices(Cc, H, W))


def stats_workspace(Cc: int, H: int, W: int, device) -> torch.Tensor:
    return torch.empty(int(L.load().swv2_stats_ws_bytes(Cc, H, W)) // 8, dtype=torch.float64, device=device).view(Cc, -1, 6)


def stats_accumulate(slab, prev, pivot, tsum, part, first: bool, stream=None):
    _chk(slab, torch.float32, "stats slab"); _chk(pivot, torch.float64, "stats pivot")
    _chk(tsum, torch.float64, "stats tsum"); _chk(part, torch.float64, "stats workspace")
    if slab.dim() != 3 or tsum.shape != slab.shape or pivot.numel() != slab.shape[0]:
        raise L.Swv2Error(f"stats_accumulate: slab {tuple(slab.shape)}, tsum {tuple(tsum.shape)}, pivot {tuple(pivot.shape)}: expected "
                          "[C, H, W], [C, H, W], [C]")
    if prev is not None and _chk(prev, torch.float32, "stats prev").shape != slab.shape:
        raise L.Swv2Error(f"stats_accumulate: prev {tuple(prev.shape)}, slab {tuple(slab.shape)}")
    Cc, H, W = slab.shape
    L.check(L.load().swv2_stats_accumulate(_p(slab), _p(prev), _p(pivot), _p(tsum), _p(part), part.numel() * 8, Cc, H, W, int(bool(first)),
                                           stream if stream is not None else _stream()), "swv2_stats_accumulate")


def stats_finalize(part, tsum, pivot, T: int, stream=None):
    _chk(part, torch.float64, "stats workspace"); _chk(tsum, torch.float64, "stats tsum"); _chk(pivot, torch.float64, "stats pivot")
    if tsum.dim() != 3 or pivot.numel() != tsum.shape[0]:
        raise L.Swv2Error(f"stats_finalize: tsum {tuple(tsum.shape)}, pivot {tuple(pivot.shape)}: expected [C, H, W], [C]")
    Cc, H, W = tsum.shape
    folded = torch.empty(Cc, 6, dtype=torch.float64, device=tsum.device)
    time_means = torch.empty(Cc, H, W, dtype=torch.float32, device=tsum.device)
    L.check(L.load().swv2_stats_finalize(_p(part), part.numel() * 8, _p(tsum), _p(pivot), Cc, H, W, int(T), _p(folded), _p(time_means),
                                         stream if stream is not None else _stream()), "swv2_stats_finalize")
    return folded, time_means


def era5_select_normalize(raw, out, chan, mean, std, coff=0, stream=None):
    B, S, Craw, Hraw, Wraw = raw.shape
    _, Ct, H, W = out.shape
    _chk(raw, torch.float32, "era5 raw"); _chk(out, torch.float32, "era5 out")
    L.check(L.load().swv2_era5_select_normalize(_p(raw), _p(out), _p(chan), _p(mean), _p(std), B, S, chan.numel(), Craw, Hraw, Wraw,
                                                H, W, Ct, coff, stream if stream is not None else _stream()), "swv2_era5_select_normalize")


def era5_zenith(out, sun, coff, stream=None):
    B, Ct, H, W = out.shape
    _chk(sun, torch.float32, "era5_zenith sun")
    if sun.dim() != 3 or sun.shape[0] != B or sun.shape[2] != 3:
        raise L.Swv2Error(f"era5_zenith: sun must be [B, nz, 3], got {tuple(sun.shape)}")
    L.check(L.load().swv2_era5_zenith(_p(out), _p(sun), B, sun.shape[1], H, W, Ct, coff,
                                      stream if stream is not None else _stream()), "swv2_era5_zenith")


def era5_static(stat, out, coff, stream=None):
    B, Ct, H, W = out.shape
    L.check(L.load().swv2_era5_static(_p(stat), _p(out), B, stat.shape[0], H, W, Ct, coff,
                                      stream if stream is not None else _stream()), "swv2_era5_static")


def adam_step(p, g, m, v, lr, beta1, beta2, eps, step, grad_inv_scale=1.0):
    L.check(L.load().swv2_adam_step(_p(p), _p(g), _p(m), _p(v), p.numel(), lr, beta1, beta2, eps, step, grad_inv_scale,
                                    _stream()), "swv2_adam_step")


def mlp_fwd(x, w1, b1, w2, b2, gamma, beta, scale, rows_per_sample, eps=1e-5, keep_hpre=True, out=None):
    M, Cc = x.shape
    hid = w1.shape[0]
    _chk(x, torch.float32, "mlp x"); _chk(w1, BF16, "mlp w1"); _chk(w2, BF16, "mlp w2")
    dev = x.device
    if out is None:
        out = (torch.empty(M, Cc, dtype=torch.float32, device=dev), torch.empty(M, hid, dtype=BF16, device=dev) if keep_hpre else None,
               torch.empty(M, Cc, dtype=BF16, device=dev), torch.empty(M, device=dev), torch.empty(M, device=dev))
    y, hpre, a2, mean, rstd = out
    a = L.MlpArgs()
    a.x, a.w1, a.b1, a.w2, a.b2, a.gamma, a.beta, a.scale = (_p(t) for t in (x, w1, b1, w2, b2, gamma, beta, scale))
    a.hpre, a.a2, a.mean, a.rstd, a.y = (_p(t) for t in (hpre, a2, mean, rstd, y))
    a.M, a.C, a.hidden, a.rows_per_sample, a.eps = M, Cc, hid, rows_per_sample, eps
    L.check(_timed("mlp_fwd", L.load().swv2_mlp_fwd, C.byref(a), _stream()), "swv2_mlp_fwd")
    return y, hpre, a2, mean, rstd


def mlp_bwd(dy, a2, mean, rstd, gamma, scale, hpre, w2t, w1t, dgamma, dbeta, rows_per_sample, x=None, w1=None, b1=None, out=None, ws=None):
    M, Cc = dy.shape
    hid = w2t.shape[0]
    dev = dy.device
    if out is None:
        out = (torch.empty(M, Cc, dtype=torch.float32, device=dev), torch.empty(M, Cc, dtype=BF16, device=dev),
               torch.empty(M, hid, dtype=BF16, device=dev))
    if ws is None:
        ws = torch.empty(L.load().swv2_mlp_bwd_ws_floats(M, Cc), dtype=torch.float32, device=dev)
    dx, da2, dh = out
    a = L.MlpBwdArgs()
    a.dy, a.a2, a.mean, a.rstd, a.gamma, a.scale, a.hpre, a.w2t, a.w1t = (_p(t) for t in (dy, a2, mean, rstd, gamma, scale, hpre, w2t, w1t))
    a.da2, a.dh, a.dx, a.dgamma, a.dbeta, a.ws = (_p(t) for t in (da2, dh, dx, dgamma, dbeta, ws))
    a.M, a.C, a.hidden, a.rows_per_sample = M, Cc, hid, rows_per_sample
    a.x, a.w1, a.b1 = _p(x), _p(w1), _p(b1)
    L.check(_timed("mlp_bwd", L.load().swv2_mlp_bwd, C.byref(a), _stream()), "swv2_mlp_bwd")
    return dx, da2, dh


def proj_ln_fwd(oh, wp, bp, gamma, beta, scale, rowidx, x, Bw, Lp, heads, rows_per_sample, eps=1e-5, out=None):
    Cc, Mw = wp.shape[0], Bw * Lp
    _chk(oh, BF16, "proj_ln oh"); _chk(wp, BF16, "proj_ln wp"); _chk(x, torch.float32, "proj_ln x")
    dev = x.device
    if out is None:
        out = (torch.empty_like(x), torch.empty(Mw, Cc, dtype=BF16, device=dev), torch.empty(Mw, device=dev), torch.empty(Mw, device=dev))
    y, a1, mean, rstd = out
    a = L.ProjLnArgs()
    a.oh, a.wp, a.bp, a.gamma, a.beta, a.scale, a.rowidx, a.x = (_p(t) for t in (oh, wp, bp, gamma, beta, scale, rowidx, x))
    a.a1, a.mean, a.rstd, a.y = (_p(t) for t in (a1, mean, rstd, y))
    a.Bw, a.Lp, a.heads, a.C, a.rows_per_sample, a.eps = Bw, Lp, heads, Cc, rows_per_sample, eps
    L.check(_timed("proj_ln_fwd", L.load().swv2_proj_ln_fwd, C.byref(a), _stream()), "swv2_proj_ln_fwd")
    return y, a1, mean, rstd


def proj_ln_bwd(dy, a1, mean, rstd, gamma, scale, rowidx, wpt, dgamma, dbeta, Bw, Lp, heads, rows_per_sample, out=None, ws=None):
    Cc, Mw = wpt.shape[1], Bw * Lp
    _chk(dy, torch.float32, "proj_ln dy"); _chk(a1, BF16, "proj_ln a1"); _chk(wpt, BF16, "proj_ln wpt")
    dev = dy.device
    if out is None:
        out = (torch.empty(Mw, Cc, dtype=BF16, device=dev), torch.empty(Bw, heads, Lp, wpt.shape[0] // max(heads, 1), dtype=BF16, device=dev))
    if ws is None:
        ws = torch.empty(L.load().swv2_proj_ln_bwd_ws_floats(Mw, Cc), dtype=torch.float32, device=dev)
    da1, doh = out
    a = L.ProjLnBwdArgs()
    a.dy, a.a1, a.mean, a.rstd, a.gamma, a.scale, a.rowidx, a.wpt = (_p(t) for t in (dy, a1, mean, rstd, gamma, scale, rowidx, wpt))
    a.da1, a.doh, a.dgamma, a.dbeta, a.ws = (_p(t) for t in (da1, doh, dgamma, dbeta, ws))
    a.Bw, a.Lp, a.heads, a.C, a.rows_per_sample = Bw, Lp, heads, Cc, rows_per_sample
    L.check(_timed("proj_ln_bwd", L.load().swv2_proj_ln_bwd, C.byref(a), _stream()), "swv2_proj_ln_bwd")
    return da1, doh


def cpb_fwd(w1, b1, w2, b2, keep, bias, wh, ww, heads, hidden, drop_p):
    L.check(L.load().swv2_cpb_fwd(_p(w1), _p(b1), _p(w2), _p(b2), _p(keep), _p(bias), wh, ww, heads, hidden, drop_p, _stream()),
            "swv2_cpb_fwd")


_SCRATCH = {}


def _scratch(nbytes: int, device, tag: str) -> torch.Tensor:
    key = (device.index if device.index is not None else torch.cuda.current_device(), tag, _stream())
    t = _SCRATCH.get(key)
    if t is None or t.numel() < nbytes:
        t = _SCRATCH[key] = torch.empty(max(int(nbytes), 1), dtype=torch.uint8, device=device)
    return t


def cpb_bwd(dbias, w1, b1, w2, keep, dw1, db1, dw2, db2, wh, ww, heads, hidden, drop_p, atomics=False):
    lib = L.load()
    if atomics:
        L.check(lib.swv2_cpb_bwd(_p(dbias), _p(w1), _p(b1), _p(w2), _p(keep), _p(dw1), _p(db1), _p(dw2), _p(db2), wh, ww,
                                 heads, hidden, drop_p, _stream()), "swv2_cpb_bwd")
        return
    nb = lib.swv2_cpb_bwd_ws_bytes(wh, ww, heads, hidden)
    ws = _scratch(nb, dbias.device, "cpb_bwd")
    L.check(lib.swv2_cpb_bwd_ws(_p(dbias), _p(w1), _p(b1), _p(w2), _p(keep), _p(dw1), _p(db1), _p(dw2), _p(db2), wh, ww,
                                heads, hidden, drop_p, _p(ws), nb, _stream()), "swv2_cpb_bwd_ws")


def cpb_multi_supported(heads: int, hidden: int, drop_p: float) -> bool:
    return 0 < heads <= 16 and hidden in (64, 128, 256, 384, 512) and abs(drop_p - 0.125) < 1e-6


def cpb_fwd_multi(ptab, nblk, keep_bits, bias_all, wh, ww, heads, hidden, drop_p):
    _chk(bias_all, torch.float32, "cpb_fwd_multi bias")
    if keep_bits is not None:
        _chk(keep_bits, torch.int32, "cpb_fwd_multi keep_bits")
    L.check(L.load().swv2_cpb_fwd_multi(_p(ptab), nblk, _p(keep_bits), _p(bias_all), wh, ww, heads, hidden, drop_p, _stream()),
            "swv2_cpb_fwd_multi")


def cpb_bwd_multi(dtables, nchunk, ptab, nblk, keep_bits, grads, wh, ww, heads, hidden, drop_p):
    lib = L.load()
    _chk(dtables, torch.float32, "cpb_bwd_multi tables"); _chk(grads, torch.float32, "cpb_bwd_multi grads")
    nb = lib.swv2_cpb_bwd_multi_ws_bytes(nblk, wh, ww, heads, hidden)
    ws = _scratch(nb, grads.device, "cpb_bwd_multi")
    L.check(lib.swv2_cpb_bwd_multi(_p(dtables), nchunk, _p(ptab), nblk, _p(keep_bits), _p(grads), wh, ww, heads, hidden, drop_p,
                                   _p(ws), nb, _stream()), "swv2_cpb_bwd_multi")


def attn_pack_bias_multi(bias_all: torch.Tensor) -> torch.Tensor:
    _chk(bias_all, torch.float32, "attn_pack_bias_multi")
    ntab, heads, Lw = bias_all.shape[0], bias_all.shape[1], bias_all.shape[2]
    nb = L.load().swv2_attn_pack_bias_bytes(heads, Lw)
    out = torch.empty(ntab, nb, dtype=torch.uint8, device=bias_all.device)
    L.check(L.load().swv2_attn_pack_bias_multi(_p(bias_all), ntab, heads, Lw, _p(out), _stream()), "swv2_attn_pack_bias_multi")
    return out


class WindowPlan:

    def __init__(self, B, gh, gw, wh, ww, sh, sw, heads, head_dim, device):
        self.B, self.gh, self.gw, self.wh, self.ww, self.sh, self.sw = B, gh, gw, wh, ww, sh, sw
        self.heads, self.d = heads, head_dim
        self.L = wh * ww
        self.Lp, self.DP = attn_geometry(self.L, head_dim)
        self.nwh, self.nww = gh // wh, gw // ww
        self.nW = self.nwh * self.nww
        self.Bw = B * self.nW
        self.T = gh * gw
        if gh % wh or gw % ww:
            raise L.Swv2Error(f"window {wh}x{ww} does not divide the patch grid {gh}x{gw}")
        self.mask_thr = (wh - sh) * ww if sh > 0 else 0
        wi = torch.arange(self.nwh).view(-1, 1, 1, 1)
        wj = torch.arange(self.nww).view(1, -1, 1, 1)
        r = torch.arange(wh).view(1, 1, -1, 1)
        c = torch.arange(ww).view(1, 1, 1, -1)
        src = (((wi * wh + r + sh) % gh) * gw + (wj * ww + c + sw) % gw).reshape(self.nW, self.L)
        tab = torch.full((B, self.nW, self.Lp), -1, dtype=torch.int64)
        tab[:, :, :self.L] = src.unsqueeze(0) + (torch.arange(B) * self.T).view(B, 1, 1)
        self.rowidx = tab.reshape(-1).to(torch.int32).to(device)
        Cc = heads * head_dim
        j = torch.arange(self.DP)
        hd = torch.arange(heads).view(-1, 1)
        one = torch.where(j.view(1, -1) < head_dim, hd * head_dim + j.view(1, -1), torch.full((1, 1), -1)).reshape(-1)
        self.proj_map = one.to(torch.int32).to(device)
        three = torch.cat([torch.where(one >= 0, one + part * Cc, one) for part in range(3)])
        self.qkv_map = three.to(torch.int32).to(device)


@functools.lru_cache(maxsize=64)
def window_plan(B, gh, gw, wh, ww, sh, sw, heads, head_dim, device_index) -> WindowPlan:
    return WindowPlan(B, gh, gw, wh, ww, sh, sw, heads, head_dim, torch.device("cuda", device_index))
```

Before: 225.2.

## Skip padded window rows in QKV GEMM and proj+LN kernels

Adds a RealRows mapping so the fused QKV GEMM and the proj+LayerNorm backward kernels loop only over real tokens per window (L) rather than padded rows (Lp). The padded rows get zero-filled explicitly in the QKV epilogue. The goal is to stop spending GEMM and LN work on padding rows. Each row index now costs an extra magic-number division, and the kernel variants are new. Forward proj_ln is still passed L=0, so only its backward and the QKV path use the compacted rows.

```diff
diff --git a/include/swv2.h b/include/swv2.h
--- a/include/swv2.h
+++ b/include/swv2.h
@@ -20,6 +20,7 @@
 const char* swv2_last_error(void);
 
 int swv2_attn_geometry(int L, int head_dim, int* Lp, int* DP);
+int swv2_real_row(int mc, int L, int Lp);
 
 int swv2_attn_fwd_regime(int L, int head_dim, int has_bias, int dbg);
 
@@ -307,6 +308,7 @@
     float* y;
     int Bw, Lp, heads, C, rows_per_sample;
     float eps;
+    int L;
 } swv2_proj_ln_args;
 typedef struct {
     const float* dy;
@@ -317,9 +319,11 @@
     void* doh;
     float* dgamma; float* dbeta; float* ws;
     int Bw, Lp, heads, C, rows_per_sample;
+    int L;
 } swv2_proj_ln_bwd_args;
 int swv2_proj_ln_supported(int C, int heads, int head_pad);
 size_t swv2_proj_ln_bwd_ws_floats(int Mw, int C);
+int swv2_proj_ln_workgroups(int Bw, int Lp, int L, int C);
 int swv2_proj_ln_fwd(const swv2_proj_ln_args* a, void* stream);
 int swv2_proj_ln_bwd(const swv2_proj_ln_bwd_args* a, void* stream);
 
diff --git a/swin_v2_weather_amd/_lib.py b/swin_v2_weather_amd/_lib.py
--- a/swin_v2_weather_amd/_lib.py
+++ b/swin_v2_weather_amd/_lib.py
@@ -110,12 +110,12 @@
 
 class ProjLnArgs(C.Structure):
     _fields_ = [(n, C.c_void_p) for n in ("oh", "wp", "bp", "gamma", "beta", "scale", "rowidx", "x", "a1", "mean", "rstd", "y")] + \
-               [(n, C.c_int) for n in ("Bw", "Lp", "heads", "C", "rows_per_sample")] + [("eps", C.c_float)]
+               [(n, C.c_int) for n in ("Bw", "Lp", "heads", "C", "rows_per_sample")] + [("eps", C.c_float), ("L", C.c_int)]
 
 
 class ProjLnBwdArgs(C.Structure):
     _fields_ = [(n, C.c_void_p) for n in ("dy", "a1", "mean", "rstd", "gamma", "scale", "rowidx", "wpt", "da1", "doh", "dgamma", "dbeta",
-                                           "ws")] + [(n, C.c_int) for n in ("Bw", "Lp", "heads", "C", "rows_per_sample")]
+                                           "ws")] + [(n, C.c_int) for n in ("Bw", "Lp", "heads", "C", "rows_per_sample", "L")]
 
 
 class MlpArgs(C.Structure):
@@ -264,6 +264,8 @@
     "swv2_era5_static": (_I, [_P, _P, _I, _I, _I, _I, _I, _I, _P]),
     "swv2_proj_ln_supported": (_I, [_I, _I, _I]),
     "swv2_proj_ln_bwd_ws_floats": (C.c_size_t, [_I, _I]),
+    "swv2_proj_ln_workgroups": (_I, [_I, _I, _I, _I]),
+    "swv2_real_row": (_I, [_I, _I, _I]),
     "swv2_proj_ln_fwd": (_I, [C.POINTER(ProjLnArgs), _P]),
     "swv2_proj_ln_bwd": (_I, [C.POINTER(ProjLnBwdArgs), _P]),
     "swv2_mlp_supported": (_I, [_I, _I]),
diff --git a/swin_v2_weather_amd/csrc/block.hip b/swin_v2_weather_amd/csrc/block.hip
--- a/swin_v2_weather_amd/csrc/block.hip
+++ b/swin_v2_weather_amd/csrc/block.hip
@@ -164,6 +164,7 @@
         m.oh = d->oh; m.wp = d->w_proj; m.bp = d->proj_b; m.gamma = d->n1_w; m.beta = d->n1_b; m.scale = d->dp1; m.rowidx = d->rowidx;
         m.x = d->x; m.a1 = d->a1; m.mean = d->mean1; m.rstd = d->rstd1; m.y = d->x1; m.Bw = Bw; m.Lp = d->Lp; m.heads = h; m.C = C;
         m.rows_per_sample = d->T; m.eps = 1e-5f;
+        m.L = 0;
         LAUNCH(SWV2_STEP_PROJ_LN_FWD, swv2_proj_ln_fwd(&m, st));
     } break;
     case SWV2_STEP_PROJ: {
@@ -247,7 +248,7 @@
         swv2_proj_ln_bwd_args m = {};
         m.dy = d->dx1; m.a1 = d->a1; m.mean = d->mean1; m.rstd = d->rstd1; m.gamma = d->n1_w; m.scale = d->dp1; m.rowidx = d->rowidx;
         m.wpt = d->w_projt; m.da1 = d->da1; m.doh = d->doh; m.dgamma = d->d_n1_w; m.dbeta = d->d_n1_b; m.ws = ln1_ws;
-        m.Bw = Bw; m.Lp = d->Lp; m.heads = h; m.C = C; m.rows_per_sample = d->T;
+        m.Bw = Bw; m.Lp = d->Lp; m.heads = h; m.C = C; m.rows_per_sample = d->T; m.L = d->L;
         LAUNCH(SWV2_STEP_PROJ_LN_BWD, swv2_proj_ln_bwd_impl(&m, st, p.ln_deferred ? &n_ln1 : nullptr));
     } break;
     case SWV2_STEP_LN1_BWD: {
diff --git a/swin_v2_weather_amd/csrc/gemm.hip b/swin_v2_weather_amd/csrc/gemm.hip
--- a/swin_v2_weather_amd/csrc/gemm.hip
+++ b/swin_v2_weather_amd/csrc/gemm.hip
@@ -964,8 +964,8 @@
 #include "stamps.h"
 __device__ __forceinline__ int swzk(int r, int kc, int K) { return r * K + ((kc ^ ((r >> 1) & 7)) << 3); }
 
-template <int AK, int EK, int N, int K, int BMT, int HS = 16>
-__global__ __launch_bounds__(512) void gemm_rw_kernel(ALoad<AK> al, const uint16_t* __restrict__ Wb, Epi<EK> ep, int M) {
+template <int AK, int EK, int N, int K, int BMT, int HS = 16, bool RR = false>
+__global__ __launch_bounds__(512) void gemm_rw_kernel(ALoad<AK> al, const uint16_t* __restrict__ Wb, Epi<EK> ep, int M, RealRows rr) {
     constexpr int NTH = 512, KC = K / 8;
     constexpr int ACH = BMT * KC / NTH;
     constexpr int RT = BMT / 64;
@@ -1007,13 +1007,14 @@
             const int c = tid + i * NTH, m = t * BMT + crow(c);
             const bool in = (t < ntiles) && (m < M);
             ain |= (uint32_t)in << i;
-            if constexpr (AK == A_F32) arow[i] = al.d.rowidx[min(m, M - 1)];
-            else arow[i] = min(m, M - 1);
+            const int mp = RR ? rr_row(rr, min(m, M - 1)) : min(m, M - 1);
+            if constexpr (AK == A_F32) arow[i] = al.d.rowidx[mp];
+            else arow[i] = mp;
         }
         if constexpr (EK == E_F32) {
             const int m = t * BMT + wr * 16 + (lane >> 2);
             ein = (t < ntiles) && (m < M);
-            erow_res = ein ? ep.d.rowidx[m] : -1;
+            erow_res = ein ? ep.d.rowidx[RR ? rr_row(rr, m) : m] : -1;
         }
     };
     auto issue = [&]() {
@@ -1092,10 +1093,10 @@
                     const EpiDesc& d = ep.d;
                     const int h = d.p0, Lp = d.p2, L = d.p4;
                     const int r = lane & 15, slot = lane >> 4, nb = n0 + slot * 16, m = m0 + r;
-                    if (m < d.M) {
+                    if (m < M) {
                         const int ph = HS == 16 ? nb >> 4 : nb >> 5, lp = (h == 1) ? ph : fdiv(ph, h, d.mg1), hd = ph - lp * h;
                         const int part = lp + d.p1;
-                        const int bw = fdiv(m, Lp, d.mg0), tt = m - bw * Lp;
+                        const int bw = RR ? rr_window(rr, m) : fdiv(m, Lp, d.mg0), tt = m - bw * (RR ? rr.L : Lp);
                         const bool valid = tt < L;
                         float v[16];
                         float ss = 0.f;
@@ -1135,6 +1136,25 @@
                     ep.tile(st, m0, n0, lane);
                 }
             }
+        if constexpr (EK == E_QKV_HEADS && RR) {
+            {
+                const EpiDesc& d = ep.d;
+                const int h = d.p0, Lp = d.p2;
+                const int w0 = rr_window(rr, t * BMT), w1 = rr_window(rr, min((t + 1) * BMT, M));
+                constexpr int RUNS = N / HS;
+                const int cq = rr.pad * (HS / 8);
+                for (int i = tid; i < (w1 - w0) * RUNS * cq; i += NTH) {
+                    const int q = i / cq, c = i - q * cq, w = w0 + q / RUNS, ph = q % RUNS;
+                    const int lp = (h == 1) ? ph : fdiv(ph, h, d.mg1), hd = ph - lp * h, part = lp + d.p1;
+                    *(uint4*)((uint16_t*)d.out + ((((long)w * h + hd) * 3 + part) * Lp + rr.L) * HS + 8 * c) = make_uint4(0, 0, 0, 0);
+                }
+                for (int i = tid; i < (w1 - w0) * RUNS * rr.pad; i += NTH) {
+                    const int q = i / rr.pad, c = i - q * rr.pad, w = w0 + q / RUNS, ph = q % RUNS;
+                    const int lp = (h == 1) ? ph : fdiv(ph, h, d.mg1), hd = ph - lp * h, part = lp + d.p1;
+                    if (part < 2) d.aux_out[(((long)w * h + hd) * 2 + part) * Lp + rr.L + c] = 0.f;
+                }
+            }
+        }
         STAMP(6);
         __syncthreads();
         STAMP(7);
@@ -1234,12 +1254,16 @@
     const Epi<EK> ep = make_epi<EK>(e, M, N);
     const uint16_t* wb = (const uint16_t*)w;
     const LinearKernel kern = linear_kernel_for(AK, EK, a, e, N, swv2_gemm_wide());
+    const int rw_Lp = qkv_pair(AK, EK) ? e->p[2] : 0, rw_L = qkv_pair(AK, EK) ? e->p[4] : 0;
+    const RealRows rr = real_rows(rw_Lp > 0 && M % rw_Lp == 0 ? rw_L : 0, rw_Lp > 0 ? rw_Lp : 1);
+    const int Mr = rr.pad ? M / rw_Lp * rr.L : M;
     switch (kern) {
         case LinearKernel::RESIDENT_QKV128:
             if constexpr (qkv_pair(AK, EK)) {
                 Epi<EK> ep1 = ep;
                 ep1.d.p1 = 0;
-                hipLaunchKernelGGL((gemm_rw_kernel<AK, EK, 384, 128, 128>), dim3(256), dim3(512), 0, st, make_loader<AK>(a), wb, ep1, M);
+                if (rr.pad) hipLaunchKernelGGL((gemm_rw_kernel<AK, EK, 384, 128, 128, 16, true>), dim3(256), dim3(512), 0, st, make_loader<AK>(a), wb, ep1, Mr, rr);
+                else hipLaunchKernelGGL((gemm_rw_kernel<AK, EK, 384, 128, 128>), dim3(256), dim3(512), 0, st, make_loader<AK>(a), wb, ep1, M, rr);
             }
             break;
         case LinearKernel::RESIDENT_QKV192X3:
@@ -1249,14 +1273,16 @@
                     ep2.d.N = 256;
                     ep2.d.p1 = part;
                     ep2.d.bias = e->bias ? e->bias + 256 * part : nullptr;
-                    hipLaunchKernelGGL((gemm_rw_kernel<AK, EK, 256, 192, 128, 32>), dim3(256), dim3(512), 0, st, make_loader<AK>(a),
-                                       wb + (size_t)part * 256 * 192, ep2, M);
+                    if (rr.pad) hipLaunchKernelGGL((gemm_rw_kernel<AK, EK, 256, 192, 128, 32, true>), dim3(256), dim3(512), 0, st, make_loader<AK>(a),
+                                                   wb + (size_t)part * 256 * 192, ep2, Mr, rr);
+                    else hipLaunchKernelGGL((gemm_rw_kernel<AK, EK, 256, 192, 128, 32>), dim3(256), dim3(512), 0, st, make_loader<AK>(a),
+                                            wb + (size_t)part * 256 * 192, ep2, M, rr);
                 }
             }
             break;
         case LinearKernel::RESIDENT_DX128:
             if constexpr (dx_pair(AK, EK))
-                hipLaunchKernelGGL((gemm_rw_kernel<AK, EK, 128, 384, 64>), dim3(256), dim3(512), 0, st, make_loader<AK>(a), wb, ep, M);
+                hipLaunchKernelGGL((gemm_rw_kernel<AK, EK, 128, 384, 64>), dim3(256), dim3(512), 0, st, make_loader<AK>(a), wb, ep, M, rr);
             break;
         case LinearKernel::WIDE_DMA:
         case LinearKernel::WIDE:
diff --git a/swin_v2_weather_amd/csrc/gemm_common.h b/swin_v2_weather_amd/csrc/gemm_common.h
--- a/swin_v2_weather_amd/csrc/gemm_common.h
+++ b/swin_v2_weather_amd/csrc/gemm_common.h
@@ -33,6 +33,25 @@
     return q - (q * d > n);
 }
 static inline uint32_t fdiv_magic(int d) { return d > 1 ? (uint32_t)((0x100000000ull + (uint64_t)d - 1) / (uint64_t)d) : 0u; }
+
+struct RealRows {
+    int L, pad;
+    uint32_t mg;
+};
+static inline RealRows real_rows(int L, int Lp) {
+    const int l = (L > 0 && L < Lp) ? L : Lp;
+    const RealRows r = {l, Lp - l, fdiv_magic(l)};
+    return r;
+}
+__host__ __device__ __forceinline__ int rr_window(const RealRows& r, int mc) {
+#ifdef __HIP_DEVICE_COMPILE__
+    return r.L == 1 ? mc : fdiv(mc, r.L, r.mg);
+#else
+    const int q = (int)(((uint64_t)(uint32_t)mc * r.mg) >> 32);
+    return r.L == 1 ? mc : q - (q * r.L > mc);
+#endif
+}
+__host__ __device__ __forceinline__ int rr_row(const RealRows& r, int mc) { return mc + rr_window(r, mc) * r.pad; }
 
 __device__ __forceinline__ float gelu_f(float x) {
     float e, gs;
@@ -327,7 +346,7 @@
         SWV2_CHECK_ARG(o->aux0 && o->p[0] > 0 && o->p[2] * 16 >= o->cols && o->cols % 16 == 0 && !o->rowidx,
                        "%s: scaled operand needs aux0, rows per sample p[0] > 0, p[2] >= cols / 16 groups, no gather", who);
     if (o->kind == SWV2_OP_HEADS)
-        SWV2_CHECK_ARG(o->p[3] == 16 || o->p[3] == 32 || o->p[3] == 64 || o->p[3] == 96 || o->p[3] == 128 || o->p[3] == 256, "%s: head pad %d not in {16,32,64,96,128,256}", who, o->p[3]);
+        SWV2_CHECK_ARG(o->p[3] == 16|| o->p[3] == 32 || o->p[3] == 64 || o->p[3] == 96 || o->p[3] == 128 || o->p[3] == 256, "%s: head pad %d not in {16,32,64,96,128,256}", who, o->p[3]);
     if (o->kind == SWV2_OP_PATCH)
         SWV2_CHECK_ARG(o->p[1] % 4 == 0 && o->p[2] % 4 == 0 && o->cols == o->p[0] * 16, "%s: bad patch geometry", who);
     if (o->kind == SWV2_OP_MERGE_LN)
diff --git a/swin_v2_weather_amd/csrc/proj_ln.hip b/swin_v2_weather_amd/csrc/proj_ln.hip
--- a/swin_v2_weather_amd/csrc/proj_ln.hip
+++ b/swin_v2_weather_amd/csrc/proj_ln.hip
@@ -29,10 +29,11 @@
 struct ProjLnFwd {
     const uint16_t* oh; const uint16_t* wp; const float* bp; const float* gamma; const float* beta; const float* scale;
     const int32_t* rowidx; const float* x; uint16_t* a1; float* mean; float* rstd; float* y;
-    int Mw, Lp, h, rows_per_sample; float eps;
+    int Mc, Lp, h, rows_per_sample; float eps;
+    RealRows rr;
 };
 
-template <int C, int MT, int HS = 16, int NW = 4>
+template <int C, int MT, int HS = 16, int NW = 4, bool RR = false>
 __global__ __launch_bounds__(64 * NW, NW == 4 ? 2 : 1) void proj_ln_fwd_kernel(const ProjLnFwd a) {
     constexpr int NTC = C / 16, NT = 64 * NW;
     constexpr int HDPM = 8 * HS;
@@ -48,6 +49,7 @@
     const int tid = threadIdx.x, lane = tid & 63, wave = tid >> 6, fr = lane & 15, g = lane >> 4;
     const int hdp = a.h * HS, ksn = hdp / 32;
     const int row0 = blockIdx.x * (16 * NW * MT) + wave * (16 * MT);
+    auto prow = [&](int mc) { if constexpr (RR) return rr_row(a.rr, mc); else return mc; };
 
     constexpr int UNITS = 16 * (C / 8), NP = (UNITS + 63) / 64;
     int dstv[MT][NP];
@@ -58,13 +60,13 @@
 #pragma unroll
         for (int p = 0; p < NP; ++p) {
             const int u = min(lane + 64 * p, UNITS - 1), row = u / (C / 8);
-            const int m = min(row0 + 16 * mt + row, a.Mw - 1);
+            const int m = prow(min(row0 + 16 * mt + row, a.Mc - 1));
             dstv[mt][p] = a.rowidx ? a.rowidx[m] : m;
         }
     bf16x8 xf[MT][KSM];
 #pragma unroll
     for (int mt = 0; mt < MT; ++mt) {
-        const int m = min(row0 + 16 * mt + fr, a.Mw - 1), w = m / a.Lp, t = m - w * a.Lp;
+        const int mc = min(row0 + 16 * mt + fr, a.Mc - 1), w = RR ? rr_window(a.rr, mc) : mc / a.Lp, t = mc - w * (RR ? a.rr.L : a.Lp);
 #pragma unroll
         for (int ks = 0; ks < KSM; ++ks) {
             const int k0 = 32 * ks + 8 * g, kc = min(k0, hdp - 8);
@@ -125,7 +127,7 @@
         q = xor32_allsum(xor16_allsum(q));
         const float rs = rsqrtf(q * (1.f / C) + a.eps);
         if (g == 0) {
-            const int m = min(row0 + 16 * mt + fr, a.Mw - 1);
+            const int m = prow(min(row0 + 16 * mt + fr, a.Mc - 1));
             a.mean[m] = mu;
             a.rstd[m] = rs;
             St[2 * fr] = mu;
@@ -136,7 +138,7 @@
         for (int p = 0; p < NP; ++p) {
             const int u = lane + 64 * p, row = u / (C / 8), c8 = u % (C / 8);
             if (UNITS % 64 == 0 || u < UNITS) {
-                const int m = min(row0 + 16 * mt + row, a.Mw - 1);
+                const int m = prow(min(row0 + 16 * mt + row, a.Mc - 1));
                 const u32x4 av = *(const u32x4*)(As + row * PA + 8 * c8);
                 *(u32x4*)(a.a1 + (size_t)m * C + 8 * c8) = av;
                 const int dst = dstv[mt][p];
@@ -164,10 +166,11 @@
 struct ProjLnBwd {
     const float* dy; const uint16_t* a1; const float* mean; const float* rstd; const float* gamma; const float* scale;
     const int32_t* rowidx; const uint16_t* wpt; uint16_t* da1; uint16_t* doh; float* ws;
-    int Mw, Lp, h, rows_per_sample;
+    int Mc, Lp, h, rows_per_sample;
+    RealRows rr;
 };
 
-template <int C, int MT, int HS = 16, int NW = 4>
+template <int C, int MT, int HS = 16, int NW = 4, bool RR = false>
 __global__ __launch_bounds__(64 * NW, NW == 4 ? 2 : 1) void proj_ln_bwd_kernel(const ProjLnBwd a) {
     constexpr int KS = C / 32, NT = 64 * NW, HDPM = 8 * HS;
     constexpr int ROWS = 16 * NW * MT, PX = C + 8, PW = C + 8;
@@ -185,9 +188,11 @@
     const int tid = threadIdx.x, lane = tid & 63, wave = tid >> 6, fr = lane & 15, g = lane >> 4;
     const int hdp = a.h * HS;
     const int wg_row0 = blockIdx.x * ROWS;
+    auto prow = [&](int mc) { if constexpr (RR) return rr_row(a.rr, mc); else return mc; };
 
     stage_weight<HDPM, C, PW, NT>(Wts, a.wpt, hdp, C, tid);
     {
+#pragma clang fp contract(off)
         const int lr = tid % LPR, rg = tid / LPR;
         const bool act = 4 * lr < C;
         const int c0 = act ? 4 * lr : 0;
@@ -196,7 +201,7 @@
         int srcv[NPASS];
 #pragma unroll
         for (int i = 0; i < NPASS; ++i) {
-            const int m = min(wg_row0 + i * RPP + rg, a.Mw - 1);
+            const int m = prow(min(wg_row0 + i * RPP + rg, a.Mc - 1));
             srcv[i] = a.rowidx ? a.rowidx[m] : m;
         }
         f32x4 d4s[2][BATCH];
@@ -208,7 +213,7 @@
             constexpr int S = decltype(set_c)::value;
 #pragma unroll
             for (int i = 0; i < BATCH; ++i) {
-                const int m = min(wg_row0 + (pb + i) * RPP + rg, a.Mw - 1);
+                const int m = prow(min(wg_row0 + (pb + i) * RPP + rg, a.Mc - 1));
                 const int src = srcv[(pb + i) % NPASS];
                 oks[S][i] = src >= 0;
                 const int sr = max(src, 0);
@@ -241,7 +246,7 @@
             for (int i = 0; i < BATCH; ++i) {
                 const int row = (pb + i) * RPP + rg;
                 const bool live = act && ok[i];
-                const float once = (live && wg_row0 + row < a.Mw) ? 1.f : 0.f;
+                const float once = (live && wg_row0 + row < a.Mc) ? 1.f : 0.f;
                 const float av[4] = {__uint_as_float(a4[i][0] << 16), __uint_as_float(a4[i][0] & 0xffff0000u),
                                      __uint_as_float(a4[i][1] << 16), __uint_as_float(a4[i][1] & 0xffff0000u)};
                 float gg[4], xh[4], t1 = 0.f, t2 = 0.f;
@@ -259,10 +264,10 @@
                 t1 *= (1.f / C); t2 *= (1.f / C);
                 f32x4 o4;
 #pragma unroll
-                for (int e = 0; e < 4; ++e) o4[e] = ok[i] ? rs[i] * (gg[e] - t1 - xh[e] * t2) : 0.f;
+                for (int e = 0; e < 4; ++e) o4[e] = ok[i] ? rs[i] * fmaf(-xh[e], t2, gg[e] - t1) : 0.f;
                 const bf16x4 ob = f2bf4(o4);
                 if (act) {
-                    *(bf16x4*)(a.da1 + (size_t)min(wg_row0 + row, a.Mw - 1) * C + c0) = ob;
+                    *(bf16x4*)(a.da1 + (size_t)prow(min(wg_row0 + row, a.Mc - 1)) * C + c0) = ob;
                     *(bf16x4*)(Xs + row * PX + c0) = ob;
                 }
             }
@@ -296,7 +301,7 @@
         bf16x8 xf[KS];
 #pragma unroll
         for (int ks = 0; ks < KS; ++ks) xf[ks] = *(const bf16x8*)(Xs + (wave * 16 * MT + 16 * mt + fr) * PX + 32 * ks + 8 * g);
-        const int m = min(wg_row0 + wave * 16 * MT + 16 * mt + fr, a.Mw - 1), w = m / a.Lp, t = m - w * a.Lp;
+        const int mc = min(wg_row0 + wave * 16 * MT + 16 * mt + fr, a.Mc - 1), w = RR ? rr_window(a.rr, mc) : mc / a.Lp, t = mc - w * (RR ? a.rr.L : a.Lp);
         for (int kt = 0; kt < a.h * (HS / 16); ++kt) {
             f32x4 acc = {0.f, 0.f, 0.f, 0.f};
 #pragma unroll
@@ -307,6 +312,19 @@
             *(bf16x4*)(a.doh + (((size_t)w * a.h + kt / (HS / 16)) * a.Lp + t) * HS + 16 * (kt % (HS / 16)) + 4 * g) = f2bf4(acc);
         }
     }
+    if constexpr (RR) {
+        const int w0 = rr_window(a.rr, wg_row0), w1 = rr_window(a.rr, min(wg_row0 + ROWS, a.Mc));
+        const u32x4 z = {0u, 0u, 0u, 0u};
+        const int ca = a.rr.pad * (C / 8), ch = a.rr.pad * (HS / 8);
+        for (int i = tid; i < (w1 - w0) * ca; i += NT) {
+            const int w = w0 + i / ca, c = i % ca;
+            *(u32x4*)(a.da1 + ((size_t)w * a.Lp + a.rr.L) * C + 8 * c) = z;
+        }
+        for (int i = tid; i < (w1 - w0) * a.h * ch; i += NT) {
+            const int wh = w0 * a.h + i / ch, c = i % ch;
+            *(u32x4*)(a.doh + ((size_t)wh * a.Lp + a.rr.L) * HS + 8 * c) = z;
+        }
+    }
 }
 
 }
@@ -317,28 +335,48 @@
 }
 
 extern "C" size_t swv2_proj_ln_bwd_ws_floats(int Mw, int C) { return (Mw > 0 && C > 0) ? (size_t)cdiv(Mw, 64) * 2 * C : 0; }
+
+extern "C" int swv2_real_row(int mc, int L, int Lp) {
+    if (Lp <= 0 || L < 0 || L > Lp || mc < 0) return -1;
+    return rr_row(real_rows(L, Lp), mc);
+}
+
+static int proj_ln_wg_rows(int Bw, int Lp, int C) { return (C == 192 || (long)Bw * Lp >= 128 * 256) ? 128 : 64; }
+
+extern "C" int swv2_proj_ln_workgroups(int Bw, int Lp, int L, int C) {
+    if (Bw <= 0 || Lp <= 0 || L < 0 || L > Lp) return -1;
+    return cdiv((long)Bw * real_rows(L, Lp).L, proj_ln_wg_rows(Bw, Lp, C));
+}
 
 extern "C" int swv2_proj_ln_fwd(const swv2_proj_ln_args* a, void* stream) {
     SWV2_CHECK_ARG(a && a->oh && a->wp && a->bp && a->gamma && a->beta && a->x && a->a1 && a->mean && a->rstd && a->y,
                    "swv2_proj_ln_fwd: null pointer");
     SWV2_CHECK_ARG(a->Bw > 0 && a->Lp > 0 && a->Lp % 16 == 0 && a->rows_per_sample > 0, "swv2_proj_ln_fwd: bad geometry");
+    SWV2_CHECK_ARG(a->L >= 0 && a->L <= a->Lp, "swv2_proj_ln_fwd: L = %d outside [0, Lp = %d]", a->L, a->Lp);
     if (!swv2_proj_ln_supported(a->C, a->heads, a->C == 192 ? 32 : 16)) {
         swv2_set_error("swv2_proj_ln_fwd: C=%d heads=%d not instantiated; use swv2_linear + swv2_ln_residual_fwd", a->C, a->heads);
         return SWV2_ERR_UNSUPPORTED;
     }
-    const int Mw = a->Bw * a->Lp;
+    const RealRows rr = real_rows(a->L, a->Lp);
+    const int Mc = a->Bw * rr.L;
     ProjLnFwd k = {(const uint16_t*)a->oh, (const uint16_t*)a->wp, a->bp, a->gamma, a->beta, a->scale, a->rowidx, a->x,
-                   (uint16_t*)a->a1, a->mean, a->rstd, a->y, Mw, a->Lp, a->heads, a->rows_per_sample, a->eps};
+                   (uint16_t*)a->a1, a->mean, a->rstd, a->y, Mc, a->Lp, a->heads, a->rows_per_sample, a->eps, rr};
     hipStream_t st = (hipStream_t)stream;
-    const bool mt2 = Mw >= 128 * 256;
+    const bool mt2 = proj_ln_wg_rows(a->Bw, a->Lp, a->C) == 128;
+    const int nblk = swv2_proj_ln_workgroups(a->Bw, a->Lp, a->L, a->C);
 #define PL_CASE(CC)                                                                                                  \
     case CC:                                                                                                         \
-        if (mt2) hipLaunchKernelGGL((proj_ln_fwd_kernel<CC, 2>), dim3(cdiv(Mw, 128)), dim3(256), 0, st, k);          \
-        else hipLaunchKernelGGL((proj_ln_fwd_kernel<CC, 1>), dim3(cdiv(Mw, 64)), dim3(256), 0, st, k);               \
+        if (mt2 && rr.pad) hipLaunchKernelGGL((proj_ln_fwd_kernel<CC, 2, 16, 4, true>), dim3(nblk), dim3(256), 0, st, k);  \
+        else if (mt2) hipLaunchKernelGGL((proj_ln_fwd_kernel<CC, 2>), dim3(nblk), dim3(256), 0, st, k);              \
+        else if (rr.pad) hipLaunchKernelGGL((proj_ln_fwd_kernel<CC, 1, 16, 4, true>), dim3(nblk), dim3(256), 0, st, k);    \
+        else hipLaunchKernelGGL((proj_ln_fwd_kernel<CC, 1>), dim3(nblk), dim3(256), 0, st, k);                       \
         break;
     switch (a->C) {
         PL_CASE(32) PL_CASE(64) PL_CASE(96) PL_CASE(128)
-        case 192: hipLaunchKernelGGL((proj_ln_fwd_kernel<192, 1, 32, 8>), dim3(cdiv(Mw, 128)), dim3(512), 0, st, k); break;
+        case 192:
+            if (rr.pad) hipLaunchKernelGGL((proj_ln_fwd_kernel<192, 1, 32, 8, true>), dim3(nblk), dim3(512), 0, st, k);
+            else hipLaunchKernelGGL((proj_ln_fwd_kernel<192, 1, 32, 8>), dim3(nblk), dim3(512), 0, st, k);
+            break;
     }
 #undef PL_CASE
     SWV2_CHECK_LAUNCH("swv2_proj_ln_fwd");
@@ -351,24 +389,31 @@
     SWV2_CHECK_ARG(a && a->dy && a->a1 && a->mean && a->rstd && a->gamma && a->wpt && a->da1 && a->doh && a->dgamma && a->dbeta &&
                        a->ws, "swv2_proj_ln_bwd: null pointer");
     SWV2_CHECK_ARG(a->Bw > 0 && a->Lp > 0 && a->Lp % 16 == 0 && a->rows_per_sample > 0, "swv2_proj_ln_bwd: bad geometry");
+    SWV2_CHECK_ARG(a->L >= 0 && a->L <= a->Lp, "swv2_proj_ln_bwd: L = %d outside [0, Lp = %d]", a->L, a->Lp);
     if (!swv2_proj_ln_supported(a->C, a->heads, a->C == 192 ? 32 : 16)) {
         swv2_set_error("swv2_proj_ln_bwd: C=%d heads=%d not instantiated; use swv2_ln_residual_bwd + swv2_linear", a->C, a->heads);
         return SWV2_ERR_UNSUPPORTED;
     }
-    const int Mw = a->Bw * a->Lp;
+    const RealRows rr = real_rows(a->L, a->Lp);
+    const int Mc = a->Bw * rr.L;
     ProjLnBwd k = {a->dy, (const uint16_t*)a->a1, a->mean, a->rstd, a->gamma, a->scale, a->rowidx, (const uint16_t*)a->wpt,
-                   (uint16_t*)a->da1, (uint16_t*)a->doh, a->ws, Mw, a->Lp, a->heads, a->rows_per_sample};
+                   (uint16_t*)a->da1, (uint16_t*)a->doh, a->ws, Mc, a->Lp, a->heads, a->rows_per_sample, rr};
     hipStream_t st = (hipStream_t)stream;
-    const bool mt2 = Mw >= 128 * 256;
+    const bool mt2 = proj_ln_wg_rows(a->Bw, a->Lp, a->C) == 128;
+    const int nblk = swv2_proj_ln_workgroups(a->Bw, a->Lp, a->L, a->C);
 #define PL_CASE(CC)                                                                                                  \
     case CC:                                                                                                         \
-        if (mt2) hipLaunchKernelGGL((proj_ln_bwd_kernel<CC, 2>), dim3(cdiv(Mw, 128)), dim3(256), 0, st, k);          \
-        else hipLaunchKernelGGL((proj_ln_bwd_kernel<CC, 1>), dim3(cdiv(Mw, 64)), dim3(256), 0, st, k);               \
+        if (mt2 && rr.pad) hipLaunchKernelGGL((proj_ln_bwd_kernel<CC, 2, 16, 4, true>), dim3(nblk), dim3(256), 0, st, k);  \
+        else if (mt2) hipLaunchKernelGGL((proj_ln_bwd_kernel<CC, 2>), dim3(nblk), dim3(256), 0, st, k);              \
+        else if (rr.pad) hipLaunchKernelGGL((proj_ln_bwd_kernel<CC, 1, 16, 4, true>), dim3(nblk), dim3(256), 0, st, k);    \
+        else hipLaunchKernelGGL((proj_ln_bwd_kernel<CC, 1>), dim3(nblk), dim3(256), 0, st, k);                       \
         break;
-    int nblk = cdiv(Mw, mt2 ? 128 : 64);
     switch (a->C) {
         PL_CASE(32) PL_CASE(64) PL_CASE(96) PL_CASE(128)
-        case 192: nblk = cdiv(Mw, 128); hipLaunchKernelGGL((proj_ln_bwd_kernel<192, 1, 32, 8>), dim3(nblk), dim3(512), 0, st, k); break;
+        case 192:
+            if (rr.pad) hipLaunchKernelGGL((proj_ln_bwd_kernel<192, 1, 32, 8, true>), dim3(nblk), dim3(512), 0, st, k);
+            else hipLaunchKernelGGL((proj_ln_bwd_kernel<192, 1, 32, 8>), dim3(nblk), dim3(512), 0, st, k);
+            break;
     }
 #undef PL_CASE
     if (deferred) *deferred = nblk;
diff --git a/swin_v2_weather_amd/ops.py b/swin_v2_weather_amd/ops.py
--- a/swin_v2_weather_amd/ops.py
+++ b/swin_v2_weather_amd/ops.py
@@ -599,7 +599,7 @@
     return dx, da2, dh
 
 
-def proj_ln_fwd(oh, wp, bp, gamma, beta, scale, rowidx, x, Bw, Lp, heads, rows_per_sample, eps=1e-5, out=None):
+def proj_ln_fwd(oh, wp, bp, gamma, beta, scale, rowidx, x, Bw, Lp, heads, rows_per_sample, eps=1e-5, out=None, Lwin=0):
     Cc, Mw = wp.shape[0], Bw * Lp
     _chk(oh, BF16, "proj_ln oh"); _chk(wp, BF16, "proj_ln wp"); _chk(x, torch.float32, "proj_ln x")
     dev = x.device
@@ -609,12 +609,12 @@
     a = L.ProjLnArgs()
     a.oh, a.wp, a.bp, a.gamma, a.beta, a.scale, a.rowidx, a.x = (_p(t) for t in (oh, wp, bp, gamma, beta, scale, rowidx, x))
     a.a1, a.mean, a.rstd, a.y = (_p(t) for t in (a1, mean, rstd, y))
-    a.Bw, a.Lp, a.heads, a.C, a.rows_per_sample, a.eps = Bw, Lp, heads, Cc, rows_per_sample, eps
+    a.Bw, a.Lp, a.heads, a.C, a.rows_per_sample, a.eps, a.L = Bw, Lp, heads, Cc, rows_per_sample, eps, Lwin
     L.check(_timed("proj_ln_fwd", L.load().swv2_proj_ln_fwd, C.byref(a), _stream()), "swv2_proj_ln_fwd")
     return y, a1, mean, rstd
 
 
-def proj_ln_bwd(dy, a1, mean, rstd, gamma, scale, rowidx, wpt, dgamma, dbeta, Bw, Lp, heads, rows_per_sample, out=None, ws=None):
+def proj_ln_bwd(dy, a1, mean, rstd, gamma, scale, rowidx, wpt, dgamma, dbeta, Bw, Lp, heads, rows_per_sample, out=None, ws=None, Lwin=0):
     Cc, Mw = wpt.shape[1], Bw * Lp
     _chk(dy, torch.float32, "proj_ln dy"); _chk(a1, BF16, "proj_ln a1"); _chk(wpt, BF16, "proj_ln wpt")
     dev = dy.device
@@ -626,7 +626,7 @@
     a = L.ProjLnBwdArgs()
     a.dy, a.a1, a.mean, a.rstd, a.gamma, a.scale, a.rowidx, a.wpt = (_p(t) for t in (dy, a1, mean, rstd, gamma, scale, rowidx, wpt))
     a.da1, a.doh, a.dgamma, a.dbeta, a.ws = (_p(t) for t in (da1, doh, dgamma, dbeta, ws))
-    a.Bw, a.Lp, a.heads, a.C, a.rows_per_sample = Bw, Lp, heads, Cc, rows_per_sample
+    a.Bw, a.Lp, a.heads, a.C, a.rows_per_sample, a.L = Bw, Lp, heads, Cc, rows_per_sample, Lwin
     L.check(_timed("proj_ln_bwd", L.load().swv2_proj_ln_bwd, C.byref(a), _stream()), "swv2_proj_ln_bwd")
     return da1, doh
 
```

Result: no change. 225.4, median of 2 (+0.1%).
